# yanqinJiang/Animate3D

Measured on AMD Instinct MI355X. Metric: UNet denoise-steps/sec, 4view×16frame×512² MV-VDM @1/2/4/8 GPU, higher is better.
Workload: dtype bf16; 1 GPU; BASELINE config 2: 4 views x 16 frames x 512^2 px (64x64 latent), CFG-doubled batch V=8 videos, one MVUNetMotionModel.forward per step, SD1.5 MV-VDM UNet 1.53 B params, seeded synthetic weights; parallelism=single GPU

## Files before the change

### animate3d_amd/csrc/gemm_common.h

```cpp
#pragma once
#include "common.h"

struct GemmParams {
  const uint16_t* X; int64_t ldx;
  const uint16_t* W; int64_t ldw;
  const float* bias;
  const uint16_t* rowbias; int64_t rb_div;
  const uint16_t* R; int64_t ldr;
  uint16_t* Y; int64_t ldy;
  int64_t M, N, K;
  float alpha, beta;
  int vec16;
  int out_f32;
  int B, H, Wd, Cin, Ho, Wo, stride, up, He, We;
  int64_t tiles_n, tiles_m;
  int ksplit, nk_item;
  float* ws; int64_t ws_bytes;
  const uint16_t* X2; int64_t ldx2; int64_t K1;
};

constexpr int EPI_LINEAR = 0, EPI_GEGLU = 1;

static inline int a3d_gemm_kernel_of(int flags) { return flags & A3D_GEMM_KERNEL_MASK; }
static inline int a3d_gemm_reserved_cus_of(int flags) { return flags & A3D_GEMM_RESERVED_CUS_MASK; }

A3D_DEV float epi_scale(float v, float alpha) { return __fmul_rn(v, alpha); }
A3D_DEV float epi_axpy(float v, float beta, float r) { return __fmaf_rn(beta, r, v); }

A3D_DEV float gelu_erf(float gte) {
  const float x = fabsf(gte) * 0.70710678118654752f;
  const float t = __builtin_amdgcn_rcpf(fmaf(0.3275911f, x, 1.0f));
  float poly = fmaf(1.061405429f, t, -1.453152027f);
  poly = fmaf(poly, t, 1.421413741f);
  poly = fmaf(poly, t, -0.284496736f);
  poly = fmaf(poly, t, 0.254829592f);
  poly *= t;
  const float e = __builtin_amdgcn_exp2f(-x * x * 1.4426950408889634f);
  const float erfx = fmaf(-poly, e, 1.0f);
  const float hg = __fmul_rn(0.5f, gte);
  return __fmaf_rn(fabsf(hg), erfx, hg);
}

A3D_DEV f32x2_t splat2(float v) { return f32x2_t{v, v}; }
A3D_DEV f32x2_t gelu_erf2(f32x2_t g) {
  const f32x2_t x = __builtin_elementwise_abs(g) * 0.70710678118654752f;
  const f32x2_t den = __builtin_elementwise_fma(splat2(0.3275911f), x, splat2(1.0f));
  const f32x2_t t = {__builtin_amdgcn_rcpf(den[0]), __builtin_amdgcn_rcpf(den[1])};
  f32x2_t poly = __builtin_elementwise_fma(splat2(1.061405429f), t, splat2(-1.453152027f));
  poly = __builtin_elementwise_fma(poly, t, splat2(1.421413741f));
  poly = __builtin_elementwise_fma(poly, t, splat2(-0.284496736f));
  poly = __builtin_elementwise_fma(poly, t, splat2(0.254829592f));
  poly = poly * t;
  const f32x2_t a = (-x) * x * 1.4426950408889634f;
  const f32x2_t e = {__builtin_amdgcn_exp2f(a[0]), __builtin_amdgcn_exp2f(a[1])};
  const f32x2_t erfx = __builtin_elementwise_fma(-poly, e, splat2(1.0f));
  const f32x2_t hg = g * 0.5f;
  return __builtin_elementwise_fma(__builtin_elementwise_abs(hg), erfx, hg);
}
A3D_DEV void geglu8(const float (&hv)[8], const float (&gv)[8], const float (&bh)[8], const float (&bg)[8], float (&y)[8]) {
#pragma unroll
  for (int e = 0; e < 4; ++e) {
    const f32x2_t gg = f32x2_t{gv[2 * e], gv[2 * e + 1]} + f32x2_t{bg[2 * e], bg[2 * e + 1]};
    const f32x2_t hh = f32x2_t{hv[2 * e], hv[2 * e + 1]} + f32x2_t{bh[2 * e], bh[2 * e + 1]};
    const f32x2_t yy = hh * gelu_erf2(gg);
    y[2 * e] = yy[0]; y[2 * e + 1] = yy[1];
  }
}

static __device__ u32x4_t g_zero_page[4];

A3D_DEV uint32_t lds_addr(const void* p) {
  return (uint32_t)(uintptr_t)(__attribute__((address_space(3))) const void*)p;
}
A3D_DEV void glds16_v(const void* gsrc, uint32_t lds_dst) {
  unsigned keep;
  asm volatile("s_mov_b32 %0, m0\n\ts_mov_b32 m0, %2\n\ts_nop 0\n\tglobal_load_lds_dwordx4 %1, off\n\ts_mov_b32 m0, %0"
               : "=&s"(keep) : "v"(gsrc), "s"(__builtin_amdgcn_readfirstlane(lds_dst)) : "memory");
}
A3D_DEV void glds16_s(uint32_t voff, const void* sbase, uint32_t lds_dst) {
  unsigned keep;
  asm volatile("s_mov_b32 %0, m0\n\ts_mov_b32 m0, %3\n\ts_nop 0\n\tglobal_load_lds_dwordx4 %1, %2\n\ts_mov_b32 m0, %0"
               : "=&s"(keep) : "v"(voff), "s"(sbase), "s"(__builtin_amdgcn_readfirstlane(lds_dst)) : "memory");
}
A3D_DEV const uint16_t* scalar_ptr(const uint16_t* ptr) {
  const uint64_t a = (uint64_t)(uintptr_t)ptr;
  return (const uint16_t*)(uintptr_t)(((uint64_t)(uint32_t)__builtin_amdgcn_readfirstlane((int)(a >> 32)) << 32) |
                                      (uint32_t)__builtin_amdgcn_readfirstlane((int)(uint32_t)a));
}
A3D_DEV u32x4_t lds_vload128(const void* p) {
  return *(const volatile __attribute__((address_space(3))) u32x4_t*)(uintptr_t)lds_addr(p);
}
A3D_DEV u32x2_t lds_vload64(const void* p) {
  return *(const volatile __attribute__((address_space(3))) u32x2_t*)(uintptr_t)lds_addr(p);
}
A3D_DEV void wave_lds_fence() {
  __builtin_amdgcn_fence(__ATOMIC_RELEASE, "wavefront");
  __builtin_amdgcn_wave_barrier();
  __builtin_amdgcn_fence(__ATOMIC_ACQUIRE, "wavefront");
}

A3D_DEV void tile_barrier() {
  asm volatile("s_barrier" ::: "memory");
  __builtin_amdgcn_sched_barrier(0);
}

template <int NB> struct WaveCols {
  static constexpr int PASSES = (NB + 1) / 2;
  int first, last;
  __device__ __forceinline__ explicit WaveCols(int wn) : first(NB == 5 ? wn * 4 : wn * NB), last(NB == 5 ? 8 + wn : wn * NB + NB - 1) {}
  __device__ __forceinline__ int block(int tn) const { return tn < NB - 1 ? first + tn : last; }
  A3D_DEV int pass_width(int ps) { return 2 * ps + 1 < NB ? 64 : 32; }
  __device__ __forceinline__ int pass_col0(int ps) const { return block(2 * ps) * 32; }
};

constexpr int BIAS_IMG_STRIDE = 2048;
constexpr int BIAS_IMG_ROWBIAS = 1280;
constexpr int BIAS_IMG_DMA = 1024;
A3D_DEV const float* bias_image(const char* img, int par) { return reinterpret_cast<const float*>(img + par * BIAS_IMG_STRIDE); }
A3D_DEV const uint16_t* rowbias_image(const char* img, int par) {
  return reinterpret_cast<const uint16_t*>(img + par * BIAS_IMG_STRIDE + BIAS_IMG_ROWBIAS);
}
template <int THREADS> A3D_DEV void zero_absent_bias_images(char* img, const float* bias, const uint16_t* rowbias, int tid) {
  if (!bias || !rowbias) {
    uint32_t* const bz = reinterpret_cast<uint32_t*>(img);
    for (int i = tid; i < 2 * BIAS_IMG_STRIDE / 4; i += THREADS) {
      const int o = (i * 4) % BIAS_IMG_STRIDE;
      if ((o < BIAS_IMG_ROWBIAS && !bias) || (o >= BIAS_IMG_ROWBIAS && !rowbias)) bz[i] = 0u;
    }
    asm volatile("s_waitcnt lgkmcnt(0)" ::: "memory");
    tile_barrier();
  }
}

template <int NB> A3D_DEV void read_frags(const char* stage, uint32_t xrd, uint32_t wrd, uint32_t wrd_last, uint32_t ko, u32x4_t (&fx)[2],
                                          u32x4_t (&fw)[NB]) {
  const char* xs = stage + xrd;
  const char* ws = stage + wrd;
  const char* wl = stage + wrd_last;
#pragma unroll
  for (int tm = 0; tm < 2; ++tm) fx[tm] = *reinterpret_cast<const u32x4_t*>(xs + tm * 4096 + ko);
#pragma unroll
  for (int tn = 0; tn < NB - 1; ++tn) fw[tn] = *reinterpret_cast<const u32x4_t*>(ws + tn * 4096 + ko);
  fw[NB - 1] = *reinterpret_cast<const u32x4_t*>(wl + ko);
}

template <int EPI, int NB>
A3D_DEV void epilogue_rounded(const GemmParams& p, f32x16_t (&acc)[NB][2], float* const stg, const float* const bias_lds,
                              const uint16_t* const rowbias_lds, const int64_t m0, const int64_t n0, const int wm, const WaveCols<NB> wc,
                              const int lane) {
  const int wblk = wc.first, wblk_last = wc.last;
  auto pass_cols = [&](int ps) { return (2 * ps + 1 < NB) ? 64 : 32; };
  auto pass_col0 = [&](int ps) { return ((2 * ps + 1 < NB) ? wblk + 2 * ps : wblk_last) * 32; };
  const int l31 = lane & 31, g = lane >> 5;
  constexpr int NP = (NB + 1) / 2;
  constexpr int RS = (EPI == EPI_GEGLU) ? 64 : 128;
  char* const stg16 = reinterpret_cast<char*>(stg);
  const int wsw = (EPI == EPI_GEGLU) ? ((l31 >> 1) & 3) : (l31 & 7);
  const int whalf = 8 * (g ^ ((l31 >> 3) & 1));
  auto unswap = [](u32x4_t o, int row) {
    const bool sw = row & 8;
    u32x4_t r;
    r[0] = sw ? o[2] : o[0]; r[1] = sw ? o[3] : o[1]; r[2] = sw ? o[0] : o[2]; r[3] = sw ? o[1] : o[3];
    return r;
  };
  constexpr int BUF2 = 32 * RS;
#pragma unroll
  for (int pi = 0; pi < 2 * NP; ++pi) {
    const int tm = pi / NP, ps = pi % NP;
    const int ncol = pass_cols(ps);
    const int64_t mbase = m0 + wm * 64 + tm * 32;
    const int64_t nbase = n0 + pass_col0(ps);
    char* const sb = stg16 + (pi & 1) * BUF2;
    if constexpr (EPI == EPI_GEGLU) {
      u32x4_t bq[2][4];
      auto fetch = [&](int q2, int slot) __attribute__((always_inline)) {
#pragma unroll
        for (int h = 0; h < 2; ++h) {
          const int c0 = 8 * (2 * q2 + h) + 4 * g;
          bq[slot][2 * h] = lds_vload128(bias_lds + pass_col0(ps) + c0);
          bq[slot][2 * h + 1] = lds_vload128(bias_lds + pass_col0(ps) + 32 + c0);
        }
      };
      fetch(0, 0);
#pragma unroll
      for (int q2 = 0; q2 < 2; ++q2) {
        if (q2 + 1 < 2) fetch(q2 + 1, (q2 + 1) & 1);
        __builtin_amdgcn_sched_barrier(0);
        float hv[8], gv[8], bh[8], bg[8], y[8];
#pragma unroll
        for (int h = 0; h < 2; ++h) {
          const u32x4_t b0 = bq[q2 & 1][2 * h], b1 = bq[q2 & 1][2 * h + 1];
#pragma unroll
          for (int j = 0; j < 4; ++j) { bh[4 * h + j] = __uint_as_float(b0[j]); bg[4 * h + j] = __uint_as_float(b1[j]); }
#pragma unroll
          for (int j = 0; j < 4; ++j) { hv[4 * h + j] = acc[2 * ps][tm][4 * (2 * q2 + h) + j]; gv[4 * h + j] = acc[2 * ps + 1][tm][4 * (2 * q2 + h) + j]; }
        }
        geglu8(hv, gv, bh, bg, y);
#pragma unroll
        for (int h = 0; h < 2; ++h) {
          u32x2_t o;
          o[0] = pack16(y[4 * h], y[4 * h + 1]);
          o[1] = pack16(y[4 * h + 2], y[4 * h + 3]);
          *reinterpret_cast<u32x2_t*>(sb + l31 * RS + 16 * ((2 * q2 + h) ^ wsw) + whalf) = o;
        }
      }
      wave_lds_fence();
      const int cc = lane & 3;
      const int64_t oc = nbase / 2 + 8 * cc;
      u32x4_t ob[2];
#pragma unroll
      for (int j = 0; j < 2; ++j) {
        const int row = 16 * j + (lane >> 2);
        ob[j] = *reinterpret_cast<const u32x4_t*>(sb + row * RS + 16 * (cc ^ ((row >> 1) & 3)));
      }
#pragma unroll
      for (int j = 0; j < 2; ++j) {
        const int row = 16 * j + (lane >> 2);
        const int64_t m = mbase + row;
        const u32x4_t o = unswap(ob[j], row);
        *reinterpret_cast<u32x4_t*>(p.Y + m * p.ldy + oc) = o;
      }
    } else {
      constexpr int NQ = 8;
      const int nq = (2 * ps + 1 < NB) ? 8 : 4;
      u32x4_t bq[3];
      u32x2_t tq[3];
      auto fetch = [&](int idx, int slot) __attribute__((always_inline)) {
        const int c0 = (idx >> 2) * 32 + 8 * (idx & 3) + 4 * g;
        bq[slot] = lds_vload128(bias_lds + pass_col0(ps) + c0);
        tq[slot] = lds_vload64(rowbias_lds + pass_col0(ps) + c0);
      };
      auto quads = [&](auto with_c) __attribute__((always_inline)) {
        constexpr bool WITH = decltype(with_c)::value;
        if constexpr (WITH) { fetch(0, 0); fetch(1, 1); }
#pragma unroll
        for (int idx = 0; idx < NQ; ++idx) {
          if (idx >= nq) continue;
          const int tl = idx >> 2, q = idx & 3;
          const int tn = 2 * ps + tl;
          if constexpr (WITH) {
            if (idx + 2 < nq) fetch(idx + 2, (idx + 2) % 3);
            __builtin_amdgcn_sched_barrier(0);
          }
          float v[4] = {acc[tn][tm][4 * q], acc[tn][tm][4 * q + 1], acc[tn][tm][4 * q + 2], acc[tn][tm][4 * q + 3]};
          if constexpr (WITH) {
            const u32x4_t b = bq[idx % 3];
            v[0] += __uint_as_float(b[0]); v[1] += __uint_as_float(b[1]); v[2] += __uint_as_float(b[2]); v[3] += __uint_as_float(b[3]);
            const u32x2_t tb = tq[idx % 3];
            v[0] += lo16(tb[0]); v[1] += hi16(tb[0]); v[2] += lo16(tb[1]); v[3] += hi16(tb[1]);
          }
#pragma unroll
          for (int e = 0; e < 4; ++e) v[e] = epi_scale(v[e], p.alpha);
          u32x2_t o;
          o[0] = pack16(v[0], v[1]);
          o[1] = pack16(v[2], v[3]);
          *reinterpret_cast<u32x2_t*>(sb + l31 * RS + 16 * ((4 * tl + q) ^ wsw) + whalf) = o;
          if constexpr (WITH) __builtin_amdgcn_sched_barrier(0);
        }
      };
      if (p.bias || p.rowbias) quads(std::true_type{});
      else quads(std::false_type{});
      wave_lds_fence();
      const int lpr = ncol / 8;
      const int cc = lane & (lpr - 1);
      u32x4_t ob[4];
#pragma unroll
      for (int j = 0; j < 4; ++j) {
        if (j * (64 / lpr) >= 32) continue;
        const int row = (64 / lpr) * j + lane / lpr;
        ob[j] = *reinterpret_cast<const u32x4_t*>(sb + row * RS + 16 * (cc ^ (row & 7)));
      }
#pragma unroll
      for (int j = 0; j < 4; ++j) {
        if (j * (64 / lpr) >= 32) continue;
        const int row = (64 / lpr) * j + lane / lpr;
        const int64_t m = mbase + row;
        const u32x4_t o = unswap(ob[j], row);
        *reinterpret_cast<u32x4_t*>(p.Y + m * p.ldy + nbase + 8 * cc) = o;
      }
    }
  }
}

template <int NB>
A3D_DEV void epilogue_residual(const GemmParams& p, f32x16_t (&acc)[NB][2], float* const stg, const float* const bias_lds,
                               const uint16_t* const rowbias_lds, const int64_t m0, const int64_t n0, const int wm, const WaveCols<NB> wc,
                               const int lane) {
  const int l31 = lane & 31, g = lane >> 5;
  constexpr int SROW = 68;
  constexpr int NP = WaveCols<NB>::PASSES;
  u32x4_t rres[2][4];
  auto load_res = [&](int pi, int slot) {
    const int tm = pi / NP, ps = pi % NP;
    const int64_t mbase = m0 + wm * 64 + tm * 32;
    const int64_t nbase = n0 + wc.pass_col0(ps);
    if (WaveCols<NB>::pass_width(ps) == 64) {
#pragma unroll
      for (int j = 0; j < 4; ++j) {
        const int64_t m = mbase + 8 * j + (lane >> 3);
        rres[slot][j] = *reinterpret_cast<const u32x4_t*>(p.R + m * p.ldr + nbase + 8 * (lane & 7));
      }
    } else {
#pragma unroll
      for (int j = 0; j < 2; ++j) {
        const int64_t m = mbase + 16 * j + (lane >> 2);
        rres[slot][j] = *reinterpret_cast<const u32x4_t*>(p.R + m * p.ldr + nbase + 8 * (lane & 3));
      }
    }
  };
  load_res(0, 0);
#pragma unroll
  for (int pi = 0; pi < 2 * NP; ++pi) {
    const int tm = pi / NP, ps = pi % NP;
    const int ncol = WaveCols<NB>::pass_width(ps);
    if (pi + 1 < 2 * NP) load_res(pi + 1, (pi + 1) & 1);
#pragma unroll
    for (int tl = 0; tl < 2; ++tl) {
      const int tn = 2 * ps + tl;
      if (tn < NB) {
#pragma unroll
        for (int q = 0; q < 4; ++q) {
          float4 v;
          v.x = acc[tn][tm][4 * q]; v.y = acc[tn][tm][4 * q + 1]; v.z = acc[tn][tm][4 * q + 2]; v.w = acc[tn][tm][4 * q + 3];
          *reinterpret_cast<float4*>(stg + l31 * SROW + tl * 32 + 8 * q + 4 * g) = v;
        }
      }
    }
    wave_lds_fence();
    const int64_t mbase = m0 + wm * 64 + tm * 32;
    const int64_t nbase = n0 + wc.pass_col0(ps);

    const int lpr = ncol / 8;
    const int cc = lane & (lpr - 1);
    const int64_t n = nbase + 8 * cc;
    const int ncl = wc.pass_col0(ps) + 8 * cc;
    float bv[8];
#pragma unroll
    for (int e = 0; e < 8; ++e) bv[e] = bias_lds[ncl + e];
    const u32x4_t tb = *reinterpret_cast<const u32x4_t*>(rowbias_lds + ncl);
#pragma unroll
    for (int j = 0; j < 4; ++j) {
      if (j * (64 / lpr) >= 32) continue;
      const int row = (64 / lpr) * j + lane / lpr;
      const int64_t m = mbase + row;
      const float4 a0 = *reinterpret_cast<const float4*>(stg + row * SROW + 8 * cc);
      const float4 a1 = *reinterpret_cast<const float4*>(stg + row * SROW + 8 * cc + 4);
      float v[8] = {a0.x, a0.y, a0.z, a0.w, a1.x, a1.y, a1.z, a1.w};
#pragma unroll
      for (int e = 0; e < 8; ++e) v[e] += bv[e];
#pragma unroll
      for (int e = 0; e < 4; ++e) { v[2 * e] += lo16(tb[e]); v[2 * e + 1] += hi16(tb[e]); }
#pragma unroll
      for (int e = 0; e < 8; ++e) v[e] = epi_scale(v[e], p.alpha);
      const u32x4_t tr = rres[pi & 1][j];
#pragma unroll
      for (int e = 0; e < 4; ++e) { v[2 * e] = epi_axpy(v[2 * e], p.beta, lo16(tr[e])); v[2 * e + 1] = epi_axpy(v[2 * e + 1], p.beta, hi16(tr[e])); }
      u32x4_t o;
#pragma unroll
      for (int e = 0; e < 4; ++e) o[e] = pack16(v[2 * e], v[2 * e + 1]);
      *reinterpret_cast<u32x4_t*>(p.Y + m * p.ldy + n) = o;
    }
    wave_lds_fence();
  }
}


__attribute__((visibility("hidden"))) int A3D_FN(a3d_launch_gemm_pp)(int conv, int epi, int nb, hipStream_t stream, const GemmParams& p, int cus);
__attribute__((visibility("hidden"))) int A3D_FN(a3d_launch_gemm_ring)(int nb, hipStream_t stream, const GemmParams& p, int cus);
```

### animate3d_amd/csrc/gemm_conv.hip

```cpp
#include "gemm_common.h"

namespace {

constexpr int BM = 128, BN = 128;
template <int BKT> struct TileCfg {
  static constexpr int LROW = BKT + 8;
  static constexpr int TILE_ELEMS = 128 * LROW;
  static constexpr int STAGE_BYTES = 2 * 2 * TILE_ELEMS * 2;
  static constexpr int EPI_BYTES = 4 * 32 * 68 * 4;
  static constexpr int SMEM_BYTES = STAGE_BYTES > EPI_BYTES ? STAGE_BYTES : EPI_BYTES;
  static constexpr int CPR = BKT / 8;
  static constexpr int RPT = 256 / CPR;
  static constexpr int NPASS = 128 / RPT;
};



template <int CONV, int EPI, int BKT, bool RES>
__global__ __launch_bounds__(256, (BKT == 64 ? 2 : 3)) void gemm_kernel(const GemmParams p) {
  using TC = TileCfg<BKT>;
  constexpr int LROW = TC::LROW, TILE_ELEMS = TC::TILE_ELEMS, NPASS = TC::NPASS, RPT = TC::RPT, BK = BKT;
  extern __shared__ __attribute__((aligned(16))) uint16_t smem[];
  const int tid = threadIdx.x;
  const int lane = tid & 63, wid = tid >> 6;
  const int wm = wid >> 1, wn = wid & 1;
  const int l31 = lane & 31, g = lane >> 5;

  const int64_t nblk = p.tiles_n * p.tiles_m;
  const int64_t lid = xcd_remap(blockIdx.x, nblk);
  const int64_t tile_n = lid % p.tiles_n, tile_m = lid / p.tiles_n;
  const int64_t m0 = tile_m * BM, n0 = tile_n * BN;

  const int kc = tid % TC::CPR;
  const int srow = tid / TC::CPR;

  const uint16_t* a_ptr[NPASS];
  int a_b[CONV == 2 ? NPASS : 1], a_y[CONV == 2 ? NPASS : 1], a_x[CONV == 2 ? NPASS : 1];
  bool a_ok[NPASS];
  int a_mask[NPASS];
#pragma unroll
  for (int i = 0; i < NPASS; ++i) {
    int64_t m = m0 + srow + RPT * i;
    a_ok[i] = m < p.M;
    if (m >= p.M) m = p.M - 1;
    if constexpr (CONV != 0) {
      const int hw = p.Ho * p.Wo;
      const int b = (int)(m / hw);
      const int rem = (int)(m - (int64_t)b * hw);
      const int oy = rem / p.Wo, ox = rem - oy * p.Wo;
      if constexpr (CONV == 2) {
        a_b[i] = b; a_y[i] = oy; a_x[i] = ox;
        a_ptr[i] = nullptr; a_mask[i] = 0;
      } else {
        const int y0 = oy * p.stride - 1, x0 = ox * p.stride - 1;
        a_ptr[i] = p.X + (((int64_t)b * p.H + y0) * p.Wd + x0) * p.Cin + kc * 8;
        int mask = 0;
#pragma unroll
        for (int t = 0; t < 9; ++t) {
          const int yy = y0 + t / 3, xx = x0 + t % 3;
          if (a_ok[i] && yy >= 0 && yy < p.H && xx >= 0 && xx < p.Wd) mask |= 1 << t;
        }
        a_mask[i] = mask;
      }
    } else {
      a_ptr[i] = p.X + m * p.ldx + kc * 8;
      a_mask[i] = 0;
    }
  }
  const uint16_t* w_ptr[NPASS];
#pragma unroll
  for (int i = 0; i < NPASS; ++i) {
    int64_t n = n0 + srow + RPT * i;
    if (n >= p.N) n = p.N - 1;
    w_ptr[i] = p.W + n * p.ldw + kc * 8;
  }

  struct RegTile { u32x4_t a[NPASS], w[NPASS]; };
  RegTile rt0, rt1;
  auto load_tile = [&](int64_t k0, RegTile& rt) {
    u32x4_t (&ra)[NPASS] = rt.a; u32x4_t (&rw)[NPASS] = rt.w;
    if constexpr (CONV != 0) {
      {
        const int kt64 = (int)(k0 >> 6);
        const int c64 = kt64 / 9, t = kt64 - 9 * c64;
        k0 = (int64_t)t * p.Cin + c64 * 64 + (k0 & 63);
      }
      const int tap = (int)(k0 / p.Cin);
      const int ci0 = (int)(k0 - (int64_t)tap * p.Cin);
      const int ky = tap / 3, kx = tap - ky * 3;
      if constexpr (CONV == 1) {
        const int64_t toff = ((int64_t)ky * p.Wd + kx) * p.Cin + ci0;
#pragma unroll
        for (int i = 0; i < NPASS; ++i) {
          if ((a_mask[i] >> tap) & 1) ra[i] = *reinterpret_cast<const u32x4_t*>(a_ptr[i] + toff);
          else ra[i] = u32x4_t{0u, 0u, 0u, 0u};
        }
      } else {
        const int He = p.He, We = p.We;
#pragma unroll
        for (int i = 0; i < NPASS; ++i) {
          const int yy = a_y[i] + ky - 1, xx = a_x[i] + kx - 1;
          const bool ok = a_ok[i] && yy >= 0 && yy < He && xx >= 0 && xx < We;
          if (ok) {
            const uint16_t* src = p.X + (((int64_t)a_b[i] * p.H + (yy >> 1)) * p.Wd + (xx >> 1)) * p.Cin + ci0 + kc * 8;
            ra[i] = *reinterpret_cast<const u32x4_t*>(src);
          } else {
            ra[i] = u32x4_t{0u, 0u, 0u, 0u};
          }
        }
      }
    } else {
#pragma unroll
      for (int i = 0; i < NPASS; ++i) ra[i] = *reinterpret_cast<const u32x4_t*>(a_ptr[i] + k0);
    }
#pragma unroll
    for (int i = 0; i < NPASS; ++i) rw[i] = *reinterpret_cast<const u32x4_t*>(w_ptr[i] + k0);
  };
  auto store_tile = [&](int buf, const RegTile& rt) {
    const u32x4_t (&ra)[NPASS] = rt.a; const u32x4_t (&rw)[NPASS] = rt.w;
    uint16_t* As = smem + (buf * 2 + 0) * TILE_ELEMS;
    uint16_t* Ws = smem + (buf * 2 + 1) * TILE_ELEMS;
#pragma unroll
    for (int i = 0; i < NPASS; ++i) {
      *reinterpret_cast<u32x4_t*>(As + (srow + RPT * i) * LROW + kc * 8) = ra[i];
      *reinterpret_cast<u32x4_t*>(Ws + (srow + RPT * i) * LROW + kc * 8) = rw[i];
    }
  };

  f32x16_t acc[2][2];
#pragma unroll
  for (int a = 0; a < 2; ++a)
#pragma unroll
    for (int b = 0; b < 2; ++b)
#pragma unroll
      for (int r = 0; r < 16; ++r) acc[a][b][r] = 0.f;

  u32x4_t rres[RES ? 4 : 1];
  const int ecc = lane & 7;
  const int64_t en = n0 + wn * 64 + 8 * ecc;
  const bool epf = RES && (EPI == EPI_LINEAR) && p.R != nullptr && p.vec16 && en + 8 <= p.N;
  auto prefetch_residual = [&](int tm) {
    if constexpr (RES) {
#pragma unroll
      for (int j = 0; j < 4; ++j) {
        int64_t m = m0 + wm * 64 + tm * 32 + 8 * j + (lane >> 3);
        if (m >= p.M) m = p.M - 1;
        rres[j] = *reinterpret_cast<const u32x4_t*>(p.R + m * p.ldr + en);
      }
    }
  };

  const int64_t nk = p.K / BK;
  auto compute = [&](int cur) {
    const uint16_t* As = smem + (cur * 2 + 0) * TILE_ELEMS;
    const uint16_t* Ws = smem + (cur * 2 + 1) * TILE_ELEMS;
    u32x4_t fw[2][2], fa[2][2];
    auto load_frags = [&](int slot, int ks) {
#pragma unroll
      for (int t = 0; t < 2; ++t) {
        fw[slot][t] = *reinterpret_cast<const u32x4_t*>(Ws + (wn * 64 + t * 32 + l31) * LROW + ks * 16 + g * 8);
        fa[slot][t] = *reinterpret_cast<const u32x4_t*>(As + (wm * 64 + t * 32 + l31) * LROW + ks * 16 + g * 8);
      }
    };
    load_frags(0, 0);
#pragma unroll
    for (int ks = 0; ks < BK / 16; ++ks) {
      if (ks + 1 < BK / 16) load_frags((ks + 1) & 1, ks + 1);
#pragma unroll
      for (int tn = 0; tn < 2; ++tn)
#pragma unroll
        for (int tm = 0; tm < 2; ++tm) acc[tn][tm] = mfma32(fw[ks & 1][tn], fa[ks & 1][tm], acc[tn][tm]);
    }
  };

  load_tile(0, rt0);
  store_tile(0, rt0);
  if (nk > 1) load_tile(1 * BK, rt0);
  if (nk > 2) load_tile(2 * BK, rt1);
  __syncthreads();
  for (int64_t kt = 0;;) {
    if (kt + 1 >= nk && epf) prefetch_residual(0);
    compute(0);
    if (kt + 1 < nk) store_tile(1, rt0);
    if (kt + 3 < nk) load_tile((kt + 3) * BK, rt0);
    __syncthreads();
    if (++kt >= nk) break;
    if (kt + 1 >= nk && epf) prefetch_residual(0);
    compute(1);
    if (kt + 1 < nk) store_tile(0, rt1);
    if (kt + 3 < nk) load_tile((kt + 3) * BK, rt1);
    __syncthreads();
    if (++kt >= nk) break;
  }

  constexpr int SROW = 68;
  float* const stg = reinterpret_cast<float*>(smem) + wid * (32 * SROW);
#pragma unroll
  for (int tm = 0; tm < 2; ++tm) {
  if (tm == 1) __syncthreads();
#pragma unroll
  for (int tn = 0; tn < 2; ++tn)
#pragma unroll
    for (int q = 0; q < 4; ++q) {
      float4 v;
      v.x = acc[tn][tm][4 * q]; v.y = acc[tn][tm][4 * q + 1]; v.z = acc[tn][tm][4 * q + 2]; v.w = acc[tn][tm][4 * q + 3];
      *reinterpret_cast<float4*>(stg + l31 * SROW + tn * 32 + 8 * q + 4 * g) = v;
    }
  __syncthreads();
  const int64_t mbase = m0 + wm * 64 + tm * 32;

  if constexpr (EPI == EPI_GEGLU) {
    const int cc = lane & 3;
    const int64_t nh = n0 + wn * 64 + 8 * cc;
    const int64_t oc = (n0 + wn * 64) / 2 + 8 * cc;
    if (nh + 32 < p.N + 0 && oc + 8 <= p.N / 2) {
      float bh[8], bg[8];
#pragma unroll
      for (int e = 0; e < 8; ++e) { bh[e] = p.bias ? p.bias[nh + e] : 0.f; bg[e] = p.bias ? p.bias[nh + 32 + e] : 0.f; }
#pragma unroll
      for (int j = 0; j < 2; ++j) {
        const int row = 16 * j + (lane >> 2);
        const int64_t m = mbase + row;
        if (m >= p.M) continue;
        const float4 h0 = *reinterpret_cast<const float4*>(stg + row * SROW + 8 * cc);
        const float4 h1 = *reinterpret_cast<const float4*>(stg + row * SROW + 8 * cc + 4);
        const float4 g0 = *reinterpret_cast<const float4*>(stg + row * SROW + 32 + 8 * cc);
        const float4 g1 = *reinterpret_cast<const float4*>(stg + row * SROW + 32 + 8 * cc + 4);
        const float hv[8] = {h0.x, h0.y, h0.z, h0.w, h1.x, h1.y, h1.z, h1.w};
        const float gv[8] = {g0.x, g0.y, g0.z, g0.w, g1.x, g1.y, g1.z, g1.w};
        float y[8];
        geglu8(hv, gv, bh, bg, y);
        u32x4_t o;
#pragma unroll
        for (int e = 0; e < 4; ++e) o[e] = pack16(y[2 * e], y[2 * e + 1]);
        *reinterpret_cast<u32x4_t*>(p.Y + m * p.ldy + oc) = o;
      }
    }
  } else {
    const int cc = lane & 7;
    const int64_t n = n0 + wn * 64 + 8 * cc;
    if (n < p.N) {
      const bool full = (n + 8 <= p.N) && p.vec16;
      float bv[8];
#pragma unroll
      for (int e = 0; e < 8; ++e) bv[e] = (p.bias && n + e < p.N) ? p.bias[n + e] : 0.f;
#pragma unroll
      for (int j = 0; j < 4; ++j) {
        const int row = 8 * j + (lane >> 3);
        const int64_t m = mbase + row;
        if (m >= p.M) continue;
        const float4 a0 = *reinterpret_cast<const float4*>(stg + row * SROW + 8 * cc);
        const float4 a1 = *reinterpret_cast<const float4*>(stg + row * SROW + 8 * cc + 4);
        float v[8] = {a0.x, a0.y, a0.z, a0.w, a1.x, a1.y, a1.z, a1.w};
#pragma unroll
        for (int e = 0; e < 8; ++e) v[e] += bv[e];
        const uint16_t* rb = p.rowbias ? p.rowbias + (m / p.rb_div) * p.N + n : nullptr;
        const uint16_t* rr = p.R ? p.R + m * p.ldr + n : nullptr;
        uint16_t* yy = p.Y + m * p.ldy + n;
        if (full) {
          if (rb) {
            const u32x4_t t = *reinterpret_cast<const u32x4_t*>(rb);
#pragma unroll
            for (int e = 0; e < 4; ++e) { v[2 * e] += lo16(t[e]); v[2 * e + 1] += hi16(t[e]); }
          }
#pragma unroll
          for (int e = 0; e < 8; ++e) v[e] = epi_scale(v[e], p.alpha);
          if constexpr (RES) {
            if (rr) {
              const u32x4_t t = rres[j];
#pragma unroll
              for (int e = 0; e < 4; ++e) { v[2 * e] = epi_axpy(v[2 * e], p.beta, lo16(t[e])); v[2 * e + 1] = epi_axpy(v[2 * e + 1], p.beta, hi16(t[e])); }
            }
          }
          if (p.out_f32) {
            float* yf = reinterpret_cast<float*>(p.Y) + m * p.ldy + n;
            *reinterpret_cast<float4*>(yf) = float4{v[0], v[1], v[2], v[3]};
            *reinterpret_cast<float4*>(yf + 4) = float4{v[4], v[5], v[6], v[7]};
          } else {
            u32x4_t o;
#pragma unroll
            for (int e = 0; e < 4; ++e) o[e] = pack16(v[2 * e], v[2 * e + 1]);
            *reinterpret_cast<u32x4_t*>(yy) = o;
          }
        } else {
#pragma unroll
          for (int hh = 0; hh < 2; ++hh) {
            if (n + 4 * hh + 4 > p.N) continue;
            float w[4] = {v[4 * hh], v[4 * hh + 1], v[4 * hh + 2], v[4 * hh + 3]};
            if (rb) {
              const u32x2_t t = *reinterpret_cast<const u32x2_t*>(rb + 4 * hh);
              w[0] += lo16(t[0]); w[1] += hi16(t[0]); w[2] += lo16(t[1]); w[3] += hi16(t[1]);
            }
#pragma unroll
            for (int e = 0; e < 4; ++e) w[e] = epi_scale(w[e], p.alpha);
            if (rr) {
              const u32x2_t t = *reinterpret_cast<const u32x2_t*>(rr + 4 * hh);
              w[0] = epi_axpy(w[0], p.beta, lo16(t[0])); w[1] = epi_axpy(w[1], p.beta, hi16(t[0]));
              w[2] = epi_axpy(w[2], p.beta, lo16(t[1])); w[3] = epi_axpy(w[3], p.beta, hi16(t[1]));
            }
            u32x2_t o;
            o[0] = pack16(w[0], w[1]);
            o[1] = pack16(w[2], w[3]);
            *reinterpret_cast<u32x2_t*>(yy + 4 * hh) = o;
          }
        }
      }
    }
  }
  if (tm == 0 && epf) prefetch_residual(1);
  }
}


constexpr int PBM = 256;
constexpr int NOT_ELIGIBLE = -1000;

inline bool gemm_flags_ok(int flags) {
  return !(flags & ~(A3D_GEMM_RESERVED_CUS_MASK | A3D_GEMM_KERNEL_MASK)) && a3d_gemm_kernel_of(flags) <= A3D_GEMM_RING;
}

inline int device_cus() {
  static int cus_of[64] = {0};
  const int dev = a3d_current_device();
  if (cus_of[dev] == 0) {
    int n = 0;
    if (hipDeviceGetAttribute(&n, hipDeviceAttributeMultiprocessorCount, dev) != hipSuccess) return 0;
    cus_of[dev] = n > 0 ? n : 256;
  }
  return cus_of[dev];
}

constexpr int PERSIST_MIN_FILL = 50;
struct PPPlan { int nb, S, cus; int64_t tiles_m, tiles_n; };
constexpr int SPLITK_MAX = 16;
constexpr int SPLITK_MINK = 9;
template <int CONV, int EPI>
bool plan_persist(const GemmParams& p, int flags, bool allow_split, PPPlan& out) {
  if (a3d_gemm_kernel_of(flags) == A3D_GEMM_TILE128 || p.out_f32) return false;
  const int cus_dev = device_cus();
  if (cus_dev == 0) return false;
  const int reserved = a3d_gemm_reserved_cus_of(flags);
  const int cus = cus_dev - reserved > 32 ? cus_dev - reserved : 32;
  if (!p.vec16 || p.K % 64 != 0 || p.M % PBM != 0 || (p.rowbias && p.rb_div % PBM != 0)) return false;
  if (p.ldw % 64 != 0 || (CONV == 0 && p.ldx % 64 != 0)) return false;
  if (CONV == 0 && (uint64_t)p.ldx * 16u >= (1ull << 31)) return false;
  if ((uint64_t)p.ldw * 16u >= (1ull << 31)) return false;
  if (CONV != 0 && ((uint64_t)p.B * p.H * p.Wd + 2u * p.Wd + 2u) * (uint64_t)p.Cin * 2u >= (1ull << 32)) return false;
  const int64_t tm = (p.M + PBM - 1) / PBM;
  const int nk = (int)(p.K / 64);
  const int unit = CONV ? 9 : 1;
  const int cus_plan = cus_dev;
  constexpr int OVH = 12;
  int64_t best = -1, best1 = -1;
  int bnb = 0, bS = 1, bnb1 = 0;
  for (int nb = 5; nb >= 4; --nb) {
    if (EPI == EPI_GEGLU && nb == 5) continue;
    if (p.N % (nb * 64) != 0) continue;
    const int64_t tiles = tm * (p.N / (nb * 64));
    for (int S = 1; S <= (allow_split && EPI == EPI_LINEAR ? SPLITK_MAX : 1); ++S) {
      if ((nk / unit) % S != 0 || (S > 1 && nk / S < SPLITK_MINK)) continue;
      const int64_t items = tiles * S;
      const int64_t rounds = (items + cus_plan - 1) / cus_plan;
      if (items * 100 < rounds * cus_plan * PERSIST_MIN_FILL) continue;
      if (S > 1 && p.ws != nullptr && items * nb * 65536 > p.ws_bytes) continue;
      const int64_t cost = rounds * (nk / S + OVH) * nb * (nb == 4 ? 108 : 100) + (S > 1 ? 100 * nb : 0);
      if (S == 1 && (best1 < 0 || cost < best1)) { best1 = cost; bnb1 = nb; }
      if (best < 0 || cost < best) { best = cost; bnb = nb; bS = S; }
    }
  }
  if (best < 0) return false;
  if (bS > 1 && best1 >= 0 && best * 100 > best1 * 85) { bnb = bnb1; bS = 1; }
  out.nb = bnb; out.S = bS; out.cus = cus;
  out.tiles_m = tm; out.tiles_n = p.N / (bnb * 64);
  return true;
}

struct RingPlan { int nb, cus, cus_plan; int64_t cost; };
constexpr int RING_VS_PP_PCT = 75;
inline bool plan_ring(const GemmParams& p, int flags, RingPlan& out) {
  if (a3d_gemm_kernel_of(flags) == A3D_GEMM_TILE128 || p.out_f32 || !p.vec16 || p.X2 != nullptr) return false;
  if (p.M % 128 != 0 || p.K % 64 != 0 || p.K < 256 || p.ldx % 64 != 0 || p.ldw % 64 != 0) return false;
  if ((uint64_t)p.ldx * 64u >= (1ull << 32) || (uint64_t)p.ldw * 256u >= (1ull << 32)) return false;
  if (p.rowbias && p.rb_div % 128 != 0) return false;
  const int n = device_cus() ? device_cus() : 256;
  const int reserved = a3d_gemm_reserved_cus_of(flags);
  out.cus_plan = n;
  out.cus = n - reserved > 32 ? n - reserved : 32;
  out.nb = 0; out.cost = 0;
  for (int nb : {5, 4, 2}) {
    if (p.N % (64 * nb) != 0) continue;
    const int64_t tiles = (p.M / 128) * (p.N / (64 * nb));
    const int64_t rounds = (tiles + out.cus - 1) / out.cus;
    const int64_t cost = rounds * (128 + 64 * nb);
    if (out.nb == 0 || cost < out.cost) { out.nb = nb; out.cost = cost; }
  }
  return out.nb != 0;
}

template <int CONV, int EPI>
int try_launch_persist(hipStream_t stream, GemmParams& p, int flags) {
  PPPlan pl;
  if (!plan_persist<CONV, EPI>(p, flags, p.ws != nullptr, pl)) return NOT_ELIGIBLE;
  p.tiles_m = pl.tiles_m; p.tiles_n = pl.tiles_n;
  p.ksplit = pl.S; p.nk_item = (int)(p.K / 64) / pl.S;
  return A3D_FN(a3d_launch_gemm_pp)(CONV, EPI, pl.nb, stream, p, pl.cus);
}


template <int CONV, int EPI, int BKT, bool RES>
int launch_res(hipStream_t stream, GemmParams& p, int64_t nblk) {
  using TC = TileCfg<BKT>;
  static uint64_t attr_done = 0;
  if (int rc = a3d_once_per_device(attr_done, [] {
        return (int)hipFuncSetAttribute(reinterpret_cast<const void*>(&gemm_kernel<CONV, EPI, BKT, RES>),
                                        hipFuncAttributeMaxDynamicSharedMemorySize, TC::SMEM_BYTES); })) return rc;
  gemm_kernel<CONV, EPI, BKT, RES><<<dim3((unsigned)nblk), dim3(256), TC::SMEM_BYTES, stream>>>(p);
  return a3d_launch_status();
}

template <int CONV, int EPI, int BKT>
int launch_bk(hipStream_t stream, GemmParams& p, int64_t nblk) {
  if constexpr (EPI == EPI_LINEAR) {
    if (p.R != nullptr) return launch_res<CONV, EPI, BKT, true>(stream, p, nblk);
  }
  return launch_res<CONV, EPI, BKT, false>(stream, p, nblk);
}

template <int CONV, int EPI = EPI_LINEAR>
int launch(hipStream_t stream, GemmParams& p, int flags) {
  if (!gemm_flags_ok(flags)) return A3D_EINVAL;
  if constexpr (CONV == 0 && EPI == EPI_LINEAR) {
    RingPlan rp;
    if (plan_ring(p, flags, rp)) {
      PPPlan pl;
      bool ring = true;
      if (a3d_gemm_kernel_of(flags) != A3D_GEMM_RING && plan_persist<CONV, EPI>(p, flags, p.ws != nullptr, pl)) {
        const int64_t tiles = pl.tiles_m * pl.tiles_n * pl.S;
        const int64_t pp_cost = ((tiles + rp.cus_plan - 1) / rp.cus_plan) * (256 + 64 * pl.nb) * RING_VS_PP_PCT;
        ring = pl.S == 1 && rp.cost * 100 < pp_cost;
      }
      if (ring) {
        p.tiles_m = p.M / 128; p.tiles_n = p.N / (64 * rp.nb);
        return A3D_FN(a3d_launch_gemm_ring)(rp.nb, stream, p, rp.cus);
      }
    }
  }
  {
    const int rc = try_launch_persist<CONV, EPI>(stream, p, flags);
    if (rc != NOT_ELIGIBLE) return rc;
  }
  p.tiles_m = (p.M + BM - 1) / BM;
  p.tiles_n = (p.N + BN - 1) / BN;
  const int64_t nblk = p.tiles_m * p.tiles_n;
  if (nblk <= 0 || nblk > 0x7fffffffLL) return A3D_EINVAL;
  const bool small = (CONV == 0 && p.K <= 640) || nblk < 768;
  if (small) return launch_bk<CONV, EPI, 32>(stream, p, nblk);
  return launch_bk<CONV, EPI, 64>(stream, p, nblk);
}

template <int CONV>
int64_t splitk_ws_bytes(const GemmParams& p, int flags) {
  PPPlan pl;
  GemmParams q = p;
  q.ws = nullptr; q.ws_bytes = 0;
  if (!gemm_flags_ok(flags)) return 0;
  if (!plan_persist<CONV, EPI_LINEAR>(q, flags, true, pl) || pl.S <= 1) return 0;
  return pl.tiles_m * pl.tiles_n * pl.S * pl.nb * 65536;
}

void attach_workspace(GemmParams& p, void* ws, int64_t ws_bytes) {
  if (ws && ws_bytes > 0 && a3d_aligned(16, ws)) { p.ws = (float*)ws; p.ws_bytes = ws_bytes; }
}

GemmParams dense_params(const void* X, int64_t ldx, const void* W, int64_t ldw, const float* bias, const void* rowbias, int64_t rb_div,
                        const void* R, int64_t ldr, void* Y, int64_t ldy, int64_t M, int64_t N, int64_t K, float alpha, float beta,
                        bool out_f32 = false) {
  GemmParams p{};
  p.X = (const uint16_t*)X; p.ldx = ldx; p.W = (const uint16_t*)W; p.ldw = ldw;
  p.bias = bias; p.rowbias = (const uint16_t*)rowbias; p.rb_div = rowbias ? rb_div : 1;
  p.R = (const uint16_t*)R; p.ldr = ldr; p.Y = (uint16_t*)Y; p.ldy = ldy;
  p.M = M; p.N = N; p.K = K; p.alpha = alpha; p.beta = beta; p.out_f32 = out_f32;
  p.vec16 = (ldy * (out_f32 ? 4 : 2) % 16 == 0) && a3d_aligned(16, Y) && (!R || (ldr % 8 == 0 && a3d_aligned(16, R))) &&
            (!rowbias || (N % 8 == 0 && a3d_aligned(16, rowbias)));
  return p;
}

bool dense_args_ok(const GemmParams& p, uintptr_t y_align, int n_div, int ldy_div) {
  if (!p.X || !p.W || !p.Y || p.M <= 0 || p.N <= 0 || p.K <= 0) return false;
  if (p.K % 64 != 0 || p.N % n_div != 0) return false;
  if (p.ldx % 8 != 0 || p.ldw % 8 != 0 || p.ldy % ldy_div != 0 || (p.R && p.ldr % 4 != 0)) return false;
  if (!a3d_aligned(16, p.X, p.W) || !a3d_aligned(16, p.bias) || !a3d_aligned(y_align, p.Y) || !a3d_aligned(8, p.R, p.rowbias)) return false;
  return !p.rowbias || p.rb_div > 0;
}

int gemm_entry(a3d_stream_t stream, const void* X, int64_t ldx, const void* W, int64_t ldw,
               const float* bias, const void* rowbias, int64_t rb_div, const void* R, int64_t ldr,
               void* Y, int64_t ldy, int64_t M, int64_t N, int64_t K, float alpha, float beta, int flags,
               void* ws, int64_t ws_bytes, int64_t* ws_needed) {
  GemmParams p = dense_params(X, ldx, W, ldw, bias, rowbias, rb_div, R, ldr, Y, ldy, M, N, K, alpha, beta);
  if (!dense_args_ok(p, 8, 4, 4)) return A3D_EINVAL;
  if (ws_needed) { *ws_needed = splitk_ws_bytes<0>(p, flags); return 0; }
  attach_workspace(p, ws, ws_bytes);
  return launch<0>((hipStream_t)stream, p, flags);
}

}

extern "C" int A3D_FN(a3d_gemm)(a3d_stream_t stream, const void* X, int64_t ldx, const void* W, int64_t ldw,
                             const float* bias, const void* rowbias, int64_t rb_div, const void* R, int64_t ldr,
                             void* Y, int64_t ldy, int64_t M, int64_t N, int64_t K, float alpha, float beta, int flags) {
  return gemm_entry(stream, X, ldx, W, ldw, bias, rowbias, rb_div, R, ldr, Y, ldy, M, N, K, alpha, beta, flags, nullptr, 0, nullptr);
}

extern "C" int A3D_FN(a3d_gemm_ws)(a3d_stream_t stream, const void* X, int64_t ldx, const void* W, int64_t ldw,
                                const float* bias, const void* rowbias, int64_t rb_div, const void* R, int64_t ldr,
                                void* Y, int64_t ldy, int64_t M, int64_t N, int64_t K, float alpha, float beta, int flags,
                                void* ws, int64_t ws_bytes, int64_t* ws_needed) {
  return gemm_entry(stream, X, ldx, W, ldw, bias, rowbias, rb_div, R, ldr, Y, ldy, M, N, K, alpha, beta, flags, ws, ws_bytes, ws_needed);
}

extern "C" int A3D_FN(a3d_gemm2)(a3d_stream_t stream, const void* X, int64_t ldx, const void* X2, int64_t ldx2, int64_t K1,
                              const void* W, int64_t ldw, const float* bias, void* Y, int64_t ldy, int64_t M, int64_t N, int64_t K, int flags) {
  GemmParams p = dense_params(X, ldx, W, ldw, bias, nullptr, 1, nullptr, 0, Y, ldy, M, N, K, 1.f, 0.f);
  p.X2 = (const uint16_t*)X2; p.ldx2 = ldx2; p.K1 = K1;
  if (!dense_args_ok(p, 16, 8, 8) || !X2 || K1 <= 0 || K1 >= K || K1 % 64 != 0 || ldx2 % 8 != 0 || !a3d_aligned(16, X2)) return A3D_EINVAL;
  if (!gemm_flags_ok(flags)) return A3D_EINVAL;
  if (ldx2 % 64 != 0 || (uint64_t)ldx2 * 16u >= (1ull << 31)) return A3D_EUNSUPPORTED;
  const int rc = try_launch_persist<0, EPI_LINEAR>((hipStream_t)stream, p, flags);
  return rc == NOT_ELIGIBLE ? A3D_EUNSUPPORTED : rc;
}

extern "C" int A3D_FN(a3d_gemm_f32out)(a3d_stream_t stream, const void* X, int64_t ldx, const void* W, int64_t ldw,
                                    const float* bias, float* Y, int64_t ldy, int64_t M, int64_t N, int64_t K, float alpha) {
  GemmParams p = dense_params(X, ldx, W, ldw, bias, nullptr, 1, nullptr, 0, Y, ldy, M, N, K, alpha, 0.f, true);
  if (!dense_args_ok(p, 16, 8, 4)) return A3D_EINVAL;
  return launch<0>((hipStream_t)stream, p, 0);
}

static int conv_entry(a3d_stream_t stream, const void* X, const void* Wp, const float* bias,
                      const void* rowbias, int64_t rb_div, const void* R, void* Y,
                      int B, int H, int W, int Cin, int Cout, int stride, int up2x, int flags,
                      void* ws, int64_t ws_bytes, int64_t* ws_needed) {
  if (!X || !Wp || !Y || B <= 0 || H <= 0 || W <= 0) return A3D_EINVAL;
  if (Cin % 64 != 0 || Cout % 4 != 0 || (stride != 1 && stride != 2)) return A3D_EINVAL;
  if (up2x < 0 || up2x > 7 || (up2x > 1 && !(up2x & 1)) || (up2x && stride != 1)) return A3D_EINVAL;
  if (!a3d_aligned(16, X, Wp) || !a3d_aligned(16, bias) || !a3d_aligned(8, Y)) return A3D_EINVAL;
  if (rowbias && rb_div <= 0) return A3D_EINVAL;
  const int He = up2x ? 2 * H - ((up2x >> 1) & 1) : H, We = up2x ? 2 * W - ((up2x >> 2) & 1) : W;
  if (He <= 0 || We <= 0) return A3D_EINVAL;
  GemmParams p{};
  p.X = (const uint16_t*)X; p.ldx = Cin; p.W = (const uint16_t*)Wp; p.ldw = (int64_t)9 * Cin;
  p.bias = bias; p.rowbias = (const uint16_t*)rowbias; p.rb_div = rowbias ? rb_div : 1;
  p.R = (const uint16_t*)R; p.ldr = Cout; p.Y = (uint16_t*)Y; p.ldy = Cout;
  p.B = B; p.H = H; p.Wd = W; p.Cin = Cin; p.stride = stride; p.up = up2x ? 1 : 0; p.He = He; p.We = We;
  p.Ho = (He + 2 - 3) / stride + 1; p.Wo = (We + 2 - 3) / stride + 1;
  p.M = (int64_t)B * p.Ho * p.Wo; p.N = Cout; p.K = (int64_t)9 * Cin;
  p.alpha = 1.f; p.beta = 1.f;
  p.vec16 = (Cout % 8 == 0) && a3d_aligned(16, Y, R, rowbias);
  if (ws_needed) { *ws_needed = up2x ? splitk_ws_bytes<2>(p, flags) : splitk_ws_bytes<1>(p, flags); return 0; }
  attach_workspace(p, ws, ws_bytes);
  return up2x ? launch<2>((hipStream_t)stream, p, flags) : launch<1>((hipStream_t)stream, p, flags);
}

extern "C" int A3D_FN(a3d_conv3x3)(a3d_stream_t stream, const void* X, const void* Wp, const float* bias,
                                const void* rowbias, int64_t rb_div, const void* R, void* Y,
                                int B, int H, int W, int Cin, int Cout, int stride, int up2x, int flags) {
  return conv_entry(stream, X, Wp, bias, rowbias, rb_div, R, Y, B, H, W, Cin, Cout, stride, up2x, flags, nullptr, 0, nullptr);
}

extern "C" int A3D_FN(a3d_conv3x3_ws)(a3d_stream_t stream, const void* X, const void* Wp, const float* bias,
                                   const void* rowbias, int64_t rb_div, const void* R, void* Y,
                                   int B, int H, int W, int Cin, int Cout, int stride, int up2x, int flags,
                                   void* ws, int64_t ws_bytes, int64_t* ws_needed) {
  return conv_entry(stream, X, Wp, bias, rowbias, rb_div, R, Y, B, H, W, Cin, Cout, stride, up2x, flags, ws, ws_bytes, ws_needed);
}

extern "C" int A3D_FN(a3d_gemm_geglu)(a3d_stream_t stream, const void* X, int64_t ldx, const void* W, int64_t ldw,
                                   const float* bias, void* Y, int64_t ldy, int64_t M, int64_t N2, int64_t K, int flags) {
  GemmParams p = dense_params(X, ldx, W, ldw, bias, nullptr, 1, nullptr, 0, Y, ldy, M, N2, K, 1.f, 0.f);
  if (!dense_args_ok(p, 16, 64, 8)) return A3D_EINVAL;
  return launch<0, EPI_GEGLU>((hipStream_t)stream, p, flags);
}
```

### animate3d_amd/csrc/gemm_pp.hip

```cpp
#include "gemm_common.h"

namespace {

constexpr int PBM = 256;
template <int NB> struct PPCfg {
  static constexpr int BN = NB * 64;
  static constexpr int XBYTES = PBM * 128;
  static constexpr int WBYTES = BN * 128;
  static constexpr int EPI_BYTES = 8 * 32 * 68 * 4;
  static constexpr int STAGE = (XBYTES + WBYTES) > EPI_BYTES ? (XBYTES + WBYTES) : EPI_BYTES;
  static constexpr int BIAS_OFF = 2 * STAGE;
  static constexpr int SMEM = BIAS_OFF + 2 * BIAS_IMG_STRIDE;
};

constexpr int PP_GM = 8;
A3D_DEV void pp_tile_coords(int64_t t, int64_t tiles_m, int64_t tiles_n, int64_t& tile_m, int64_t& tile_n) {
  const int64_t gsz = PP_GM * tiles_n;
  const int64_t blk = t / gsz;
  const int64_t first = blk * PP_GM;
  const int64_t gm = tiles_m - first < PP_GM ? tiles_m - first : PP_GM;
  const int64_t within = t - blk * gsz;
  tile_n = within / gm;
  tile_m = first + (within - tile_n * gm);
}

template <int CONV, int EPI, int NB, bool RES, bool SPLIT = false, bool TWO = false>
__global__ __launch_bounds__(512, 1) void gemm_pp_kernel(const GemmParams p) {
  static_assert(!TWO || CONV == 0, "the two-source A operand is a dense-GEMM feature");
  using PC = PPCfg<NB>;
  constexpr int PH = 1, NPH = 4;
  constexpr int NP = 4 + NB;
  extern __shared__ __attribute__((aligned(16))) uint16_t smem[];
  char* const smem_b = reinterpret_cast<char*>(smem);
  const int tid = threadIdx.x, lane = tid & 63;
  const int wid = __builtin_amdgcn_readfirstlane(tid >> 6);
  const int wm = wid >> 1, wn = wid & 1;
  const int grp = wid >> 2;
  const int l31 = lane & 31, g = lane >> 5;
  const int lr = lane >> 3, pos = lane & 7;
  const uint32_t lds0 = lds_addr(smem);

  const int S = SPLIT ? p.ksplit : 1;
  const int64_t ntiles = p.tiles_m * p.tiles_n * S;
  const int64_t G = gridDim.x;
  int64_t t = xcd_remap(blockIdx.x, G);
  if (t >= ntiles) return;
  const int nk = SPLIT ? p.nk_item : (int)(p.K / 64);

  const uint32_t koff0 = (uint32_t)((g ^ ((l31 >> 1) & 7)) << 4);
  const uint32_t xrd = (uint32_t)(wm * 64 + l31) * 128u;
  const WaveCols<NB> wc(wn);
  const uint32_t wrd = (uint32_t)PC::XBYTES + (uint32_t)(wc.first * 32 + l31) * 128u;
  const uint32_t wrd_last = (uint32_t)PC::XBYTES + (uint32_t)(wc.last * 32 + l31) * 128u;

  const uint32_t vx0 = (uint32_t)(lr * p.ldx * 2 + ((pos ^ (lr >> 1)) << 4));
  const uint32_t vw0 = (uint32_t)(lr * p.ldw * 2 + ((pos ^ (lr >> 1)) << 4));
  uint32_t aoff[CONV ? 4 : 1];
  uint32_t amask[CONV ? 2 : 1];
  uint32_t sok[CONV ? 2 : 1];
  const int64_t cbias = CONV ? ((int64_t)p.Wd + 1) * p.Cin : 0;
  int64_t ld_m0 = 0, ld_n0 = 0;
  int ld_par = 0;
  int ik0 = 0, itap = 0, ikx = 0, iky = 0;
  uint64_t xck = 0;
  uint64_t zpage = 0;
  if constexpr (CONV != 0) {
    zpage = (uint64_t)(uintptr_t)g_zero_page;
    asm volatile("" : "+s"(zpage));
  }
  uint64_t xk = 0, wk = 0, rbk = 0;
  const uint32_t sx8 = (uint32_t)(p.ldx * 16), sw8 = (uint32_t)(p.ldw * 16);
  uint64_t xk2 = 0;
  const uint32_t vx0b = TWO ? (uint32_t)(lr * p.ldx2 * 2 + ((pos ^ (lr >> 1)) << 4)) : 0u;
  const uint32_t sx8b = TWO ? (uint32_t)(p.ldx2 * 16) : 0u;
  auto setup_tile = [&](int64_t tt) {
    int64_t tile_n, tile_m;
    const int64_t tile_id = SPLIT ? (int64_t)((uint32_t)tt / (uint32_t)S) : tt;
    const int64_t kofs = SPLIT ? (CONV ? ((int64_t)(tt - tile_id * S) * nk / 9) * 64 : (int64_t)(tt - tile_id * S) * nk * 64) : 0;
    pp_tile_coords(tile_id, p.tiles_m, p.tiles_n, tile_m, tile_n);
    ld_m0 = tile_m * PBM; ld_n0 = tile_n * PC::BN;
    ik0 = 0; itap = 0; ikx = 0; iky = 0;
    ld_par ^= 1;
    if constexpr (CONV != 0) xck = (uint64_t)(uintptr_t)p.X - (uint64_t)cbias * 2u + (uint64_t)kofs * 2u;
    if constexpr (CONV == 0) xk = (uint64_t)(uintptr_t)(p.X + (ld_m0 + wid * 32) * p.ldx + kofs);
    if constexpr (TWO) xk2 = (uint64_t)(uintptr_t)(p.X2 + (ld_m0 + wid * 32) * p.ldx2);
    wk = (uint64_t)(uintptr_t)(p.W + (ld_n0 + wid * (NB * 8)) * p.ldw + kofs);
    if (EPI == EPI_LINEAR && p.rowbias) rbk = (uint64_t)(uintptr_t)(p.rowbias + (ld_m0 / p.rb_div) * p.N + ld_n0);
    if constexpr (CONV != 0) {
      amask[0] = 0; amask[1] = 0;
#pragma unroll
      for (int i = 0; i < 4; ++i) {
        const int r = (wid * 4 + i) * 8 + lr;
        const int slot = pos ^ ((r >> 1) & 7);
        const uint32_t m = (uint32_t)ld_m0 + (uint32_t)r;
        const uint32_t hw = (uint32_t)(p.Ho * p.Wo);
        const int b = (int)(m / hw);
        const int rem = (int)(m - (uint32_t)b * hw);
        const int oy = (int)((uint32_t)rem / (uint32_t)p.Wo), ox = rem - oy * p.Wo;
        uint32_t mask = 0;
        if constexpr (CONV == 2) {
          const int sy0 = (oy - 1) >> 1, sx0 = (ox - 1) >> 1;
          aoff[i] = (uint32_t)(((((int64_t)b * p.H + sy0) * p.Wd + sx0) * p.Cin + cbias) * 2 + slot * 16);
#pragma unroll
          for (int tp = 0; tp < 9; ++tp) {
            const int yy = oy + tp / 3 - 1, xx = ox + tp % 3 - 1;
            if (yy >= 0 && yy < p.He && xx >= 0 && xx < p.We) mask |= 1u << tp;
          }
          amask[i >> 1] |= (mask << (9 * (i & 1))) | ((uint32_t)(~oy & 1) << (18 + 2 * (i & 1))) | ((uint32_t)(~ox & 1) << (19 + 2 * (i & 1)));
        } else {
          const int y0 = oy * p.stride - 1, x0 = ox * p.stride - 1;
          aoff[i] = (uint32_t)(((((int64_t)b * p.H + y0) * p.Wd + x0) * p.Cin + cbias) * 2 + slot * 16);
#pragma unroll
          for (int tp = 0; tp < 9; ++tp) {
            const int yy = y0 + tp / 3, xx = x0 + tp % 3;
            if (yy >= 0 && yy < p.H && xx >= 0 && xx < p.Wd) mask |= 1u << tp;
          }
          amask[i >> 1] |= mask << (9 * (i & 1));
        }
      }
      sok[0] = 0; sok[1] = 0;
#pragma unroll
      for (int bit = 0; bit < 18; ++bit) {
        if (__builtin_amdgcn_ballot_w64(((amask[0] >> bit) & 1u) != 0u) == ~0ull) sok[0] |= 1u << bit;
        if (__builtin_amdgcn_ballot_w64(((amask[1] >> bit) & 1u) != 0u) == ~0ull) sok[1] |= 1u << bit;
      }
    }
  };
  auto issue_pieces = [&](int buf, auto a_c, auto b_c) __attribute__((always_inline)) {
    constexpr int A = decltype(a_c)::value, B = decltype(b_c)::value;
    if constexpr (A >= B) return;
    const uint32_t dst = lds0 + (uint32_t)buf * PC::STAGE;
    if constexpr (A == 0) {
      if (ik0 == 0) {
        const uint32_t bdst = lds0 + (uint32_t)PC::BIAS_OFF + (uint32_t)ld_par * BIAS_IMG_STRIDE;
        if (p.bias) {
          if (wid == 0) glds16_s((uint32_t)lane * 16u, p.bias + ld_n0, bdst);
          if (NB == 5 && wid == 1) { if (lane < 16) glds16_s((uint32_t)lane * 16u, p.bias + ld_n0 + BIAS_IMG_DMA / 4, bdst + (uint32_t)BIAS_IMG_DMA); }
        }
        if (EPI == EPI_LINEAR && p.rowbias && wid == 2) {
          if (lane < PC::BN / 8) glds16_s((uint32_t)lane * 16u, (const void*)(uintptr_t)rbk, bdst + (uint32_t)BIAS_IMG_ROWBIAS);
        }
      }
    }
    if constexpr (CONV != 0) {
      const int ky = iky, kx = ikx;
      const uint32_t rowb = (uint32_t)(p.Wd * p.Cin * 2), colb = (uint32_t)(p.Cin * 2);
      const uint32_t yE = (uint32_t)((ky + 1) >> 1) * rowb, yO = (uint32_t)(ky >> 1) * rowb;
      const uint32_t xE = (uint32_t)((kx + 1) >> 1) * colb, xO = (uint32_t)(kx >> 1) * colb;
#pragma unroll
      for (int i = 0; i < 4; ++i) {
        if (i < A || i >= B) continue;
        const uint32_t d = dst + (uint32_t)(wid * 4 + i) * 1024u;
        const uint32_t mk = amask[i >> 1];
        uint32_t vo = aoff[i];
        if constexpr (CONV == 2) vo += (((mk >> (18 + 2 * (i & 1))) & 1u) ? yE : yO) + (((mk >> (19 + 2 * (i & 1))) & 1u) ? xE : xO);
        const int bit = itap + 9 * (i & 1);
        if ((sok[i >> 1] >> bit) & 1u) {
          glds16_s(vo, (const void*)(uintptr_t)xck, d);
        } else {
          const uint64_t src = ((mk >> bit) & 1u) ? xck + vo : zpage;
          glds16_v((const void*)(uintptr_t)src, d);
        }
      }
    } else {
      const bool sec = TWO && ik0 >= (int)p.K1;
      const uint32_t vxs = sec ? vx0b : vx0, sxs = sec ? sx8b : sx8;
      const uint64_t xks = sec ? xk2 : xk;
#pragma unroll
      for (int i = 0; i < 4; ++i) {
        if (i < A || i >= B) continue;
        const int pc = wid * 4 + i;
        glds16_s(vxs ^ (uint32_t)((i & 1) << 6), (const void*)(uintptr_t)(xks + (uint64_t)(uint32_t)(i * sxs)), dst + (uint32_t)pc * 1024u);
      }
    }
#pragma unroll
    for (int i = 0; i < NB; ++i) {
      if (4 + i < A || 4 + i >= B) continue;
      const int pc = wid * NB + i;
      glds16_s(vw0 ^ (uint32_t)((pc & 1) << 6), (const void*)(uintptr_t)(wk + (uint64_t)(uint32_t)(i * sw8)), dst + (uint32_t)PC::XBYTES + (uint32_t)pc * 1024u);
    }
    if constexpr (B == NP) {
      if constexpr (CONV != 0) {
        const uint64_t cin2 = (uint64_t)(uint32_t)p.Cin * 2u;
        wk += cin2;
        ++itap;
        if (++ikx == 3) { ikx = 0; ++iky; }
        if (itap == 9) {
          itap = 0; iky = 0; wk -= 9u * cin2 - 128u;
          if constexpr (CONV == 1) xck -= (2u * (uint64_t)(uint32_t)p.Wd + 2u) * cin2;
          xck += 128u;
        } else if constexpr (CONV == 1) {
          xck += ikx == 0 ? ((uint64_t)(uint32_t)p.Wd - 2u) * cin2 : cin2;
        }
      } else {
        if (TWO && ik0 >= (int)p.K1) xk2 += 128; else xk += 128;
        wk += 128;
      }
      ik0 += 64;
    }
  };
  auto issue_phase = [&](int buf, auto ph_c, bool late) __attribute__((always_inline)) {
    constexpr int ph = decltype(ph_c)::value;
    using I0 = std::integral_constant<int, 0>;
    using I3 = std::integral_constant<int, 3>;
    using I5 = std::integral_constant<int, 5>;
    using I6 = std::integral_constant<int, 6>;
    using IN = std::integral_constant<int, NP>;
    if (!late) {
      if constexpr (ph == 0) issue_pieces(buf, I0{}, I3{});
      if constexpr (ph == 1) issue_pieces(buf, I3{}, I6{});
      if constexpr (ph == 2) issue_pieces(buf, I6{}, IN{});
    } else {
      if constexpr (ph == 1) issue_pieces(buf, I0{}, I5{});
      if constexpr (ph == 2) issue_pieces(buf, I5{}, IN{});
    }
  };

  f32x16_t acc[NB][2];
  u32x4_t fx[PH][2], fw[PH][NB];
  auto load_frags = [&](int buf, int ks0) __attribute__((always_inline)) {
#pragma unroll
    for (int s = 0; s < PH; ++s) read_frags<NB>(smem_b + buf * PC::STAGE, xrd, wrd, wrd_last, koff0 ^ (uint32_t)((ks0 + s) << 5), fx[s], fw[s]);
  };
  auto mfma_phase = [&]() __attribute__((always_inline)) {
#pragma unroll
    for (int s = 0; s < PH; ++s)
#pragma unroll
      for (int tn = 0; tn < NB; ++tn)
#pragma unroll
        for (int tm = 0; tm < 2; ++tm) acc[tn][tm] = mfma32(fw[s][tn], fx[s][tm], acc[tn][tm]);
  };

  zero_absent_bias_images<512>(smem_b + PC::BIAS_OFF, p.bias, EPI == EPI_LINEAR ? p.rowbias : nullptr, tid);
  setup_tile(t);
  issue_pieces(0, std::integral_constant<int, 0>{}, std::integral_constant<int, NP>{});
  asm volatile("s_waitcnt vmcnt(0)" ::: "memory");
  tile_barrier();
  int buf = 0;
  for (;;) {
    int64_t tile_n, tile_m;
    pp_tile_coords(SPLIT ? (int64_t)((uint32_t)t / (uint32_t)S) : t, p.tiles_m, p.tiles_n, tile_m, tile_n);
    const int64_t m0 = tile_m * PBM, n0 = tile_n * PC::BN;
    const int64_t tnext = t + G;
#pragma unroll
    for (int a = 0; a < NB; ++a)
#pragma unroll
      for (int b = 0; b < 2; ++b)
#pragma unroll
        for (int r = 0; r < 16; ++r) acc[a][b][r] = 0.f;
    const int cur_par = ld_par;
    if (grp) tile_barrier();
    for (int kt = 0; kt < nk; ++kt) {
      const bool last = kt + 1 >= nk;
      const bool more = !last || tnext < ntiles;
      const bool late = kt == 0;
      static_for<NPH>([&](auto ph_c) __attribute__((always_inline)) {
        constexpr int ph = decltype(ph_c)::value;
        load_frags(buf, ph * PH);
        if (more) {
          if constexpr (ph == 0 || ph == 1) {
            if (last && (late ? ph == 1 : ph == 0)) setup_tile(tnext);
          }
          issue_phase(buf ^ 1, ph_c, late);
          if constexpr (ph == NPH - 1) { if (grp) asm volatile("s_waitcnt vmcnt(0)" ::: "memory"); }
        }
        asm volatile("s_waitcnt lgkmcnt(0)" ::: "memory");
        tile_barrier();
        __builtin_amdgcn_s_setprio(1);
        mfma_phase();
        __builtin_amdgcn_s_setprio(0);
        __builtin_amdgcn_sched_barrier(0);
        if constexpr (ph == NPH - 1) { if (more && !grp) asm volatile("s_waitcnt vmcnt(0)" ::: "memory"); }
        tile_barrier();
      });
      buf ^= 1;
    }
    if (!grp) tile_barrier();

    if constexpr (SPLIT) {
      float* const wsi = p.ws + ((t * 8 + wid) * (NB * 8)) * 256 + lane * 4;
#pragma unroll
      for (int tn = 0; tn < NB; ++tn)
#pragma unroll
        for (int tm = 0; tm < 2; ++tm)
#pragma unroll
          for (int q = 0; q < 4; ++q)
            *reinterpret_cast<float4*>(wsi + ((tn * 2 + tm) * 4 + q) * 256) =
                float4{acc[tn][tm][4 * q], acc[tn][tm][4 * q + 1], acc[tn][tm][4 * q + 2], acc[tn][tm][4 * q + 3]};
    } else {
      float* const stg = reinterpret_cast<float*>(smem_b + (buf ^ 1) * PC::STAGE) + wid * (32 * 68);
      const float* const bias_lds = bias_image(smem_b + PC::BIAS_OFF, cur_par);
      const uint16_t* const rowbias_lds = rowbias_image(smem_b + PC::BIAS_OFF, cur_par);
      if constexpr (EPI == EPI_GEGLU || !RES) epilogue_rounded<EPI, NB>(p, acc, stg, bias_lds, rowbias_lds, m0, n0, wm, wc, lane);
      else epilogue_residual<NB>(p, acc, stg, bias_lds, rowbias_lds, m0, n0, wm, wc, lane);
    }
    if (tnext >= ntiles) break;
    t = tnext;
  }
}

template <int NB>
__global__ __launch_bounds__(512) void splitk_reduce_kernel(const GemmParams p) {
  using PC = PPCfg<NB>;
  const int tid = threadIdx.x, lane = tid & 63, wid = tid >> 6;
  const int wm = wid >> 1, wn = wid & 1, l31 = lane & 31, g = lane >> 5;
  const WaveCols<NB> wc(wn);
  const int S = p.ksplit;
  int64_t tile_n, tile_m;
  pp_tile_coords(blockIdx.x, p.tiles_m, p.tiles_n, tile_m, tile_n);
  const int64_t m0 = tile_m * PBM, n0 = tile_n * PC::BN;
  const float* const w0 = p.ws + (((int64_t)blockIdx.x * S * 8 + wid) * (NB * 8)) * 256 + lane * 4;
  const int64_t item_stride = (int64_t)8 * NB * 8 * 256;
  const int tn = blockIdx.y;
#pragma unroll
    for (int tm = 0; tm < 2; ++tm) {
      const int64_t m = m0 + wm * 64 + tm * 32 + l31;
      const int64_t nb0 = n0 + wc.block(tn) * 32 + 4 * g;
#pragma unroll
      for (int q = 0; q < 4; ++q) {
        const float* src = w0 + ((tn * 2 + tm) * 4 + q) * 256;
        float4 a = *reinterpret_cast<const float4*>(src);
        for (int s = 1; s < S; ++s) {
          const float4 b = *reinterpret_cast<const float4*>(src + s * item_stride);
          a.x += b.x; a.y += b.y; a.z += b.z; a.w += b.w;
        }
        const int64_t n = nb0 + 8 * q;
        float v[4] = {a.x, a.y, a.z, a.w};
        if (p.bias) {
          const float4 b = *reinterpret_cast<const float4*>(p.bias + n);
          v[0] += b.x; v[1] += b.y; v[2] += b.z; v[3] += b.w;
        }
        if (p.rowbias) {
          const u32x2_t tb = *reinterpret_cast<const u32x2_t*>(p.rowbias + (m / p.rb_div) * p.N + n);
          v[0] += lo16(tb[0]); v[1] += hi16(tb[0]); v[2] += lo16(tb[1]); v[3] += hi16(tb[1]);
        }
#pragma unroll
        for (int e = 0; e < 4; ++e) v[e] = epi_scale(v[e], p.alpha);
        if (p.R) {
          const u32x2_t tr = *reinterpret_cast<const u32x2_t*>(p.R + m * p.ldr + n);
          v[0] = epi_axpy(v[0], p.beta, lo16(tr[0])); v[1] = epi_axpy(v[1], p.beta, hi16(tr[0]));
          v[2] = epi_axpy(v[2], p.beta, lo16(tr[1])); v[3] = epi_axpy(v[3], p.beta, hi16(tr[1]));
        }
        u32x2_t o;
        o[0] = pack16(v[0], v[1]);
        o[1] = pack16(v[2], v[3]);
        *reinterpret_cast<u32x2_t*>(p.Y + m * p.ldy + n) = o;
      }
    }
}

template <int CONV, int EPI, int NB, bool RES, bool SPLIT = false, bool TWO = false>
int launch_pp(hipStream_t stream, const GemmParams& p, int cus) {
  using PC = PPCfg<NB>;
  static uint64_t attr_done = 0;
  if (int rc = a3d_once_per_device(attr_done, [] {
        return (int)hipFuncSetAttribute(reinterpret_cast<const void*>(&gemm_pp_kernel<CONV, EPI, NB, RES, SPLIT, TWO>),
                                        hipFuncAttributeMaxDynamicSharedMemorySize, PC::SMEM); })) return rc;
  const int64_t ntiles = p.tiles_m * p.tiles_n * (SPLIT ? p.ksplit : 1);
  const unsigned grid = (unsigned)(ntiles < cus ? ntiles : cus);
  gemm_pp_kernel<CONV, EPI, NB, RES, SPLIT, TWO><<<dim3(grid), dim3(512), PC::SMEM, stream>>>(p);
  if (int rc = a3d_launch_status()) return rc;
  if constexpr (SPLIT) {
    splitk_reduce_kernel<NB><<<dim3((unsigned)(p.tiles_m * p.tiles_n), NB), dim3(512), 0, stream>>>(p);
    return a3d_launch_status();
  }
  return 0;
}

template <int CONV>
int launch_pp_conv(int epi, int nb, hipStream_t stream, const GemmParams& p, int cus) {
  if (epi == EPI_GEGLU) {
    if constexpr (CONV == 0) { if (nb == 4) return launch_pp<0, EPI_GEGLU, 4, false>(stream, p, cus); }
    return A3D_EUNSUPPORTED;
  }
  if constexpr (CONV == 0) {
    if (p.X2 != nullptr) {
      if (p.R || p.ksplit > 1) return A3D_EUNSUPPORTED;
      if (nb == 5) return launch_pp<0, EPI_LINEAR, 5, false, false, true>(stream, p, cus);
      if (nb == 4) return launch_pp<0, EPI_LINEAR, 4, false, false, true>(stream, p, cus);
      return A3D_EUNSUPPORTED;
    }
  }
  if (p.ksplit > 1) {
    if (nb == 5) return launch_pp<CONV, EPI_LINEAR, 5, false, true>(stream, p, cus);
    if (nb == 4) return launch_pp<CONV, EPI_LINEAR, 4, false, true>(stream, p, cus);
    return A3D_EUNSUPPORTED;
  }
  if (nb == 5) return p.R ? launch_pp<CONV, EPI_LINEAR, 5, true>(stream, p, cus) : launch_pp<CONV, EPI_LINEAR, 5, false>(stream, p, cus);
  if (nb == 4) return p.R ? launch_pp<CONV, EPI_LINEAR, 4, true>(stream, p, cus) : launch_pp<CONV, EPI_LINEAR, 4, false>(stream, p, cus);
  return A3D_EUNSUPPORTED;
}

}

int A3D_FN(a3d_launch_gemm_pp)(int conv, int epi, int nb, hipStream_t stream, const GemmParams& p, int cus) {
  if (conv == 0) return launch_pp_conv<0>(epi, nb, stream, p, cus);
  if (conv == 1) return launch_pp_conv<1>(epi, nb, stream, p, cus);
  return launch_pp_conv<2>(epi, nb, stream, p, cus);
}
```

### animate3d_amd/hip_ops.py

```python
from __future__ import annotations

import ctypes
import os
from dataclasses import dataclass
from typing import Optional

import torch

_LIB_PATH = os.path.join(os.path.dirname(os.path.abspath(__file__)), "lib", "libanimate3d_hip.so")
_lib = None

c_i64, c_int, c_f32, c_f64, c_vp = ctypes.c_int64, ctypes.c_int, ctypes.c_float, ctypes.c_double, ctypes.c_void_p


class _RowMapC(ctypes.Structure):
    _fields_ = [("gdiv", c_i64), ("ga", c_i64), ("gb", c_i64), ("seg_len", c_i64), ("seg_stride", c_i64), ("ld", c_i64)]


@dataclass(frozen=True)
class RowMap:
    gdiv: int
    ga: int
    gb: int
    seg_len: int
    seg_stride: int

    def c(self, ld: int) -> _RowMapC:
        return _RowMapC(self.gdiv, self.ga, self.gb, self.seg_len, self.seg_stride, ld)


def rowmap_rows(m: RowMap, groups: int, step: int, length: int, device="cpu") -> torch.Tensor:
    g = torch.arange(0, groups, step, device=device).view(-1, 1)
    s = torch.arange(length, device=device).view(1, -1)
    return ((g // m.gdiv) * m.ga + (g % m.gdiv) * m.gb + (s // m.seg_len) * m.seg_stride + s % m.seg_len).reshape(-1)


def rowmap_covers(m: RowMap, groups: int, step: int, length: int, rows: int, device="cpu") -> bool:
    if (groups + step - 1) // step * length != rows:
        return False
    idx = rowmap_rows(m, groups, step, length, device)
    return bool(int(idx.min()) >= 0 and int(idx.max()) < rows and torch.unique(idx).numel() == rows)


_SIGNATURES = {
    "a3d_version": (ctypes.c_char_p, []),
    "a3d_gemm_bf16": (c_int, [c_vp, c_vp, c_i64, c_vp, c_i64, c_vp, c_vp, c_i64, c_vp, c_i64, c_vp, c_i64, c_i64, c_i64, c_i64, c_f32, c_f32, c_int]),
    "a3d_gemm_ws_bf16": (c_int, [c_vp, c_vp, c_i64, c_vp, c_i64, c_vp, c_vp, c_i64, c_vp, c_i64, c_vp, c_i64, c_i64, c_i64, c_i64, c_f32, c_f32, c_int,
                                 c_vp, c_i64, ctypes.POINTER(c_i64)]),
    "a3d_gemm2_bf16": (c_int, [c_vp, c_vp, c_i64, c_vp, c_i64, c_i64, c_vp, c_i64, c_vp, c_vp, c_i64, c_i64, c_i64, c_i64, c_int]),
    "a3d_gemm_geglu_bf16": (c_int, [c_vp, c_vp, c_i64, c_vp, c_i64, c_vp, c_vp, c_i64, c_i64, c_i64, c_i64, c_int]),
    "a3d_conv3x3_bf16": (c_int, [c_vp, c_vp, c_vp, c_vp, c_vp, c_i64, c_vp, c_vp, c_int, c_int, c_int, c_int, c_int, c_int, c_int, c_int]),
    "a3d_conv3x3_ws_bf16": (c_int, [c_vp, c_vp, c_vp, c_vp, c_vp, c_i64, c_vp, c_vp, c_int, c_int, c_int, c_int, c_int, c_int, c_int, c_int,
                                    c_vp, c_i64, ctypes.POINTER(c_i64)]),
    "a3d_flash_attn_bf16": (c_int, [c_vp, c_vp, c_vp, c_vp, c_vp, ctypes.POINTER(_RowMapC), ctypes.POINTER(_RowMapC), ctypes.POINTER(_RowMapC),
                                    c_int, c_int, c_int, c_i64, c_i64, c_f32, c_f32, c_int]),
    "a3d_flash_attn_counted_bf16": (c_int, [c_vp, c_vp, c_vp, c_vp, c_vp, ctypes.POINTER(_RowMapC), ctypes.POINTER(_RowMapC), ctypes.POINTER(_RowMapC),
                                            c_int, c_int, c_int, c_i64, c_i64, c_f32, c_f32, c_int, c_vp]),
    "a3d_flash_attn2_bf16": (c_int, [c_vp, c_vp, c_vp, c_vp, c_vp, c_vp, c_vp, ctypes.POINTER(_RowMapC), ctypes.POINTER(_RowMapC), ctypes.POINTER(_RowMapC),
                                     ctypes.POINTER(_RowMapC), c_int, c_int, c_int, c_i64, c_i64, c_i64, c_f32, c_f32, c_f32, c_int]),
    "a3d_temporal_attn_bf16": (c_int, [c_vp, c_vp, c_vp, c_vp, c_i64, c_vp, c_i64, c_int, c_int, c_i64, c_int, c_int, c_f32]),
    "a3d_temporal_attn_sharded_bf16": (c_int, [c_vp, c_vp, c_i64, c_vp, c_vp, c_i64, c_vp, c_i64, c_int, c_int, c_i64, c_int, c_int, c_f32,
                                               c_int, c_int, c_int, c_i64]),
    "a3d_group_norm_ws_floats": (c_i64, [c_int, c_i64, c_int]),
    "a3d_group_norm_plan": (c_int, [c_i64, c_int, c_int, ctypes.POINTER(c_int)]),
    "a3d_group_norm_bf16": (c_int, [c_vp, c_vp, c_vp, c_vp, c_vp, c_vp, c_int, c_i64, c_int, c_int, c_f32, c_int]),
    "a3d_group_norm2_bf16": (c_int, [c_vp, c_vp, c_int, c_vp, c_int, c_vp, c_vp, c_vp, c_vp, c_int, c_i64, c_int, c_f32, c_int]),
    "a3d_group_norm_sums_bf16": (c_int, [c_vp, c_vp, c_vp, c_vp, c_int, c_i64, c_int, c_int]),
    "a3d_group_norm_apply_bf16": (c_int, [c_vp, c_vp, c_vp, c_vp, c_vp, c_vp, c_int, c_i64, c_int, c_int, c_int]),
    "a3d_layer_norm_bf16": (c_int, [c_vp, c_vp, c_vp, c_vp, c_vp, c_vp, c_i64, c_int, c_f32, c_vp, c_i64, c_i64, c_vp, c_i64, c_i64]),
    "a3d_geglu_bf16": (c_int, [c_vp, c_vp, c_i64, c_vp, c_i64, c_i64, c_i64]),
    "a3d_silu_bf16": (c_int, [c_vp, c_vp, c_vp, c_i64]),
    "a3d_activation_bf16": (c_int, [c_vp, c_vp, c_vp, c_i64, c_int]),
    "a3d_concat_bf16": (c_int, [c_vp, c_vp, c_i64, c_vp, c_i64, c_vp, c_i64]),
    "a3d_timestep_embed_bf16": (c_int, [c_vp, c_vp, c_vp, c_int, c_int]),
    "a3d_im2col_in": (c_int, [c_vp, c_vp, c_int, c_vp, c_int, c_int, c_int, c_int, c_int]),
    "a3d_unpack_out": (c_int, [c_vp, c_vp, c_vp, c_int, c_int, c_int, c_int, c_int, c_int]),
    "a3d_gemm_f32out_bf16": (c_int, [c_vp, c_vp, c_i64, c_vp, c_i64, c_vp, c_vp, c_i64, c_i64, c_i64, c_i64, c_f32]),
    "a3d_softmax_rows_f32_bf16": (c_int, [c_vp, c_vp, c_i64, c_vp, c_i64, c_i64, c_i64]),
    "a3d_softmax_rows_bwd_bf16": (c_int, [c_vp, c_vp, c_i64, c_vp, c_i64, c_vp, c_i64, c_i64, c_i64, c_f32]),
    "a3d_im2col_in_bwd": (c_int, [c_vp, c_vp, c_vp, c_int, c_int, c_int, c_int, c_int, c_f32]),
    "a3d_channel_mix_f32": (c_int, [c_vp, c_vp, c_vp, c_vp, c_vp, c_int, c_int, c_int, c_i64, c_f32]),
    "a3d_cfg_ddim_step_f32": (c_int, [c_vp, c_vp, c_vp, c_vp, c_vp, c_i64, c_int, c_int, c_i64, c_f32, c_f32, c_f32]),
    "a3d_flash_attn_bwd_bf16": (c_int, [c_vp, c_vp, c_vp, c_vp, c_vp, c_vp, c_vp, c_vp, c_vp, c_vp,
                                        ctypes.POINTER(_RowMapC), ctypes.POINTER(_RowMapC), ctypes.POINTER(_RowMapC), ctypes.POINTER(_RowMapC),
                                        ctypes.POINTER(_RowMapC), c_int, c_int, c_int, c_i64, c_i64, c_int, c_f32, c_f32, c_int]),
    "a3d_flash_attn_lse_bf16": (c_int, [c_vp, c_vp, c_vp, c_vp, c_vp, ctypes.POINTER(_RowMapC), ctypes.POINTER(_RowMapC), ctypes.POINTER(_RowMapC),
                                        c_int, c_int, c_int, c_i64, c_i64, c_f32, c_f32, c_int, c_vp]),
    "a3d_attn_delta_bf16": (c_int, [c_vp, c_vp, c_vp, ctypes.POINTER(_RowMapC), ctypes.POINTER(_RowMapC), c_vp, c_int, c_int, c_int, c_i64]),
    "a3d_temporal_attn_bwd_bf16": (c_int, [c_vp, c_vp, c_vp, c_vp, c_i64, c_vp, c_i64, c_vp, c_vp, c_vp, c_i64, c_int, c_int, c_i64, c_int, c_int, c_f32]),
    "a3d_layer_norm_bwd_bf16": (c_int, [c_vp, c_vp, c_vp, c_vp, c_vp, c_vp, c_vp, c_i64, c_int, c_f32, c_int]),
    "a3d_group_norm_bwd_bf16": (c_int, [c_vp, c_vp, c_vp, c_vp, c_vp, c_vp, c_vp, c_vp, c_vp, c_vp, c_int, c_i64, c_int, c_int, c_int]),
    "a3d_geglu_bwd_bf16": (c_int, [c_vp, c_vp, c_i64, c_vp, c_i64, c_vp, c_i64, c_i64, c_i64]),
    "a3d_transpose_bf16": (c_int, [c_vp, c_vp, c_i64, c_vp, c_i64, c_i64, c_i64, c_i64]),
    "a3d_wgrad_ws_floats": (c_i64, [c_i64, c_i64, c_i64]),
    "a3d_wgrad_bf16": (c_int, [c_vp, c_vp, c_i64, c_vp, c_i64, c_vp, c_i64, c_vp, c_i64, c_i64, c_i64, c_f32, c_int]),
    "a3d_colsum_bf16": (c_int, [c_vp, c_vp, c_i64, c_i64, c_i64, c_vp, c_f32, c_int]),
    "a3d_axpby_bf16": (c_int, [c_vp, c_vp, c_vp, c_i64, c_f32, c_f32]),
    "a3d_zero_insert2x_bf16": (c_int, [c_vp, c_vp, c_vp, c_int, c_int, c_int, c_int]),
    "a3d_upsample2x_bwd_bf16": (c_int, [c_vp, c_vp, c_vp, c_int, c_int, c_int, c_int, c_int, c_int]),
    "a3d_sqnorm_f32": (c_int, [c_vp, c_vp, c_i64, c_vp, c_int]),
    "a3d_clip_ctrl_f32": (c_int, [c_vp, c_vp, c_f32, c_f32, c_vp]),
    "a3d_adamw_f32": (c_int, [c_vp, c_vp, c_vp, c_vp, c_vp, c_i64, c_f32, c_f32, c_f32, c_f32, c_f32, c_f32, c_f32, c_vp]),
    "a3d_gs_preprocess_f32": (c_int, [c_vp, c_int, c_int, c_vp, c_i64, c_vp, c_i64, c_vp, c_i64, c_vp, c_i64, c_vp, c_i64, c_int, c_int, c_vp, c_i64, c_vp, c_vp, c_vp, c_vp, c_vp, c_int, c_int, c_f32, c_vp, c_vp, c_vp, c_vp, c_vp, c_vp, c_vp]),
    "a3d_gs_duplicate_f32": (c_int, [c_vp, c_int, c_int, c_int, c_int, c_vp, c_vp, c_vp, c_vp, c_vp, c_vp]),
    "a3d_gs_tile_ranges_f32": (c_int, [c_vp, c_vp, c_i64, c_vp, c_i64]),
    "a3d_gs_render_f32": (c_int, [c_vp, c_int, c_int, c_int, c_int, c_vp, c_vp, c_vp, c_vp, c_vp, c_vp, c_vp, c_vp, c_vp, c_vp, c_vp, c_vp, c_vp]),
    "a3d_gs_render_bwd_f32": (c_int, [c_vp, c_int, c_int, c_int, c_int, c_vp, c_vp, c_vp, c_vp, c_vp, c_vp, c_vp, c_vp, c_vp, c_vp, c_vp,
                                      c_vp, c_vp, c_vp]),
    "a3d_gs_preprocess_bwd_f32": (c_int, [c_vp, c_int, c_int, c_vp, c_i64, c_vp, c_i64, c_vp, c_i64, c_vp, c_i64, c_vp, c_i64, c_int, c_int, c_vp, c_i64, c_vp, c_vp, c_vp, c_vp, c_vp, c_int, c_int, c_f32, c_vp, c_vp, c_vp, c_vp, c_vp, c_vp, c_vp, c_vp, c_vp, c_vp, c_vp, c_vp]),
    "a3d_gs_sum_batch_f32": (c_int, [c_vp, c_vp, c_vp, c_int, c_i64]),
    "a3d_dg_cells_f32": (c_int, [c_vp, c_int, c_vp, c_vp, c_vp]),
    "a3d_dg_mean_partials": (c_i64, [c_int]),
    "a3d_dg_forward_f32": (c_int, [c_vp, c_int, c_int, c_int, c_vp, c_vp, c_vp, c_vp, c_vp, c_vp, c_vp, c_int, c_vp, c_vp, c_vp, c_vp, c_vp, c_vp,
                                   c_vp, c_vp, c_vp]),
    "a3d_dg_backward_ws_floats": (c_i64, [c_int, c_int, c_vp]),
    "a3d_dg_backward_f32": (c_int, [c_vp, c_int, c_int, c_int, c_vp, c_vp, c_vp, c_vp, c_vp, c_vp, c_vp, c_int, c_vp, c_vp, c_vp, c_vp, c_vp,
                                    c_vp, c_vp, c_vp, c_vp, c_vp, c_vp, c_vp, c_vp, c_vp, c_vp]),
    "a3d_knn_f32": (c_int, [c_vp, c_int, c_vp, c_int, c_int, c_f32, c_vp, c_vp]),
    "a3d_arap_energy_f32": (c_int, [c_vp, c_int, c_int, c_int, c_int, c_vp, c_vp, c_i64, c_vp, c_vp, c_vp, c_vp, c_vp, c_vp, c_vp]),
    "a3d_arap_backward_f32": (c_int, [c_vp, c_int, c_int, c_int, c_int, c_vp, c_vp, c_i64, c_vp, c_vp, c_vp, c_vp, c_vp, c_vp, c_vp, c_vp, c_vp]),
    "a3d_mesh_sample_neighbours": (c_int, [c_vp, c_int, c_int, c_vp, c_vp, c_int, c_vp, c_vp]),
    "a3d_mesh_vertex_gaussians_f32": (c_int, [c_vp, c_int, c_int, c_int, c_vp, c_vp, c_vp, c_vp, c_vp, c_vp, c_vp, c_vp, c_int, c_int, c_vp,
                                              c_int, c_vp, c_vp, c_f64, c_f64, c_vp, c_vp, c_vp, c_vp, c_vp, c_vp]),
    "a3d_gaussians_rigid_f32": (c_int, [c_vp, c_int, c_vp, c_vp, c_vp, c_vp, c_vp, c_f64, c_vp, c_vp, c_vp]),
    "a3d_mesh_vertex_normals_f32": (c_int, [c_vp, c_int, c_int, c_int, c_vp, c_vp, c_vp, c_vp, c_vp]),
    "a3d_cameras_spherical_f32": (c_int, [c_vp, c_int, c_vp, c_vp, c_vp, c_vp, c_vp, c_f64, c_f64, c_f64, c_vp, c_vp, c_vp, c_vp, c_vp]),
    "a3d_cameras_random_f32": (c_int, [c_vp, c_int, c_int, c_int, c_vp, c_vp, c_vp, c_vp, c_int, c_int, c_f64, c_f64, c_f64, c_f64, c_f64,
                                       c_vp, c_vp, c_vp, c_vp, c_vp, c_vp, c_vp, c_vp, c_vp]),
    "a3d_cameras_from_c2w_f32": (c_int, [c_vp, c_int, c_vp, c_vp, c_f64, c_f64, c_vp, c_vp, c_vp, c_vp]),
    "a3d_recon_loss_f32": (c_int, [c_vp, c_int, c_int, c_int, c_vp, c_vp, c_vp, c_vp, c_vp, c_f32, c_f64, c_f64, c_vp, c_i64, c_vp]),
    "a3d_recon_loss_bwd_f32": (c_int, [c_vp, c_int, c_int, c_int, c_vp, c_vp, c_vp, c_vp, c_vp, c_f32, c_f32, c_f32, c_vp, c_vp, c_vp]),
    "a3d_image_reg_f32": (c_int, [c_vp, c_int, c_int, c_int, c_vp, c_vp, c_vp, c_f64, c_f64, c_f64, c_vp, c_i64, c_vp]),
    "a3d_image_reg_bwd_f32": (c_int, [c_vp, c_int, c_int, c_int, c_vp, c_vp, c_vp, c_f32, c_f32, c_f32, c_f32, c_f32, c_vp, c_vp, c_vp, c_vp]),
    "a3d_gaussian_reg_f32": (c_int, [c_vp, c_int, c_int, c_vp, c_vp, c_i64, c_vp, c_vp, c_f64, c_f64, c_f64, c_vp, c_i64, c_vp]),
    "a3d_gaussian_reg_bwd_f32": (c_int, [c_vp, c_int, c_int, c_vp, c_vp, c_f32, c_f32, c_f32, c_vp, c_vp, c_vp, c_vp]),
    "a3d_clip_preprocess_lds_limit": (c_i64, []),
    "a3d_clip_preprocess": (c_int, [c_vp, c_vp, c_int, c_int, c_int, c_i64, c_i64, c_i64, c_i64, c_vp, c_int, c_int, c_vp, c_vp, c_int, c_int,
                                    c_vp, c_vp, c_int, c_int, c_int, c_int, c_vp, c_int, c_vp, c_vp, c_int, c_int, c_vp]),
}
_UNSUFFIXED_TWINS = ("a3d_im2col_in", "a3d_unpack_out", "a3d_im2col_in_bwd")
for _name in list(_SIGNATURES):
    if _name.endswith("_bf16"):
        _SIGNATURES[_name[:-5] + "_f16"] = _SIGNATURES[_name]
    elif _name in _UNSUFFIXED_TWINS:
        _SIGNATURES[_name + "_f16"] = _SIGNATURES[_name]
EXPORTED_SYMBOLS = tuple(_SIGNATURES)

_DTYPE_CODE = {torch.float32: 0, torch.bfloat16: 1, torch.float16: 2}
A3D_EUNSUPPORTED = -2


def lib_path() -> str:
    return _LIB_PATH


def load_library():
    global _lib
    if _lib is None:
        if not os.path.exists(_LIB_PATH):
            raise RuntimeError(f"{_LIB_PATH} is missing: run `python -m animate3d_amd.build` (or __graft_entry__.build()). "
                               "There is no CPU fallback for the MI355X kernels.")
        lib = ctypes.CDLL(_LIB_PATH)
        for name, (res, args) in _SIGNATURES.items():
            fn = getattr(lib, name)
            fn.restype, fn.argtypes = res, args
        _lib = lib
    return _lib


GN_PLAN_FIELDS = ("fused", "sg", "nx", "ny", "threads", "rmax", "stream")


def group_norm_plan(rows: int, C: int, groups: int) -> dict:
    out = (c_int * len(GN_PLAN_FIELDS))()
    _check(load_library().a3d_group_norm_plan(rows, C, groups, out), f"a3d_group_norm_plan rows={rows} C={C} groups={groups}")
    plan = dict(zip(GN_PLAN_FIELDS, out))
    plan["iters"] = -(-rows // plan["ny"]) if plan["fused"] else 0
    return plan


def _check(rc: int, what: str):
    if rc != 0:
        kind = {-1: "A3D_EINVAL (shape/alignment precondition)", -2: "A3D_EUNSUPPORTED"}.get(rc, f"hipError {rc}")
        raise RuntimeError(f"{what} failed: {kind}")


def _p(t: Optional[torch.Tensor]):
    return None if t is None else t.data_ptr()


def on_model_device(method):
    import functools

    @functools.wraps(method)
    def wrapper(self, *args, **kwargs):
        dev = self.device
        if dev.type == "cuda" and torch.cuda.current_device() != (dev.index if dev.index is not None else torch.cuda.current_device()):
            with torch.cuda.device(dev):
                return method(self, *args, **kwargs)
        return method(self, *args, **kwargs)
    return wrapper


class _Entry:

    def __init__(self, lib, f16: bool):
        self._lib, self._f16 = lib, f16

    def __getattr__(self, name):
        if self._f16:
            if name.endswith("_bf16"):
                name = name[:-5] + "_f16"
            elif name in _UNSUFFIXED_TWINS:
                name = name + "_f16"
        return getattr(self._lib, name)


class HipOps:

    has_attn_lse = True

    def __init__(self, device: Optional[torch.device] = None, act_dtype: torch.dtype = torch.bfloat16, split_k: bool = True):
        if not torch.cuda.is_available():
            raise RuntimeError("HipOps needs a visible MI355X (torch.cuda.is_available() is False); no CPU fallback exists")
        if act_dtype not in (torch.bfloat16, torch.float16):
            raise ValueError(f"storage type {act_dtype} is not supported (bfloat16 or float16)")
        self.raw_lib = load_library()
        self._kv_row_cache = {}
        self._kv_cover_cache = {}
        self.act_dtype = act_dtype
        self.lib = _Entry(self.raw_lib, act_dtype == torch.float16)
        self.device = torch.device(device) if device is not None else torch.device("cuda", torch.cuda.current_device())
        self.reserved_cus = 0
        self.split_k = bool(split_k)
        self.split_k_gemm = False
        self.attn_counters = None
        self._ws_plan = {}
        self._ws_bufs = {}

    def _workspace(self, need: int) -> torch.Tensor:
        if torch.cuda.is_current_stream_capturing():
            return torch.empty(max(need, 1 << 20), dtype=torch.uint8, device=self.device)
        stream = self._stream()
        buf = self._ws_bufs.get(stream)
        if buf is None or buf.numel() < need:
            buf = self._ws_bufs[stream] = torch.empty(max(need, 1 << 20), dtype=torch.uint8, device=self.device)
        return buf

    def _gemm_flags(self, tile128: bool, ring: bool = False) -> int:
        r = int(self.reserved_cus)
        if not 0 <= r <= 0xFF:
            raise ValueError(f"reserved_cus = {self.reserved_cus}: the flags word of a3d_gemm / a3d_conv3x3 carries 0..255 reserved compute units")
        return r | (0x100 if tile128 else (0x200 if ring else 0))

    def _stream(self):
        return torch.cuda.current_stream(self.device).cuda_stream

    def _act(self, t: torch.Tensor, name: str):
        if t.dtype != self.act_dtype or not t.is_cuda or t.dim() != 2 or t.stride(1) != 1:
            raise RuntimeError(f"{name}: expected a 2-D {self.act_dtype} CUDA tensor with contiguous rows, got {t.dtype} {tuple(t.shape)} {t.device} strides {t.stride()}")
        return t

    def split_cols(self, x, *bounds):
        return tuple(x[:, a:b] for a, b in zip(bounds[:-1], bounds[1:]))

    def empty(self, rows: int, cols: int) -> torch.Tensor:
        return torch.empty((rows, cols), dtype=self.act_dtype, device=self.device)

    def gemm(self, x, w, bias=None, *, residual=None, alpha: float = 1.0, beta: float = 1.0, rowbias=None, rb_div: int = 1, out=None,
             tile128: bool = False, ring: bool = False):
        x, w = self._act(x, "gemm.x"), self._act(w, "gemm.w")
        M, K = x.shape
        N = w.shape[0]
        assert w.shape[1] == K, (x.shape, w.shape)
        y = out if out is not None else self.empty(M, N)
        self._act(y, "gemm.out")
        if residual is not None:
            self._act(residual, "gemm.residual")
            assert residual.shape == (M, N)
        if rowbias is not None:
            self._act(rowbias, "gemm.rowbias")
            assert rowbias.is_contiguous() and rowbias.shape[1] == N
        if bias is not None:
            assert bias.dtype == torch.float32 and bias.numel() == N
        flags = self._gemm_flags(tile128, ring)
        args = (self._stream(), _p(x), x.stride(0), _p(w), w.stride(0), _p(bias), _p(rowbias), rb_div,
                _p(residual), residual.stride(0) if residual is not None else 0, _p(y), y.stride(0), M, N, K, alpha, beta, flags)
        if self.split_k and self.split_k_gemm and not tile128 and M <= 32768 and K >= 1152:
            key = ("gemm", M, N, K, x.stride(0), w.stride(0), y.stride(0), rb_div if rowbias is not None else 0, flags)
            need = self._ws_plan.get(key)
            if need is None:
                q = c_i64(0)
                _check(self.lib.a3d_gemm_ws_bf16(*args, None, 0, ctypes.byref(q)), f"a3d_gemm_ws_bf16 (query) M={M} N={N} K={K}")
                need = self._ws_plan[key] = int(q.value)
            if need > 0:
                ws = self._workspace(need)
                _check(self.lib.a3d_gemm_ws_bf16(*args, _p(ws), need, None), f"a3d_gemm_ws_bf16 M={M} N={N} K={K}")
                return y
        rc = self.lib.a3d_gemm_bf16(*args)
        _check(rc, f"a3d_gemm_bf16 M={M} N={N} K={K}")
        return y

    def gemm2(self, xa, xb, w, bias=None):
        xa, xb, w = self._act(xa, "gemm2.xa"), self._act(xb, "gemm2.xb"), self._act(w, "gemm2.w")
        M, K1 = xa.shape
        K = K1 + xb.shape[1]
        N = w.shape[0]
        assert xb.shape[0] == M and w.shape[1] == K
        if K1 % 64 or K % 64 or N % 8:
            return None
        y = self.empty(M, N)
        rc = self.lib.a3d_gemm2_bf16(self._stream(), _p(xa), xa.stride(0), _p(xb), xb.stride(0), K1, _p(w), w.stride(0), _p(bias), _p(y), y.stride(0),
                                     M, N, K, self._gemm_flags(False))
        if rc == A3D_EUNSUPPORTED:
            return None
        _check(rc, f"a3d_gemm2_bf16 M={M} N={N} K={K1}+{K - K1}")
        return y

    @staticmethod
    def interleave_geglu(w: torch.Tensor) -> torch.Tensor:
        n = w.shape[0] // 2
        assert n % 32 == 0
        h, g = w[:n].reshape(n // 32, 32, *w.shape[1:]), w[n:].reshape(n // 32, 32, *w.shape[1:])
        return torch.stack([h, g], dim=1).reshape(w.shape).contiguous()

    def gemm_geglu(self, x, w_il, bias_il, *, tile128: bool = False):
        x, w_il = self._act(x, "geglu.x"), self._act(w_il, "geglu.w")
        M, K = x.shape
        N2 = w_il.shape[0]
        y = self.empty(M, N2 // 2)
        rc = self.lib.a3d_gemm_geglu_bf16(self._stream(), _p(x), x.stride(0), _p(w_il), w_il.stride(0), _p(bias_il), _p(y), y.stride(0), M, N2, K,
                                          self._gemm_flags(tile128))
        _check(rc, f"a3d_gemm_geglu_bf16 M={M} N2={N2} K={K}")
        return y

    def conv3x3(self, x, B: int, H: int, W: int, w, bias, *, stride: int = 1, up2x: bool = False, rowbias=None, rb_div: int = 1, residual=None,
                up_size=None, tile128: bool = False):
        x, w = self._act(x, "conv.x"), self._act(w, "conv.w")
        Cin = x.shape[1]
        Cout = w.shape[0]
        assert x.is_contiguous() and w.is_contiguous() and x.shape[0] == B * H * W and w.shape[1] == 9 * Cin
        He, We = (2 * H, 2 * W) if up2x else (H, W)
        up_code = 1 if up2x else 0
        if up_size is not None:
            if not up2x or up_size[0] not in (2 * H, 2 * H - 1) or up_size[1] not in (2 * W, 2 * W - 1):
                raise ValueError(f"forced upsample size {tuple(up_size)} is not reachable from {(H, W)} (2x or 2x - 1 per axis)")
            He, We = int(up_size[0]), int(up_size[1])
            up_code |= (2 if He == 2 * H - 1 else 0) | (4 if We == 2 * W - 1 else 0)
        Ho, Wo = (He - 1) // stride + 1, (We - 1) // stride + 1
        y = self.empty(B * Ho * Wo, Cout)
        if residual is not None:
            assert residual.is_contiguous() and residual.shape == y.shape
        if rowbias is not None:
            assert rowbias.is_contiguous() and rowbias.shape[1] == Cout
        flags = self._gemm_flags(tile128)
        args = (self._stream(), _p(x), _p(w), _p(bias), _p(rowbias), rb_div, _p(residual), _p(y), B, H, W, Cin, Cout, stride, up_code, flags)
        if self.split_k and not tile128 and B * Ho * Wo <= 32768:
            key = ("conv", B, H, W, Cin, Cout, stride, up_code, rb_div if rowbias is not None else 0, flags)
            need = self._ws_plan.get(key)
            if need is None:
                q = c_i64(0)
                _check(self.lib.a3d_conv3x3_ws_bf16(*args, None, 0, ctypes.byref(q)), f"a3d_conv3x3_ws_bf16 (query) B={B} H={H} W={W} Cin={Cin} Cout={Cout}")
                need = self._ws_plan[key] = int(q.value)
            if need > 0:
                ws = self._workspace(need)
                _check(self.lib.a3d_conv3x3_ws_bf16(*args, _p(ws), need, None), f"a3d_conv3x3_ws_bf16 B={B} H={H} W={W} Cin={Cin} Cout={Cout}")
                return y, Ho, Wo
        rc = self.lib.a3d_conv3x3_bf16(*args)
        _check(rc, f"a3d_conv3x3_bf16 B={B} H={H} W={W} Cin={Cin} Cout={Cout} stride={stride} up={up2x}")
        return y, Ho, Wo

    def flash_attn(self, q, k, v, qmap: RowMap, kmap: RowMap, groups: int, heads: int, q_len: int, kv_len: int, *,
                   out=None, out_scale: float = 1.0, accumulate: bool = False, causal: bool = False, with_lse: bool = False,
                   accumulation_target: bool = False, exact: bool = False, plain: bool = False):
        q, k, v = self._act(q, "attn.q"), self._act(k, "attn.k"), self._act(v, "attn.v")
        C = q.shape[1]
        D = C // heads
        assert k.stride(0) == v.stride(0)
        o = out if out is not None else self.empty(q.shape[0], C)
        qm, km, om = qmap.c(q.stride(0)), kmap.c(k.stride(0)), qmap.c(o.stride(0))
        flags = (1 if accumulate else 0) | (2 if causal else 0) | (4 if exact else 0) | (8 if plain else 0)
        if with_lse:
            lse = torch.empty((groups, heads, q_len), dtype=torch.float32, device=self.device)
            rc = self.lib.a3d_flash_attn_lse_bf16(self._stream(), _p(q), _p(k), _p(v), _p(o), ctypes.byref(qm), ctypes.byref(km), ctypes.byref(om),
                                                  groups, heads, D, q_len, kv_len, float(D) ** -0.5, out_scale,
                                                  flags, _p(lse))
            _check(rc, f"a3d_flash_attn_lse_bf16 groups={groups} heads={heads} D={D} q_len={q_len} kv_len={kv_len}")
            return o, lse
        if self.attn_counters is not None:
            cnt = self.attn_counters
            assert cnt.dtype == torch.int32 and cnt.is_cuda and cnt.numel() >= 3 and cnt.is_contiguous()
            rc = self.lib.a3d_flash_attn_counted_bf16(self._stream(), _p(q), _p(k), _p(v), _p(o), ctypes.byref(qm), ctypes.byref(km), ctypes.byref(om),
                                                      groups, heads, D, q_len, kv_len, float(D) ** -0.5, out_scale, flags, _p(cnt))
            _check(rc, f"a3d_flash_attn_counted_bf16 groups={groups} heads={heads} D={D} q_len={q_len} kv_len={kv_len}")
            return o
        rc = self.lib.a3d_flash_attn_bf16(self._stream(), _p(q), _p(k), _p(v), _p(o), ctypes.byref(qm), ctypes.byref(km), ctypes.byref(om),
                                          groups, heads, D, q_len, kv_len, float(D) ** -0.5, out_scale, flags)
        _check(rc, f"a3d_flash_attn_bf16 groups={groups} heads={heads} D={D} q_len={q_len} kv_len={kv_len}")
        return o

    def flash_attn2(self, q, k, v, k2, v2, qmap: RowMap, kmap: RowMap, kmap2: RowMap, groups: int, heads: int, q_len: int, kv_len: int,
                    kv_len2: int, *, out_scale2: float = 1.0):
        D = q.shape[1] // heads
        if D not in (40, 80):
            return None
        q, k, v, k2, v2 = self._act(q, "attn.q"), self._act(k, "attn.k"), self._act(v, "attn.v"), self._act(k2, "attn.k2"), self._act(v2, "attn.v2")
        assert k.stride(0) == v.stride(0) and k2.stride(0) == v2.stride(0)
        o = self.empty(q.shape[0], q.shape[1])
        qm, km, km2, om = qmap.c(q.stride(0)), kmap.c(k.stride(0)), kmap2.c(k2.stride(0)), qmap.c(o.stride(0))
        rc = self.lib.a3d_flash_attn2_bf16(self._stream(), _p(q), _p(k), _p(v), _p(k2), _p(v2), _p(o), ctypes.byref(qm), ctypes.byref(km),
                                           ctypes.byref(km2), ctypes.byref(om), groups, heads, D, q_len, kv_len, kv_len2, float(D) ** -0.5,
                                           1.0, out_scale2, 0)
        _check(rc, f"a3d_flash_attn2_bf16 groups={groups} heads={heads} D={D} q_len={q_len} kv_len={kv_len} kv_len2={kv_len2}")
        return o

    def temporal_attn(self, q, k, v, videos: int, frames: int, L: int, heads: int, *, q_f0: int = 0, q_frames: Optional[int] = None,
                      out=None):
        q, k, v = self._act(q, "tattn.q"), self._act(k, "tattn.k"), self._act(v, "tattn.v")
        C = q.shape[1]
        D = C // heads
        assert k.stride(0) == v.stride(0)
        o = self._act(out, "tattn.out") if out is not None else self.empty(q.shape[0], C)
        assert o.shape == (q.shape[0], C)
        if q_frames is None or q_frames == frames:
            assert q.stride(0) == k.stride(0)
            rc = self.lib.a3d_temporal_attn_bf16(self._stream(), _p(q), _p(k), _p(v), q.stride(0), _p(o), o.stride(0),
                                                 videos, frames, L, heads, D, float(D) ** -0.5)
        else:
            assert q.shape[0] == videos * q_frames * L and k.shape[0] == videos * frames * L
            rc = self.lib.a3d_temporal_attn_sharded_bf16(self._stream(), _p(q), q.stride(0), _p(k), _p(v), k.stride(0), _p(o), o.stride(0),
                                                         videos, frames, L, heads, D, float(D) ** -0.5, q_f0, q_frames, q_frames,
                                                         videos * q_frames * L)
        _check(rc, f"a3d_temporal_attn_bf16 videos={videos} frames={frames} L={L} D={D} q_f0={q_f0} q_frames={q_frames}")
        return o

    def group_norm(self, x, B: int, rows: int, gamma, beta, groups: int, eps: float, silu: bool):
        x = self._act(x, "gn.x")
        assert x.is_contiguous() and x.shape[0] == B * rows
        C = x.shape[1]
        y = self.empty(x.shape[0], C)
        ws = torch.empty(int(self.lib.a3d_group_norm_ws_floats(B, rows, groups)), dtype=torch.float32, device=self.device)
        rc = self.lib.a3d_group_norm_bf16(self._stream(), _p(x), _p(y), _p(gamma), _p(beta), _p(ws), B, rows, C, groups, eps, 1 if silu else 0)
        _check(rc, f"a3d_group_norm_bf16 B={B} rows={rows} C={C}")
        return y

    def group_norm2(self, xa, xb, B: int, rows: int, gamma, beta, groups: int, eps: float, silu: bool):
        xa, xb = self._act(xa, "gn2.xa"), self._act(xb, "gn2.xb")
        assert xa.is_contiguous() and xb.is_contiguous() and xa.shape[0] == B * rows == xb.shape[0]
        Ca, Cb = xa.shape[1], xb.shape[1]
        y = self.empty(xa.shape[0], Ca + Cb)
        ws = torch.empty(int(self.lib.a3d_group_norm_ws_floats(B, rows, groups)), dtype=torch.float32, device=self.device)
        rc = self.lib.a3d_group_norm2_bf16(self._stream(), _p(xa), Ca, _p(xb), Cb, _p(y), _p(gamma), _p(beta), _p(ws), B, rows, groups, eps, 1 if silu else 0)
        _check(rc, f"a3d_group_norm2_bf16 B={B} rows={rows} C={Ca}+{Cb}")
        return y

    def group_norm_sums(self, x, B: int, rows: int, groups: int) -> torch.Tensor:
        x = self._act(x, "gn.x")
        assert x.is_contiguous() and x.shape[0] == B * rows
        ws = torch.empty(int(self.lib.a3d_group_norm_ws_floats(B, rows, groups)), dtype=torch.float32, device=self.device)
        sums = torch.empty((B, groups, 2), dtype=torch.float64, device=self.device)
        _check(self.lib.a3d_group_norm_sums_bf16(self._stream(), _p(x), _p(ws), _p(sums), B, rows, x.shape[1], groups),
               f"a3d_group_norm_sums_bf16 B={B} rows={rows} C={x.shape[1]}")
        return sums

    def group_norm_apply(self, x, B: int, rows: int, gamma, beta, groups: int, stats: torch.Tensor, silu: bool):
        x = self._act(x, "gn.x")
        assert x.is_contiguous() and x.shape[0] == B * rows
        assert stats.dtype == torch.float32 and stats.is_contiguous() and stats.shape == (B, groups, 2)
        y = self.empty(x.shape[0], x.shape[1])
        _check(self.lib.a3d_group_norm_apply_bf16(self._stream(), _p(x), _p(y), _p(gamma), _p(beta), _p(stats), B, rows, x.shape[1], groups,
                                                  1 if silu else 0), f"a3d_group_norm_apply_bf16 B={B} rows={rows} C={x.shape[1]}")
        return y

    def layer_norm(self, x, gamma, beta, eps: float, pe1=None, pe1_div: int = 1, pe2=None, pe2_div: int = 1, two: bool = False):
        x = self._act(x, "ln.x")
        assert x.is_contiguous()
        M, C = x.shape
        y1 = self.empty(M, C)
        y2 = self.empty(M, C) if two else None
        for pe in (pe1, pe2):
            if pe is not None:
                self._act(pe, "ln.pe")
                assert pe.is_contiguous() and pe.shape[1] == C
        rc = self.lib.a3d_layer_norm_bf16(self._stream(), _p(x), _p(y1), _p(y2), _p(gamma), _p(beta), M, C, eps,
                                          _p(pe1), pe1_div, pe1.shape[0] if pe1 is not None else 1,
                                          _p(pe2), pe2_div, pe2.shape[0] if pe2 is not None else 1)
        _check(rc, f"a3d_layer_norm_bf16 M={M} C={C}")
        return (y1, y2) if two else y1

    def geglu(self, x):
        x = self._act(x, "geglu.x")
        M, N2 = x.shape
        y = self.empty(M, N2 // 2)
        _check(self.lib.a3d_geglu_bf16(self._stream(), _p(x), x.stride(0), _p(y), y.stride(0), M, N2 // 2), "a3d_geglu_bf16")
        return y

    def silu(self, x):
        x = self._act(x, "silu.x")
        assert x.is_contiguous()
        y = torch.empty_like(x)
        _check(self.lib.a3d_silu_bf16(self._stream(), _p(x), _p(y), x.numel()), "a3d_silu_bf16")
        return y

    def activation(self, x, kind: str):
        x = self._act(x, "act.x")
        assert x.is_contiguous()
        y = torch.empty_like(x)
        _check(self.lib.a3d_activation_bf16(self._stream(), _p(x), _p(y), x.numel(), {"silu": 0, "quick_gelu": 1, "gelu": 2}[kind]), f"a3d_activation {kind}")
        return y

    def concat(self, a, b):
        a, b = self._act(a, "concat.a"), self._act(b, "concat.b")
        assert a.is_contiguous() and b.is_contiguous() and a.shape[0] == b.shape[0]
        y = self.empty(a.shape[0], a.shape[1] + b.shape[1])
        _check(self.lib.a3d_concat_bf16(self._stream(), _p(a), a.shape[1], _p(b), b.shape[1], _p(y), a.shape[0]), "a3d_concat_bf16")
        return y

    def timestep_embed(self, t: torch.Tensor, dim: int):
        assert t.dtype == torch.float32 and t.is_cuda and t.dim() == 1
        y = self.empty(t.shape[0], dim)
# ... 260 lines not shown
```

### animate3d_amd/unet.py

```python
from __future__ import annotations

import math
import os
import re
from types import SimpleNamespace
from typing import Any, Dict, Optional, Tuple, Union

import torch
import torch.nn as nn

from . import modules as M
from .config import UNetConfig
from .embeddings import sine_pos_2d, sinusoidal_pos_1d
from .hip_ops import RowMap, on_model_device


class UNet3DConditionOutput:

    def __init__(self, sample: torch.Tensor):
        self.sample = sample

    def __getitem__(self, i):
        return (self.sample,)[i]

# ... 301 lines not shown

    def _invalidate(self):
        self._packed = None
        self._packed_frozen = None
        if self._train_ops is not None:
            self._train_ops._persistent.clear()

    @property
    def ops(self):
        if self._active_ops is not None:
            return self._active_ops
        return self._base_ops()

    def _base_ops(self):
        if self._ops is None:
            from .hip_ops import HipOps
            self._ops = HipOps(self.device, torch.float16 if self.dtype == torch.float16 else torch.bfloat16)
            self._ops_auto = True
        return self._ops

    def _d(self, t: torch.Tensor) -> torch.Tensor:
        return t if (self._pack_grad and t.requires_grad) else t.detach()

    def _w(self, t: torch.Tensor) -> torch.Tensor:
        if self._pack_grad and t.requires_grad and t.is_leaf:
            return self._wcat([t])
        return self._d(t).to(self.ops.act_dtype).contiguous()

    def _wcat(self, ws, interleave: bool = False) -> torch.Tensor:
        if self._pack_grad and any(w.requires_grad for w in ws):
            from .autograd_ops import pack_weight
            return pack_weight(self.ops.act_dtype, list(ws), interleave)
        w = ws[0].detach() if len(ws) == 1 else torch.cat([w.detach() for w in ws], 0)
        if interleave:
            w = self.ops.interleave_geglu(w)
        return w.to(self.ops.act_dtype).contiguous()

    def _f(self, t: Optional[torch.Tensor]) -> Optional[torch.Tensor]:
        return None if t is None else self._d(t).float().contiguous()

    def _conv_w(self, conv: nn.Conv2d) -> torch.Tensor:
        w = self._d(conv.weight)
        return self._w(w.permute(0, 2, 3, 1).reshape(w.shape[0], -1))

    def _fold(self, a: torch.Tensor, b_t: torch.Tensor) -> torch.Tensor:
        ops = self._base_ops()
        dt = ops.act_dtype
        a, b_t = a.detach().float().contiguous(), b_t.detach().float().contiguous()
        ah, bh = a.to(dt), b_t.to(dt)
        al, bl = (a - ah.float()).to(dt), (b_t - bh.float()).to(dt)
        return ops.gemm_f32out(ah, bh) + ops.gemm_f32out(ah, bl) + ops.gemm_f32out(al, bh)

    def _pack_resnet(self, r: M.ResnetBlock2D):
        return SimpleNamespace(
            n1=(self._f(r.norm1.weight), self._f(r.norm1.bias)), eps=r.norm1.eps,
            c1=(self._conv_w(r.conv1), self._f(r.conv1.bias)),
            temb=(self._w(r.time_emb_proj.weight), self._f(r.time_emb_proj.bias)),
            n2=(self._f(r.norm2.weight), self._f(r.norm2.bias)),
            c2=(self._conv_w(r.conv2), self._f(r.conv2.bias)),
            sc=None if r.conv_shortcut is None else (self._conv_w(r.conv_shortcut), self._f(r.conv_shortcut.bias)))

    def _pack_ff(self, tb):
        return SimpleNamespace(n3=(self._f(tb.norm3.weight), self._f(tb.norm3.bias)),
                               ff1=(self._wcat([tb.ff.net[0].proj.weight], interleave=True),
                                    self._f(self.ops.interleave_geglu(self._d(tb.ff.net[0].proj.bias)))),
                               ff2=(self._w(tb.ff.net[2].weight), self._f(tb.ff.net[2].bias)))

    def _pack_t2d(self, t: M.Transformer2DModel):
        tb = t.transformer_blocks[0]
        a1, a2 = tb.attn1, tb.attn2
        p1, p2 = a1.processor, a2.processor
        if p1.kind not in ("mvdream", "mvdream_i2v") or p2.kind != "ip_adapter":
            raise TypeError("Transformer2D layers need a MVDream(I2V) processor on attn1 and an IPAdapter processor on attn2")
        qkv = [a1.to_k.weight, a1.to_v.weight, a1.to_q.weight]
        i2v = p1.kind == "mvdream_i2v"
        if i2v:
            qkv.append(p1.to_q_i2v.weight)
        out = SimpleNamespace(
            heads=a1.heads, i2v=i2v,
            norm=(self._f(t.norm.weight), self._f(t.norm.bias)),
            pin=(self._conv_w(t.proj_in), self._f(t.proj_in.bias)),
            n1=(self._f(tb.norm1.weight), self._f(tb.norm1.bias)),
            qkv=self._wcat(qkv),
            oi2v=(self._w(p1.to_out_i2v.weight), self._f(p1.to_out_i2v.bias)) if i2v else None,
            o1=(self._w(a1.to_out[0].weight), self._f(a1.to_out[0].bias)),
            n2=(self._f(tb.norm2.weight), self._f(tb.norm2.bias)),
            q2=self._w(a2.to_q.weight),
            kv_text=self._wcat([a2.to_k.weight, a2.to_v.weight]),
            kv_ip=[self._wcat([k.weight, v.weight]) for k, v in zip(p2.to_k_ip, p2.to_v_ip)],
            ip_scale=list(p2.scale), ip_tokens=list(p2.num_tokens),
            o2=(self._w(a2.to_out[0].weight), self._f(a2.to_out[0].bias)),
            pout=(self._conv_w(t.proj_out), self._f(t.proj_out.bias)))
        out.o1m = None
        if i2v and not self._pack_grad:
            wo, wi = a1.to_out[0].weight.detach().float(), p1.to_out_i2v.weight.detach().float()
            bias = a1.to_out[0].bias.detach().float()
            if p1.to_out_i2v.bias is not None:
                bias = bias + self._fold(p1.to_out_i2v.bias.detach().float()[None, :], wo)[0]
            out.o1m = (self._w(torch.cat([wo, self._fold(wo, wi.t())], dim=1)), self._f(bias))
        out.ff = self._pack_ff(tb)
        return out

    def _pack_motion(self, m: M.TransformerTemporalModel):
        tb = m.transformer_blocks[0]
        attns = []
        for a, ln in ((tb.attn1, tb.norm1), (tb.attn2, tb.norm2)):
            pr = a.processor
            if pr.kind != "spatio_temporal":
                raise TypeError("motion-module attention layers need a SpatioTemporalI2VAttnProcessor")
            C = a.to_q.weight.shape[0]
            if hasattr(pr, "time_pos_embed"):
                pe = pr.time_pos_embed.pe[0]
            else:
                pe = sinusoidal_pos_1d(C, self.config.motion_max_seq_length)[0].to(a.to_q.weight.device)
            proc_pe = hasattr(pr, "time_pos_embed")
            ct, cs, ci = pr.blend_coefficients_t() if self._pack_grad else pr.blend_coefficients()
            if self._pack_grad:
                self._coef_tensors.extend(c for c in (ct, cs, ci) if torch.is_tensor(c))
            ns = SimpleNamespace(
                heads=a.heads, spatial=pr.use_spatial_attn, image=pr.use_image_attn,
                spatial_pe=pr.use_spatial_attn and pr.use_spatial_encoding, camera_pe=pr.use_spatial_attn and pr.use_camera_encoding,
                n=(self._f(ln.weight), self._f(ln.bias)),
                qkv=self._wcat([a.to_q.weight, a.to_k.weight, a.to_v.weight]),
                o=(self._w(a.to_out[0].weight), self._f(a.to_out[0].bias)),
                pe_t=self._w(pe), coef=(ct, cs, ci), proc=pr,
                block_pe=not proc_pe)
            if pr.use_spatial_attn:
                ns.qkv_sp = self._wcat([pr.to_k_sp.weight, pr.to_v_sp.weight, pr.to_q_sp.weight])
                ns.osp = (self._w(pr.to_out_sp.weight), self._f(pr.to_out_sp.bias))
            if pr.use_image_attn:
                ns.qkv_img = self._wcat([pr.to_k_i2v.weight, pr.to_v_i2v.weight, pr.to_q_i2v.weight])
                ns.oimg = (self._w(pr.to_out_i2v.weight), self._f(pr.to_out_i2v.bias))
            ns.om = None
            if not self._pack_grad and (pr.use_spatial_attn or pr.use_image_attn):
                parts = [(ct, a.to_out[0])]
                if pr.use_spatial_attn:
                    parts.append((cs, pr.to_out_sp))
                if pr.use_image_attn:
                    parts.append((ci, pr.to_out_i2v))
                bias = None
                for c, lin in parts:
                    if lin.bias is not None:
                        bias = float(c) * lin.bias.detach().float() if bias is None else bias + float(c) * lin.bias.detach().float()
                ns.om = (self._w(torch.cat([float(c) * lin.weight.detach().float() for c, lin in parts], dim=1)), self._f(bias))
            attns.append(ns)
        out = SimpleNamespace(norm=(self._f(m.norm.weight), self._f(m.norm.bias)),
                              pin=(self._w(m.proj_in.weight), self._f(m.proj_in.bias)),
                              attns=attns,
                              pout=(self._w(m.proj_out.weight), self._f(m.proj_out.bias)))
        out.ff = self._pack_ff(tb)
        return out

    def _pack_block(self, blk: M.MotionBlock):
        return SimpleNamespace(
            resnets=[self._pack_resnet(r) for r in blk.resnets],
            t2d=[self._pack_t2d(t) for t in blk.attentions] if blk.has_cross_attention else None,
            motion=[self._pack_motion(m) for m in blk.motion_modules],
            down=None if blk.downsamplers is None else (self._conv_w(blk.downsamplers[0].conv), self._f(blk.downsamplers[0].conv.bias)),
            up=None if blk.upsamplers is None else (self._conv_w(blk.upsamplers[0].conv), self._f(blk.upsamplers[0].conv.bias)))

    def _pack(self):
        cfg = self.config
        dev = self.device
        te, P = self.time_embedding, SimpleNamespace()
        P.time = (self._w(te.linear_1.weight), self._f(te.linear_1.bias), self._w(te.linear_2.weight), self._f(te.linear_2.bias))
        P.cam = None
        if cfg.camera_embedding_dim is not None:
            ce = self.camera_embedding
            w1 = torch.zeros(ce.linear_1.weight.shape[0], 64, device=dev, dtype=torch.float32)
            w1[:, : cfg.camera_embedding_dim] = ce.linear_1.weight.detach().float()
            P.cam = (self._w(w1), self._f(ce.linear_1.bias), self._w(ce.linear_2.weight), self._f(ce.linear_2.bias))
        P.ip = None
        if self.encoder_hid_proj is not None:
            ipl = self.encoder_hid_proj.image_projection_layers[0]
            P.ip = (self._w(ipl.image_embeds.weight), self._f(ipl.image_embeds.bias), self._f(ipl.norm.weight), self._f(ipl.norm.bias), ipl.norm.eps)
        wi = self.conv_in.weight.detach().float().permute(0, 2, 3, 1).reshape(self.conv_in.weight.shape[0], -1)
        wpad = torch.zeros(wi.shape[0], 64, device=dev, dtype=torch.float32)
        wpad[:, : wi.shape[1]] = wi
        P.conv_in = (self._w(wpad), self._f(self.conv_in.bias))
        P.down = [self._pack_block(b) for b in self.down_blocks]
        P.mid = self._pack_block(self.mid_block)
        P.up = [self._pack_block(b) for b in self.up_blocks]
        P.norm_out = (self._f(self.conv_norm_out.weight), self._f(self.conv_norm_out.bias))
        P.conv_out = (self._conv_w(self.conv_out), self._f(self.conv_out.bias))
        P.cond = self._pack_conditioning(P)
        self._packed = P
        return P

    def _pack_conditioning(self, P):
        blocks = [*P.down, P.mid, *P.up]
        res = [r for b in blocks for r in b.resnets]
        t2d = [t for b in blocks if b.t2d is not None for t in b.t2d]
        c = SimpleNamespace(temb=None, kv_text=None, kv_ip=None, perm={}, widths=[r.temb[0].shape[0] for r in res])
        if res:
            off = 0
            for r in res:
                r.temb_off = (off, r.temb[0].shape[0])
                off += r.temb[0].shape[0]
            c.temb = (torch.cat([r.temb[0] for r in res], 0).contiguous(), torch.cat([r.temb[1] for r in res], 0).contiguous(), off)
        if t2d:
            off = 0
            for t in t2d:
                t.kv_off = (off, t.kv_text.shape[0])
                off += t.kv_text.shape[0]
            c.kv_text = torch.cat([t.kv_text for t in t2d], 0).contiguous()
            if all(len(t.kv_ip) == 1 and t.kv_ip[0].shape[0] == t.kv_text.shape[0] for t in t2d):
                c.kv_ip = torch.cat([t.kv_ip[0] for t in t2d], 0).contiguous()
        return c

    def _project_conditioning(self, c, semb, text_rows, ip_rows):
        ops = self.ops
        out = SimpleNamespace(tp=None, M=0, kvt=None, kvi=None)
        if c.temb is not None:
            M = semb.shape[0]
            perm = c.perm.get(M)
            if perm is None:
                total = c.temb[2]
                idx = torch.arange(M * total, device=semb.device).view(M, total)
                parts, off = [], 0
                for w in c.widths:
                    parts.append(idx[:, off:off + w].reshape(-1))
                    off += w
                perm = c.perm[M] = torch.cat(parts).contiguous()
            out.tp = ops.gemm(semb, c.temb[0], c.temb[1]).reshape(-1).index_select(0, perm)
            out.M = M
        if c.kv_text is not None:
            out.kvt = ops.gemm(text_rows, c.kv_text)
            if c.kv_ip is not None and len(ip_rows) == 1:
                out.kvi = ops.gemm(ip_rows[0], c.kv_ip)
        return out


    def _pe_spatial(self, C: int, h: int, w: int) -> torch.Tensor:
        key = (C, h, w)
        if key not in self._pe_cache:
            self._pe_cache[key] = sine_pos_2d(C // 2, h, w).to(device=self.device, dtype=self.ops.act_dtype).contiguous()
        return self._pe_cache[key]

    def _pe_spatial_general(self, a, C: int, h: int, w: int, n: int, F: int, view0: int = 0):
        pr = a.proc
        L = h * w
        pe = None
        if self._active_ops is not None:
            learn = ([pr.spatial_pos_embed.row_embed.weight, pr.spatial_pos_embed.col_embed.weight]
                     if a.spatial_pe and pr.spatial_encoding_type == "learnable" else [])
            learn += [pr.camera_embed.embedding_table.weight] if a.camera_pe and pr.camera_encoding_type == "learnable" else []
            if any(t.requires_grad for t in learn):
                raise NotImplementedError("learnable positional / camera-encoding tables are not trainable on this path (the reference's "
                                          "training configuration uses the sinusoid encodings); freeze them (requires_grad_(False))")
        if a.spatial_pe:
            if pr.spatial_encoding_type == "learnable":
                sp = pr.spatial_pos_embed
                if h > sp.row_embed.weight.shape[0] or w > sp.col_embed.weight.shape[0]:
                    raise ValueError(f"feature map {(h, w)} exceeds the learnable positional tables "
                                     f"({sp.row_embed.weight.shape[0]} x {sp.col_embed.weight.shape[0]})")
                xe = sp.col_embed.weight.detach().float()[:w][None, :, :].expand(h, w, -1)
                ye = sp.row_embed.weight.detach().float()[:h][:, None, :].expand(h, w, -1)
                pe = torch.cat([xe, ye], dim=-1).reshape(L, C).to(self.device)
            else:
                pe = sine_pos_2d(C // 2, h, w).to(self.device)
        if not a.camera_pe:
            return pe.to(self.ops.act_dtype).contiguous(), 1
        cam = pr.camera_embed.embedding_table.weight if pr.camera_encoding_type == "learnable" else pr.camera_embed.pe[0]
        cam = cam.detach().float().to(self.device)[view0:view0 + n]
        if cam.shape[0] != n:
            raise ValueError(f"camera encoding holds {pr.camera_embed} vectors, the call has views {view0}..{view0 + n}")
        tab = cam[:, None, None, :].expand(n, F, L, C)
        if pe is not None:
            tab = tab + pe[None, None, :, :]
        return tab.reshape(n * F * L, C).to(self.ops.act_dtype).contiguous(), 1

    def _resnet(self, x, B2, H, W, pk, semb, rb_rows):
        ops, g = self.ops, self.config.norm_num_groups
        L = H * W
        sc = None
        if isinstance(x, tuple):
            xa, xb = x
            sc = ops.gemm2(xa, xb, pk.sc[0], pk.sc[1]) if pk.sc is not None else None
            if sc is None:
                x = ops.concat(xa, xb)
                h = ops.group_norm(x, B2, L, pk.n1[0], pk.n1[1], g, pk.eps, True)
            else:
                h = ops.group_norm2(xa, xb, B2, L, pk.n1[0], pk.n1[1], g, pk.eps, True)
        else:
            h = ops.group_norm(x, B2, L, pk.n1[0], pk.n1[1], g, pk.eps, True)
        c = self._cond
        if c is not None and c.tp is not None and hasattr(pk, "temb_off"):
            o, N = pk.temb_off
            tp = c.tp[c.M * o: c.M * (o + N)].view(c.M, N)
        else:
            tp = ops.gemm(semb, pk.temb[0], pk.temb[1])
        h, _, _ = ops.conv3x3(h, B2, H, W, pk.c1[0], pk.c1[1], rowbias=tp, rb_div=rb_rows * L)
        h = ops.group_norm(h, B2, L, pk.n2[0], pk.n2[1], g, pk.eps, True)
        if sc is None:
            sc = x if pk.sc is None else ops.gemm(x, pk.sc[0], pk.sc[1])
        out, _, _ = ops.conv3x3(h, B2, H, W, pk.c2[0], pk.c2[1], residual=sc)
        return out

    def _ff(self, h, pk):
        ops = self.ops
        n3 = ops.layer_norm(h, pk.n3[0], pk.n3[1], 1e-5)
        u = ops.gemm_geglu(n3, pk.ff1[0], pk.ff1[1])
        return ops.gemm(u, pk.ff2[0], pk.ff2[1], residual=h)

    def _mv_maps(self, n, F, L):
        qm = RowMap(gdiv=F, ga=n * F * L, gb=L, seg_len=L, seg_stride=F * L)
        k0 = RowMap(gdiv=F, ga=n * F * L, gb=0, seg_len=L, seg_stride=F * L)
# ... 339 lines not shown

    def _forward_impl(self, sample, timestep, encoder_hidden_states, *, packed, timestep_cond, attention_mask, cross_attention_kwargs,
                      added_cond_kwargs, down_block_additional_residuals, mid_block_additional_residual, return_dict, camera, num_views,
                      i2v_cond_time_zero):
        assert sample.shape[0] % num_views == 0, "[UNet] input batch size must be dividable by num_views!"
        if timestep_cond is not None:
            raise ValueError("timestep_cond needs a time_embedding.cond_proj, which this UNet (time_cond_proj_dim = None) does not have")
        if attention_mask is not None:
            self._reject_attention_mask(attention_mask, sample, num_views)
        if cross_attention_kwargs:
            extra = set(cross_attention_kwargs) - {"scale"}
            if extra:
                raise NotImplementedError(f"cross_attention_kwargs {sorted(extra)} are not supported (only the LoRA `scale`, a no-op here)")
        residuals = down_block_additional_residuals is not None or mid_block_additional_residual is not None
        if residuals and (torch.is_grad_enabled() and getattr(self, "_training_enabled", False)):
            raise NotImplementedError("ControlNet residuals are an inference input (:787-796, 816-817); the training path does not differentiate them")
        if residuals and self.parallel is not None and self.parallel.world > 1:
            raise NotImplementedError("ControlNet residuals with a sharded (shard_unet) model are not supported")
        cfg, ops = self.config, self.ops
        V, _, F, H, W = sample.shape
        n = self.num_views or num_views
        if V % n != 0:
            raise AssertionError("[UNet] input batch size must be dividable by the processors' num_views!")
        nlev = len(cfg.block_out_channels)
        if min(H, W) < (1 << (nlev - 1)):
            raise ValueError(f"latent size {(H, W)} is smaller than the {1 << (nlev - 1)}x total down-sampling")
        if F > cfg.motion_max_seq_length:
            raise ValueError(f"num_frames {F} exceeds motion_max_seq_length {cfg.motion_max_seq_length}")
        P = packed if packed is not None else (self._packed if self._packed is not None else self._pack())
        dev, adt = sample.device, ops.act_dtype
        img_embeds = None if added_cond_kwargs is None else added_cond_kwargs.get("image_embeds")
        if torch.is_tensor(timestep) and timestep.numel() not in (1, V):
            raise ValueError(f"timestep must be a scalar or have one entry per video, got {tuple(timestep.shape)}")
        par = self.parallel if (self.parallel is not None and self.parallel.world > 1) else None
        V_full, n_full, F_full, f0 = V, n, F, 0
        if par is not None:
            par.configure(V // n, n, F)
            idx = par.local_videos_on(V, n, dev)
            f0, F = par.frame_range(F)
            sample = sample.index_select(0, idx)[:, :, f0:f0 + F]
            encoder_hidden_states = encoder_hidden_states.to(dev).index_select(0, idx)
            camera = None if camera is None else camera.to(dev).index_select(0, idx)
            img_embeds = None if img_embeds is None else img_embeds.to(dev).index_select(0, idx)
            if torch.is_tensor(timestep) and timestep.numel() == V:
                timestep = timestep.to(dev).reshape(-1).index_select(0, idx)
            V, n = idx.numel(), n // par.view_shards
        self._frames = (F_full, f0)
        B2 = V * F

        if not torch.is_tensor(timestep):
            t = torch.full((V,), float(timestep), dtype=torch.float32, device=dev)
        else:
            t = timestep.to(device=dev, dtype=torch.float32).reshape(-1).expand(V).contiguous()

        def time_mlp(tt):
            e = ops.gemm(ops.timestep_embed(tt, cfg.block_out_channels[0]), P.time[0], P.time[1])
            return ops.gemm(ops.silu(e), P.time[2], P.time[3])

        emb = time_mlp(t)
        cond_emb = time_mlp(torch.zeros_like(t)) if i2v_cond_time_zero else None
        if camera is not None:
            assert camera.shape[0] == V
            if P.cam is None:
                raise ValueError("camera passed but the model has no camera_embedding")
            cam = torch.zeros((V, 64), dtype=adt, device=dev)
            cam[:, : camera.shape[1]] = camera.to(device=dev, dtype=adt)
            c1 = ops.silu(ops.gemm(cam, P.cam[0], P.cam[1]))
            emb = ops.gemm(c1, P.cam[2], P.cam[3], residual=emb)
            if cond_emb is not None:
                cond_emb = ops.gemm(c1, P.cam[2], P.cam[3], residual=cond_emb)
        if cond_emb is None:
            semb, rb_rows = ops.silu(emb), F
        else:
            per_img = emb[:, None, :].repeat(1, F, 1)
            if f0 == 0:
                per_img[:, 0] = cond_emb
            semb, rb_rows = ops.silu(per_img.reshape(B2, -1).contiguous()), 1

        T = encoder_hidden_states.shape[1]
        text_rows = encoder_hidden_states.to(device=dev, dtype=adt).reshape(V * T, -1).contiguous()
        ip_rows = []
        if self.encoder_hid_proj is not None and cfg.encoder_hid_dim_type == "ip_image_proj":
            if img_embeds is None:
                raise ValueError(f"{self.__class__} has the config param `encoder_hid_dim_type` set to 'ip_image_proj' which requires the "
                                 "keyword argument `image_embeds` to be passed in  `added_conditions`")
            img = img_embeds.to(device=dev, dtype=adt).reshape(V, -1).contiguous()
            pr = ops.gemm(img, P.ip[0], P.ip[1]).reshape(V * cfg.ip_num_tokens, cfg.cross_attention_dim)
            ip_rows.append(ops.layer_norm(pr, P.ip[2], P.ip[3], P.ip[4]))

        self._cond = None
        if self.stack_conditioning and self._active_ops is None and getattr(P, "cond", None) is not None and P is self._packed:
            self._cond = self._project_conditioning(P.cond, semb, text_rows, ip_rows)

        x = ops.gemm(ops.im2col_in(sample), P.conv_in[0], P.conv_in[1])
        h_, w_ = H, W
        skips = [x]
        sizes = [(H, W)]
        ckpt = bool(getattr(self, "_gradient_checkpointing", False)) and torch.is_grad_enabled() and self._active_ops is not None

        def layer(x_in, rp, tp, mp, hh, ww):
            aops = self._active_ops
            def run(xx):
                prev, self._active_ops = self._active_ops, aops
                try:
                    xx = self._resnet(xx, B2, hh, ww, rp, semb, rb_rows)
                    if tp is not None:
                        xx = self._t2d(xx, V, n, F, hh, ww, tp, text_rows, ip_rows, T)
                    return self._motion(xx, V, n, F, hh, ww, mp)
                finally:
                    self._active_ops = prev
            if ckpt:
                from torch.utils.checkpoint import checkpoint
                return checkpoint(run, x_in, use_reentrant=False, preserve_rng_state=False)
            return run(x_in)

        for pk in P.down:
            for j, rp in enumerate(pk.resnets):
                x = layer(x, rp, pk.t2d[j] if pk.t2d is not None else None, pk.motion[j], h_, w_)
                skips.append(x)
            if pk.down is not None:
                x, h_, w_ = ops.conv3x3(x, B2, h_, w_, pk.down[0], pk.down[1], stride=2)
                skips.append(x)
                sizes.append((h_, w_))
        def plus(x_rows, res, hh, ww):
            C = x_rows.shape[1]
            if tuple(res.shape) != (B2, C, hh, ww):
                raise ValueError(f"additional residual of shape {tuple(res.shape)}, expected {(B2, C, hh, ww)}")
            r = ops.empty(B2 * hh * ww, C)
            r.copy_(res.to(device=dev).permute(0, 2, 3, 1).reshape(B2 * hh * ww, C))
            return ops.axpby_(x_rows, r, 1.0, 1.0)

        if down_block_additional_residuals is not None:
            if len(down_block_additional_residuals) != len(skips):
                raise ValueError(f"{len(down_block_additional_residuals)} down-block residuals for {len(skips)} skip connections")
            geo = [sizes[0]]
            for bi, pkd in enumerate(P.down):
                geo += [sizes[bi]] * len(pkd.resnets) + ([sizes[bi + 1]] if pkd.down is not None else [])
            skips = [plus(s_, r_, *g_) for s_, r_, g_ in zip(skips, down_block_additional_residuals, geo)]
        pk = P.mid
        x = layer(x, pk.resnets[0], pk.t2d[0], pk.motion[0], h_, w_)
        x = self._resnet(x, B2, h_, w_, pk.resnets[1], semb, rb_rows)
        if mid_block_additional_residual is not None:
            x = plus(x, mid_block_additional_residual, h_, w_)
        lvl = len(sizes) - 1
        for bi, (blk, pk) in enumerate(zip(self.up_blocks, P.up)):
            for j, rp in enumerate(pk.resnets):
                skip = skips.pop()
                if getattr(self, "_freeu_factors", None) is not None:
                    x, skip = self._freeu(bi, x, skip, B2, h_, w_)
                pair = self._active_ops is None and hasattr(ops, "gemm2") and hasattr(ops, "group_norm2")
                x = layer((x, skip) if pair else ops.concat(x, skip), rp, pk.t2d[j] if pk.t2d is not None else None, pk.motion[j], h_, w_)
            if pk.up is not None:
                lvl -= 1
                x, h_, w_ = ops.conv3x3(x, B2, h_, w_, pk.up[0], pk.up[1], up2x=True, up_size=sizes[lvl])
        x = ops.group_norm(x, B2, h_ * w_, P.norm_out[0], P.norm_out[1], cfg.norm_num_groups, cfg.norm_eps, True)
        x, _, _ = ops.conv3x3(x, B2, h_, w_, P.conv_out[0], P.conv_out[1])
        out_dtype = sample.dtype if sample.dtype in (torch.float32, torch.bfloat16, torch.float16) else torch.float32
        out = ops.unpack_out(x, V, cfg.out_channels, F, H, W, out_dtype)
        if par is not None:
            out = par.all_gather_output(out, V_full, n_full, F_full)
        if not return_dict:
            return (out,)
        return UNet3DConditionOutput(sample=out)
```

### include/animate3d_hip.h

```cpp
#ifndef ANIMATE3D_HIP_H
#define ANIMATE3D_HIP_H

#include <stdint.h>

#ifdef __cplusplus
extern "C" {
#endif

typedef void* a3d_stream_t;

enum {
  A3D_OK = 0,
  A3D_EINVAL = -1,
  A3D_EUNSUPPORTED = -2
};

enum { A3D_F32 = 0, A3D_BF16 = 1, A3D_F16 = 2 };

const char* a3d_version(void);

typedef struct a3d_rowmap {
  int64_t gdiv, ga, gb;
  int64_t seg_len, seg_stride;
  int64_t ld;
} a3d_rowmap;

#define A3D_GEMM_RESERVED_CUS_MASK 0xff
#define A3D_GEMM_KERNEL_MASK 0x300
#define A3D_GEMM_TILE128 0x100
#define A3D_GEMM_RING 0x200
int a3d_gemm_bf16(a3d_stream_t stream, const void* X, int64_t ldx, const void* W, int64_t ldw,
                  const float* bias, const void* rowbias, int64_t rb_div, const void* R, int64_t ldr,
                  void* Y, int64_t ldy, int64_t M, int64_t N, int64_t K, float alpha, float beta, int flags);

int a3d_gemm_ws_bf16(a3d_stream_t stream, const void* X, int64_t ldx, const void* W, int64_t ldw,
                     const float* bias, const void* rowbias, int64_t rb_div, const void* R, int64_t ldr,
                     void* Y, int64_t ldy, int64_t M, int64_t N, int64_t K, float alpha, float beta, int flags,
                     void* ws, int64_t ws_bytes, int64_t* ws_needed);

int a3d_gemm2_bf16(a3d_stream_t stream, const void* X, int64_t ldx, const void* X2, int64_t ldx2, int64_t K1,
                   const void* W, int64_t ldw, const float* bias, void* Y, int64_t ldy, int64_t M, int64_t N, int64_t K, int flags);

int a3d_gemm_f32out_bf16(a3d_stream_t stream, const void* X, int64_t ldx, const void* W, int64_t ldw,
                         const float* bias, float* Y, int64_t ldy, int64_t M, int64_t N, int64_t K, float alpha);

int a3d_gemm_geglu_bf16(a3d_stream_t stream, const void* X, int64_t ldx, const void* W, int64_t ldw,
                        const float* bias, void* Y, int64_t ldy, int64_t M, int64_t N2, int64_t K, int flags);

int a3d_conv3x3_bf16(a3d_stream_t stream, const void* X, const void* Wp, const float* bias,
                     const void* rowbias, int64_t rb_div, const void* R, void* Y,
                     int B, int H, int W, int Cin, int Cout, int stride, int up2x, int flags);

int a3d_conv3x3_ws_bf16(a3d_stream_t stream, const void* X, const void* Wp, const float* bias,
                        const void* rowbias, int64_t rb_div, const void* R, void* Y,
                        int B, int H, int W, int Cin, int Cout, int stride, int up2x, int flags,
                        void* ws, int64_t ws_bytes, int64_t* ws_needed);

#define A3D_ATTN_ACCUMULATE 1
#define A3D_ATTN_CAUSAL 2
#define A3D_ATTN_EXACT 4
#define A3D_ATTN_PLAIN 8
int a3d_flash_attn_bf16(a3d_stream_t stream, const void* Q, const void* K, const void* V, void* O,
                        const a3d_rowmap* qmap, const a3d_rowmap* kmap, const a3d_rowmap* omap,
                        int groups, int heads, int head_dim, int64_t q_len, int64_t kv_len,
                        float scale, float out_scale, int accumulate);

int a3d_flash_attn_counted_bf16(a3d_stream_t stream, const void* Q, const void* K, const void* V, void* O,
                                const a3d_rowmap* qmap, const a3d_rowmap* kmap, const a3d_rowmap* omap,
                                int groups, int heads, int head_dim, int64_t q_len, int64_t kv_len,
                                float scale, float out_scale, int accumulate, unsigned int* counters);

int a3d_flash_attn2_bf16(a3d_stream_t stream, const void* Q, const void* K, const void* V, const void* K2, const void* V2, void* O,
                         const a3d_rowmap* qmap, const a3d_rowmap* kmap, const a3d_rowmap* kmap2, const a3d_rowmap* omap,
                         int groups, int heads, int head_dim, int64_t q_len, int64_t kv_len, int64_t kv_len2,
                         float scale, float out_scale, float out_scale2, int accumulate);

int a3d_temporal_attn_bf16(a3d_stream_t stream, const void* Q, const void* K, const void* V, int64_t ldqkv,
                           void* O, int64_t ldo, int videos, int frames, int64_t L, int heads,
                           int head_dim, float scale);

int a3d_temporal_attn_sharded_bf16(a3d_stream_t stream, const void* Q, int64_t ldq, const void* K, const void* V, int64_t ldkv,
                                   void* O, int64_t ldo, int videos, int frames, int64_t L, int heads,
                                   int head_dim, float scale, int q_f0, int q_frames, int kv_frames_per_block,
                                   int64_t kv_block_stride);

int64_t a3d_group_norm_ws_floats(int B, int64_t rows, int groups);
int a3d_group_norm_bf16(a3d_stream_t stream, const void* X, void* Y, const float* gamma, const float* beta,
                        float* ws, int B, int64_t rows, int C, int groups, float eps, int silu);

int a3d_group_norm_plan(int64_t rows, int C, int groups, int* out);

int a3d_group_norm2_bf16(a3d_stream_t stream, const void* Xa, int Ca, const void* Xb, int Cb, void* Y, const float* gamma,
                         const float* beta, float* ws, int B, int64_t rows, int groups, float eps, int silu);

int a3d_group_norm_sums_bf16(a3d_stream_t stream, const void* X, float* ws, double* sums, int B, int64_t rows, int C, int groups);
int a3d_group_norm_apply_bf16(a3d_stream_t stream, const void* X, void* Y, const float* gamma, const float* beta,
                              const float* stats, int B, int64_t rows, int C, int groups, int silu);

int a3d_layer_norm_bf16(a3d_stream_t stream, const void* X, void* Y1, void* Y2, const float* gamma,
                        const float* beta, int64_t M, int C, float eps,
                        const void* pe1, int64_t pe1_div, int64_t pe1_mod,
                        const void* pe2, int64_t pe2_div, int64_t pe2_mod);

int a3d_geglu_bf16(a3d_stream_t stream, const void* X, int64_t ldx, void* Y, int64_t ldy, int64_t M, int64_t N);

int a3d_silu_bf16(a3d_stream_t stream, const void* X, void* Y, int64_t n);

int a3d_activation_bf16(a3d_stream_t stream, const void* X, void* Y, int64_t n, int mode);

int a3d_concat_bf16(a3d_stream_t stream, const void* A, int64_t Ca, const void* Bsrc, int64_t Cb, void* Y, int64_t M);

int a3d_timestep_embed_bf16(a3d_stream_t stream, const float* t, void* Y, int V, int dim);

int a3d_im2col_in(a3d_stream_t stream, const void* sample, int dtype, void* Y, int V, int C, int F, int H, int W);

int a3d_im2col_in_bwd(a3d_stream_t stream, const void* dCol, float* dX, int V, int C, int F, int H, int W, float scale);

int a3d_unpack_out(a3d_stream_t stream, const void* X, void* Y, int dtype, int V, int C, int F, int H, int W);

int a3d_softmax_rows_f32_bf16(a3d_stream_t stream, const float* X, int64_t ldx, void* Y, int64_t ldy, int64_t M, int64_t N);

int a3d_softmax_rows_bwd_bf16(a3d_stream_t stream, const void* P, int64_t ldp, const float* dP, int64_t lddp, void* dS, int64_t ldds,
                              int64_t M, int64_t N, float alpha);

int a3d_channel_mix_f32(a3d_stream_t stream, const float* X, const float* W, const float* bias, float* Y,
                        int B, int Cin, int Cout, int64_t HW, float scale);

int a3d_cfg_ddim_step_f32(a3d_stream_t stream, const float* eps_pair, const float* x, const float* first_frame,
                          float* x_prev, int64_t n, int C, int F, int64_t HW, float guidance,
                          float alpha_t, float alpha_prev);



int a3d_flash_attn_bwd_bf16(a3d_stream_t stream, const void* Q, const void* K, const void* V, const void* dO,
                            void* dQ, void* dK, void* dV, float* lse2, float* delta,
                            const a3d_rowmap* qmap, const a3d_rowmap* kmap, const a3d_rowmap* domap,
                            const a3d_rowmap* dqmap, const a3d_rowmap* dkmap,
                            int groups, int heads, int head_dim, int64_t q_len, int64_t kv_len, int q_per_kv,
                            float scale, float do_scale, int accumulate);

int a3d_flash_attn_lse_bf16(a3d_stream_t stream, const void* Q, const void* K, const void* V, void* O,
                            const a3d_rowmap* qmap, const a3d_rowmap* kmap, const a3d_rowmap* omap,
                            int groups, int heads, int head_dim, int64_t q_len, int64_t kv_len,
                            float scale, float out_scale, int accumulate, float* lse2);
int a3d_attn_delta_bf16(a3d_stream_t stream, const void* dO, const void* O, const a3d_rowmap* domap, const a3d_rowmap* omap,
                        float* delta, int groups, int heads, int head_dim, int64_t q_len);

int a3d_temporal_attn_bwd_bf16(a3d_stream_t stream, const void* Q, const void* K, const void* V, int64_t ldqkv,
                               const void* dO, int64_t lddo, void* dQ, void* dK, void* dV, int64_t ldd,
                               int videos, int frames, int64_t L, int heads, int head_dim, float scale);

int a3d_layer_norm_bwd_bf16(a3d_stream_t stream, const void* X, const void* dY, const float* gamma, void* dX,
                            float* dgamma, float* dbeta, int64_t M, int C, float eps, int accumulate);

int a3d_group_norm_bwd_bf16(a3d_stream_t stream, const void* X, const void* dY, const float* gamma, const float* beta,
                            const float* stats, void* dX, float* ws, float* dgamma, float* dbeta,
                            int B, int64_t rows, int C, int groups, int silu);

int a3d_geglu_bwd_bf16(a3d_stream_t stream, const void* P, int64_t ldp, const void* dY, int64_t lddy, void* dP, int64_t lddp,
                       int64_t M, int64_t N);

int a3d_transpose_bf16(a3d_stream_t stream, const void* X, int64_t ldx, void* Y, int64_t ldy, int64_t rows, int64_t cols,
                       int64_t rows_pad);

int64_t a3d_wgrad_ws_floats(int64_t M, int64_t N, int64_t K);
int a3d_wgrad_bf16(a3d_stream_t stream, const void* dY, int64_t lddy, const void* X, int64_t ldx, float* dW, int64_t lddw,
                   float* ws, int64_t M, int64_t N, int64_t K, float alpha, int accumulate);

int a3d_colsum_bf16(a3d_stream_t stream, const void* X, int64_t ldx, int64_t rows, int64_t cols, float* out, float alpha, int accumulate);

int a3d_axpby_bf16(a3d_stream_t stream, const void* X, void* Y, int64_t n, float a, float b);

int a3d_zero_insert2x_bf16(a3d_stream_t stream, const void* dY, void* Z, int B, int H, int W, int C);

int a3d_upsample2x_bwd_bf16(a3d_stream_t stream, const void* dU, void* dX, int B, int H, int W, int He, int We, int C);

int a3d_sqnorm_f32(a3d_stream_t stream, const float* g, int64_t n, float* out, int accumulate);
int a3d_clip_ctrl_f32(a3d_stream_t stream, const float* sqnorm, float max_norm, float inv_loss_scale, float* ctrl);
int a3d_adamw_f32(a3d_stream_t stream, float* p, const float* g, float* m, float* v, int64_t n, float lr, float beta1, float beta2,
                  float eps, float weight_decay, float bias_corr1, float bias_corr2, const float* ctrl);

int a3d_gs_preprocess_f32(a3d_stream_t stream, int B, int N, const float* means, int64_t means_bs, const float* scales, int64_t scales_bs,
                          const float* rots, int64_t rots_bs, const float* opac, int64_t opac_bs, const float* shs, int64_t shs_bs, int M,
                          int deg, const float* colors, int64_t colors_bs, const float* view, const float* proj, const float* campos,
                          const float* tanfovx, const float* tanfovy, int H, int W, float scale_mod, int* radii, float* xy, float* depth,
                          float* conic_o, float* rgb, int* clamped, int* tiles_touched);
int a3d_gs_duplicate_f32(a3d_stream_t stream, int B, int N, int H, int W, const float* xy, const float* depth, const int* radii,
                         const int64_t* offsets, int64_t* keys, int* vals);
int a3d_gs_tile_ranges_f32(a3d_stream_t stream, const int64_t* keys, int64_t L, int* ranges, int64_t n_tiles);
int a3d_gs_render_f32(a3d_stream_t stream, int B, int N, int H, int W, const int* ranges, const int64_t* perm, const int* vals,
                      const float* xy, const float* conic_o, const float* rgb, const float* depth, const float* bg,
                      float* out_img, float* out_depth, float* out_alpha, float* T_final, int* n_contrib);
int a3d_gs_render_bwd_f32(a3d_stream_t stream, int B, int N, int H, int W, const int* ranges, const int64_t* perm, const int* vals,
                          const float* xy, const float* conic_o, const float* rgb, const float* depth, const float* bg,
                          const float* T_final, const int* n_contrib, const float* d_img, const float* d_depth,
                          const float* d_alpha, float* rows);
int a3d_gs_preprocess_bwd_f32(a3d_stream_t stream, int B, int N, const float* means, int64_t means_bs, const float* scales, int64_t scales_bs,
                              const float* rots, int64_t rots_bs, const float* opac, int64_t opac_bs, const float* shs, int64_t shs_bs, int M,
                              int deg, const float* colors, int64_t colors_bs, const float* view, const float* proj, const float* campos,
                              const float* tanfovx, const float* tanfovy, int H, int W, float scale_mod, const int* radii,
                              const int* clamped, const int64_t* offsets, const int* tiles_touched, const float* rows,
                              float* d_means2d, float* d_means, float* d_scales, float* d_rots, float* d_opac, float* d_shs,
                              float* d_colors);
int a3d_gs_sum_batch_f32(a3d_stream_t stream, const float* src, float* dst, int B, int64_t M);

int a3d_dg_cells_f32(a3d_stream_t stream, int N, const float* xyz, const int64_t* plane_desc, int* cells);
int64_t a3d_dg_mean_partials(int N);
int a3d_dg_forward_f32(a3d_stream_t stream, int T, int N, int B, const float* xyz, const float* scaling, const float* rotation,
                       const float* timestamps, const float* grid, const int64_t* plane_desc, const float* weights, int flags,
                       const int* img_start, const int* img_list, float* sp, float* mpart, float* gmean, float* glob, float* means,
                       float* scales, float* rots);
int64_t a3d_dg_backward_ws_floats(int T, int N, const int64_t* plane_desc);
int a3d_dg_backward_f32(a3d_stream_t stream, int T, int N, int B, const float* xyz, const float* scaling, const float* rotation,
                        const float* timestamps, const float* grid, const int64_t* plane_desc, const float* weights, int flags,
                        const int* img_start, const int* img_list, const float* sp, const float* gmean, const float* glob,
                        const int* order, const int* starts, const float* d_means, const float* d_scales, const float* d_rots,
                        float* ws, float* d_grid, float* d_weights, float* d_scaling, float* d_rotation);

int a3d_knn_f32(a3d_stream_t stream, int N, const float* points, int K, int least_edge_num, float radius2, int* nn_idx, float* nn_dist);
int a3d_arap_energy_f32(a3d_stream_t stream, int F, int Nv, int K, int S, const float* source, const float* targets, int64_t targets_bs,
                        const int* nn_idx, const float* weight, const int* sample_idx, double* rot, float* rot_f32, double* energy,
                        float* loss);
int a3d_arap_backward_f32(a3d_stream_t stream, int F, int Nv, int K, int S, const float* source, const float* targets, int64_t targets_bs,
                          const int* nn_idx, const float* weight, const int* sample_idx, const double* rot, const int* order,
                          const int* starts, const float* grad_out, float* d_targets, float* d_source);
int a3d_mesh_sample_neighbours(a3d_stream_t stream, int Nv, int E, const int* row_start, const int* col, int K, const int64_t* seed,
                               int* nn_idx);

int a3d_mesh_vertex_gaussians_f32(a3d_stream_t stream, int Nv, int E, int C, const float* verts, const int* row_start, const int* col,
                                  const int* corner_order, const int* corner_start, const float* vertex_colors, const float* corner_colors,
                                  const float* texture, int Ht, int Wt, const float* uvs, int Nt, const int* corner_uv, const double* rot9,
                                  double scale_factor, double shrink, float* xyz, float* scaling, float* shs, float* colors,
                                  float* mean_edge, float* edge_length);
int a3d_gaussians_rigid_f32(a3d_stream_t stream, int N, const float* xyz_in, const float* scaling_in, const float* rotation_in,
                            const double* rot9, const double* quat4, double scale_factor, float* xyz, float* scaling, float* rotation);

int a3d_mesh_vertex_normals_f32(a3d_stream_t stream, int T, int Nv, int C, const float* pos, const int* faces, const int* order,
                                const int* starts, float* nrm);

int a3d_cameras_spherical_f32(a3d_stream_t stream, int B, const float* elevation, const float* azimuth, const float* distance,
                              const float* fovy, const float* perturb, double angle_unit, double znear, double zfar, float* c2w, float* w2c,
                              float* full_proj, float* campos, float* tanfov);
int a3d_cameras_random_f32(a3d_stream_t stream, int R, int n_view, int total_frame, const float* obj, const float* pert_u,
                           const float* pert_n, const double* ranges10, int elev_mode, int relative_radius, double camera_perturb,
                           double center_perturb, double up_perturb, double znear, double zfar, float* c2w, float* w2c, float* full_proj,
                           float* campos, float* tanfov, float* elevation_deg, float* azimuth_deg, float* fovy, float* camera_distances);
int a3d_cameras_from_c2w_f32(a3d_stream_t stream, int B, const float* c2w, const float* fovy, double znear, double zfar, float* w2c,
                             float* full_proj, float* campos, float* tanfov);

int a3d_recon_loss_f32(a3d_stream_t stream, int B, int H, int W, const float* image, const float* alpha, const float* gt_rgb,
                       const uint8_t* gt_mask, const int* index, float bg, double lambda_rgb, double lambda_mask, float* partials,
                       int64_t n_partials, float* out);
int a3d_recon_loss_bwd_f32(a3d_stream_t stream, int B, int H, int W, const float* image, const float* alpha, const float* gt_rgb,
                           const uint8_t* gt_mask, const int* index, float bg, float coef_rgb, float coef_mask, const float* grad_out,
                           float* d_image, float* d_alpha);

int a3d_image_reg_f32(a3d_stream_t stream, int B, int H, int W, const float* image, const float* depth, const float* alpha, double lambda_tv,
                      double lambda_depth_tv, double lambda_sparsity, float* partials, int64_t n_partials, float* out);
int a3d_image_reg_bwd_f32(a3d_stream_t stream, int B, int H, int W, const float* image, const float* depth, const float* alpha,
                          float coef_tv_h, float coef_tv_w, float coef_depth_tv_h, float coef_depth_tv_w, float coef_sparsity,
                          const float* grad_out, float* d_image, float* d_depth, float* d_alpha);
int a3d_gaussian_reg_f32(a3d_stream_t stream, int B, int N, const float* means, const float* scales, int64_t scales_bs, const float* scaling,
                         const float* opacity, double lambda_position, double lambda_scales, double lambda_opacity, float* partials,
                         int64_t n_partials, float* out);
int a3d_gaussian_reg_bwd_f32(a3d_stream_t stream, int B, int N, const float* means, const float* scaling, float coef_position,
                             float coef_scales, float coef_opacity, const float* grad_out, float* d_means, float* d_scales,
                             float* d_opacity);

int64_t a3d_clip_preprocess_lds_limit(void);
int a3d_clip_preprocess(a3d_stream_t stream, const float* rgb, int n_src, int in_h, int in_w, int64_t s_img, int64_t s_y, int64_t s_x,
                        int64_t s_c, const int* image_index, int n_img, int crop, const int* coef_x, const int* bounds_x, int ksize_x,
                        int off_x, const int* coef_y, const int* bounds_y, int ksize_y, int off_y, int tile_rows, int max_rows,
                        const float* table, int dtype, void* pixel_values, void* patch_rows, int patch, int kp, uint8_t* u8);

int a3d_gemm_f16(a3d_stream_t stream, const void* X, int64_t ldx, const void* W, int64_t ldw,
                  const float* bias, const void* rowbias, int64_t rb_div, const void* R, int64_t ldr,
                  void* Y, int64_t ldy, int64_t M, int64_t N, int64_t K, float alpha, float beta, int flags);
int a3d_gemm_ws_f16(a3d_stream_t stream, const void* X, int64_t ldx, const void* W, int64_t ldw,
                    const float* bias, const void* rowbias, int64_t rb_div, const void* R, int64_t ldr,
                    void* Y, int64_t ldy, int64_t M, int64_t N, int64_t K, float alpha, float beta, int flags,
                    void* ws, int64_t ws_bytes, int64_t* ws_needed);
int a3d_gemm2_f16(a3d_stream_t stream, const void* X, int64_t ldx, const void* X2, int64_t ldx2, int64_t K1,
                  const void* W, int64_t ldw, const float* bias, void* Y, int64_t ldy, int64_t M, int64_t N, int64_t K, int flags);
int a3d_gemm_f32out_f16(a3d_stream_t stream, const void* X, int64_t ldx, const void* W, int64_t ldw,
                         const float* bias, float* Y, int64_t ldy, int64_t M, int64_t N, int64_t K, float alpha);
int a3d_gemm_geglu_f16(a3d_stream_t stream, const void* X, int64_t ldx, const void* W, int64_t ldw,
                        const float* bias, void* Y, int64_t ldy, int64_t M, int64_t N2, int64_t K, int flags);
int a3d_conv3x3_f16(a3d_stream_t stream, const void* X, const void* Wp, const float* bias,
                     const void* rowbias, int64_t rb_div, const void* R, void* Y,
                     int B, int H, int W, int Cin, int Cout, int stride, int up2x, int flags);
int a3d_conv3x3_ws_f16(a3d_stream_t stream, const void* X, const void* Wp, const float* bias,
                       const void* rowbias, int64_t rb_div, const void* R, void* Y,
                       int B, int H, int W, int Cin, int Cout, int stride, int up2x, int flags,
                       void* ws, int64_t ws_bytes, int64_t* ws_needed);
int a3d_flash_attn_f16(a3d_stream_t stream, const void* Q, const void* K, const void* V, void* O,
                        const a3d_rowmap* qmap, const a3d_rowmap* kmap, const a3d_rowmap* omap,
                        int groups, int heads, int head_dim, int64_t q_len, int64_t kv_len,
                        float scale, float out_scale, int accumulate);
int a3d_flash_attn_counted_f16(a3d_stream_t stream, const void* Q, const void* K, const void* V, void* O,
                               const a3d_rowmap* qmap, const a3d_rowmap* kmap, const a3d_rowmap* omap,
                               int groups, int heads, int head_dim, int64_t q_len, int64_t kv_len,
                               float scale, float out_scale, int accumulate, unsigned int* counters);
int a3d_flash_attn2_f16(a3d_stream_t stream, const void* Q, const void* K, const void* V, const void* K2, const void* V2, void* O,
                        const a3d_rowmap* qmap, const a3d_rowmap* kmap, const a3d_rowmap* kmap2, const a3d_rowmap* omap,
                        int groups, int heads, int head_dim, int64_t q_len, int64_t kv_len, int64_t kv_len2,
                        float scale, float out_scale, float out_scale2, int accumulate);
int a3d_temporal_attn_f16(a3d_stream_t stream, const void* Q, const void* K, const void* V, int64_t ldqkv,
                           void* O, int64_t ldo, int videos, int frames, int64_t L, int heads,
                           int head_dim, float scale);
int a3d_temporal_attn_sharded_f16(a3d_stream_t stream, const void* Q, int64_t ldq, const void* K, const void* V, int64_t ldkv,
                                   void* O, int64_t ldo, int videos, int frames, int64_t L, int heads,
                                   int head_dim, float scale, int q_f0, int q_frames, int kv_frames_per_block,
                                   int64_t kv_block_stride);
int a3d_group_norm_f16(a3d_stream_t stream, const void* X, void* Y, const float* gamma, const float* beta,
                        float* ws, int B, int64_t rows, int C, int groups, float eps, int silu);
int a3d_group_norm2_f16(a3d_stream_t stream, const void* Xa, int Ca, const void* Xb, int Cb, void* Y, const float* gamma,
                        const float* beta, float* ws, int B, int64_t rows, int groups, float eps, int silu);
int a3d_group_norm_sums_f16(a3d_stream_t stream, const void* X, float* ws, double* sums, int B, int64_t rows, int C, int groups);
int a3d_group_norm_apply_f16(a3d_stream_t stream, const void* X, void* Y, const float* gamma, const float* beta,
                              const float* stats, int B, int64_t rows, int C, int groups, int silu);
int a3d_layer_norm_f16(a3d_stream_t stream, const void* X, void* Y1, void* Y2, const float* gamma,
                        const float* beta, int64_t M, int C, float eps,
                        const void* pe1, int64_t pe1_div, int64_t pe1_mod,
                        const void* pe2, int64_t pe2_div, int64_t pe2_mod);
int a3d_geglu_f16(a3d_stream_t stream, const void* X, int64_t ldx, void* Y, int64_t ldy, int64_t M, int64_t N);
int a3d_silu_f16(a3d_stream_t stream, const void* X, void* Y, int64_t n);
int a3d_activation_f16(a3d_stream_t stream, const void* X, void* Y, int64_t n, int mode);
int a3d_concat_f16(a3d_stream_t stream, const void* A, int64_t Ca, const void* Bsrc, int64_t Cb, void* Y, int64_t M);
int a3d_timestep_embed_f16(a3d_stream_t stream, const float* t, void* Y, int V, int dim);
int a3d_im2col_in_f16(a3d_stream_t stream, const void* sample, int dtype, void* Y, int V, int C, int F, int H, int W);
int a3d_unpack_out_f16(a3d_stream_t stream, const void* X, void* Y, int dtype, int V, int C, int F, int H, int W);
int a3d_softmax_rows_f32_f16(a3d_stream_t stream, const float* X, int64_t ldx, void* Y, int64_t ldy, int64_t M, int64_t N);
int a3d_softmax_rows_bwd_f16(a3d_stream_t stream, const void* P, int64_t ldp, const float* dP, int64_t lddp, void* dS, int64_t ldds,
                             int64_t M, int64_t N, float alpha);
int a3d_im2col_in_bwd_f16(a3d_stream_t stream, const void* dCol, float* dX, int V, int C, int F, int H, int W, float scale);
int a3d_flash_attn_bwd_f16(a3d_stream_t stream, const void* Q, const void* K, const void* V, const void* dO,
                            void* dQ, void* dK, void* dV, float* lse2, float* delta,
                            const a3d_rowmap* qmap, const a3d_rowmap* kmap, const a3d_rowmap* domap,
                            const a3d_rowmap* dqmap, const a3d_rowmap* dkmap,
                            int groups, int heads, int head_dim, int64_t q_len, int64_t kv_len, int q_per_kv,
                            float scale, float do_scale, int accumulate);
int a3d_flash_attn_lse_f16(a3d_stream_t stream, const void* Q, const void* K, const void* V, void* O,
                           const a3d_rowmap* qmap, const a3d_rowmap* kmap, const a3d_rowmap* omap,
                           int groups, int heads, int head_dim, int64_t q_len, int64_t kv_len,
                           float scale, float out_scale, int accumulate, float* lse2);
int a3d_attn_delta_f16(a3d_stream_t stream, const void* dO, const void* O, const a3d_rowmap* domap, const a3d_rowmap* omap,
                       float* delta, int groups, int heads, int head_dim, int64_t q_len);
int a3d_temporal_attn_bwd_f16(a3d_stream_t stream, const void* Q, const void* K, const void* V, int64_t ldqkv,
                               const void* dO, int64_t lddo, void* dQ, void* dK, void* dV, int64_t ldd,
                               int videos, int frames, int64_t L, int heads, int head_dim, float scale);
int a3d_layer_norm_bwd_f16(a3d_stream_t stream, const void* X, const void* dY, const float* gamma, void* dX,
                            float* dgamma, float* dbeta, int64_t M, int C, float eps, int accumulate);
int a3d_group_norm_bwd_f16(a3d_stream_t stream, const void* X, const void* dY, const float* gamma, const float* beta,
                            const float* stats, void* dX, float* ws, float* dgamma, float* dbeta,
                            int B, int64_t rows, int C, int groups, int silu);
int a3d_geglu_bwd_f16(a3d_stream_t stream, const void* P, int64_t ldp, const void* dY, int64_t lddy, void* dP, int64_t lddp,
                       int64_t M, int64_t N);
int a3d_transpose_f16(a3d_stream_t stream, const void* X, int64_t ldx, void* Y, int64_t ldy, int64_t rows, int64_t cols,
                       int64_t rows_pad);
int a3d_colsum_f16(a3d_stream_t stream, const void* X, int64_t ldx, int64_t rows, int64_t cols, float* out, float alpha, int accumulate);
int a3d_axpby_f16(a3d_stream_t stream, const void* X, void* Y, int64_t n, float a, float b);
int a3d_zero_insert2x_f16(a3d_stream_t stream, const void* dY, void* Z, int B, int H, int W, int C);
int a3d_upsample2x_bwd_f16(a3d_stream_t stream, const void* dU, void* dX, int B, int H, int W, int He, int We, int C);
int a3d_wgrad_f16(a3d_stream_t stream, const void* dY, int64_t lddy, const void* X, int64_t ldx, float* dW, int64_t lddw,
                   float* ws, int64_t M, int64_t N, int64_t K, float alpha, int accumulate);

#ifdef __cplusplus
}
#endif
#endif
```

Measured before the change: 2.417 denoise-steps/s.

## Fold nearest-upsample into 3x3 conv as four 2x2 phase convolutions

Adds a CONV==3 path that computes a nearest-2x upsample followed by a 3x3 conv as four sub-pixel phases. Each phase is a 2x2 conv on the low-resolution input, using weights pre-summed on the host at pack time. The epilogue scatters rows to interleaved high-resolution output positions. This cuts the reduction length from 9 to 4 taps per output and reads the small input directly, at the cost of a weight-folding precompute and strided output writes. It only applies when there is no residual, no rowbias and no split-K.

```diff
diff --git a/animate3d_amd/csrc/gemm_common.h b/animate3d_amd/csrc/gemm_common.h
--- a/animate3d_amd/csrc/gemm_common.h
+++ b/animate3d_amd/csrc/gemm_common.h
@@ -144,10 +144,19 @@
   fw[NB - 1] = *reinterpret_cast<const u32x4_t*>(wl + ko);
 }
 
-template <int EPI, int NB>
+struct RowSame { __device__ __forceinline__ int64_t operator()(int64_t m) const { return m; } };
+struct RowUp2x {
+  uint32_t W; int a, b;
+  __device__ __forceinline__ int64_t operator()(int64_t m) const {
+    const uint32_t q = (uint32_t)m / W, j = (uint32_t)m - q * W;
+    return (int64_t)(2u * q + (uint32_t)a) * (2u * W) + 2u * j + (uint32_t)b;
+  }
+};
+
+template <int EPI, int NB, class ROW = RowSame>
 A3D_DEV void epilogue_rounded(const GemmParams& p, f32x16_t (&acc)[NB][2], float* const stg, const float* const bias_lds,
                               const uint16_t* const rowbias_lds, const int64_t m0, const int64_t n0, const int wm, const WaveCols<NB> wc,
-                              const int lane) {
+                              const int lane, const ROW orow = ROW{}) {
   const int wblk = wc.first, wblk_last = wc.last;
   auto pass_cols = [&](int ps) { return (2 * ps + 1 < NB) ? 64 : 32; };
   auto pass_col0 = [&](int ps) { return ((2 * ps + 1 < NB) ? wblk + 2 * ps : wblk_last) * 32; };
@@ -276,7 +285,7 @@
         const int row = (64 / lpr) * j + lane / lpr;
         const int64_t m = mbase + row;
         const u32x4_t o = unswap(ob[j], row);
-        *reinterpret_cast<u32x4_t*>(p.Y + m * p.ldy + nbase + 8 * cc) = o;
+        *reinterpret_cast<u32x4_t*>(p.Y + orow(m) * p.ldy + nbase + 8 * cc) = o;
       }
     }
   }
diff --git a/animate3d_amd/csrc/gemm_conv.hip b/animate3d_amd/csrc/gemm_conv.hip
--- a/animate3d_amd/csrc/gemm_conv.hip
+++ b/animate3d_amd/csrc/gemm_conv.hip
@@ -28,7 +28,10 @@
 
   const int64_t nblk = p.tiles_n * p.tiles_m;
   const int64_t lid = xcd_remap(blockIdx.x, nblk);
-  const int64_t tile_n = lid % p.tiles_n, tile_m = lid / p.tiles_n;
+  const int64_t tile_n = lid % p.tiles_n, tile_mp = lid / p.tiles_n;
+  const int phase = CONV == 3 ? (int)(tile_mp & 3) : 0;
+  const int pa = phase >> 1, pb = phase & 1;
+  const int64_t tile_m = CONV == 3 ? tile_mp >> 2 : tile_mp;
   const int64_t m0 = tile_m * BM, n0 = tile_n * BN;
 
   const int kc = tid % TC::CPR;
@@ -51,6 +54,16 @@
       if constexpr (CONV == 2) {
         a_b[i] = b; a_y[i] = oy; a_x[i] = ox;
         a_ptr[i] = nullptr; a_mask[i] = 0;
+      } else if constexpr (CONV == 3) {
+        const int y0 = oy + pa - 1, x0 = ox + pb - 1;
+        a_ptr[i] = p.X + (((int64_t)b * p.H + y0) * p.Wd + x0) * p.Cin + kc * 8;
+        int mask = 0;
+#pragma unroll
+        for (int t = 0; t < 4; ++t) {
+          const int yy = y0 + (t >> 1), xx = x0 + (t & 1);
+          if (a_ok[i] && yy >= 0 && yy < p.H && xx >= 0 && xx < p.Wd) mask |= 1 << t;
+        }
+        a_mask[i] = mask;
       } else {
         const int y0 = oy * p.stride - 1, x0 = ox * p.stride - 1;
         a_ptr[i] = p.X + (((int64_t)b * p.H + y0) * p.Wd + x0) * p.Cin + kc * 8;
@@ -72,7 +85,7 @@
   for (int i = 0; i < NPASS; ++i) {
     int64_t n = n0 + srow + RPT * i;
     if (n >= p.N) n = p.N - 1;
-    w_ptr[i] = p.W + n * p.ldw + kc * 8;
+    w_ptr[i] = p.W + ((CONV == 3 ? phase * p.N : 0) + n) * p.ldw + kc * 8;
   }
 
   struct RegTile { u32x4_t a[NPASS], w[NPASS]; };
@@ -81,14 +94,16 @@
     u32x4_t (&ra)[NPASS] = rt.a; u32x4_t (&rw)[NPASS] = rt.w;
     if constexpr (CONV != 0) {
       {
+        constexpr int NT = CONV == 3 ? 4 : 9;
         const int kt64 = (int)(k0 >> 6);
-        const int c64 = kt64 / 9, t = kt64 - 9 * c64;
+        const int c64 = kt64 / NT, t = kt64 - NT * c64;
         k0 = (int64_t)t * p.Cin + c64 * 64 + (k0 & 63);
       }
+      constexpr int TW = CONV == 3 ? 2 : 3;
       const int tap = (int)(k0 / p.Cin);
       const int ci0 = (int)(k0 - (int64_t)tap * p.Cin);
-      const int ky = tap / 3, kx = tap - ky * 3;
-      if constexpr (CONV == 1) {
+      const int ky = tap / TW, kx = tap - ky * TW;
+      if constexpr (CONV == 1 || CONV == 3) {
         const int64_t toff = ((int64_t)ky * p.Wd + kx) * p.Cin + ci0;
 #pragma unroll
         for (int i = 0; i < NPASS; ++i) {
@@ -249,6 +264,7 @@
         const int row = 8 * j + (lane >> 3);
         const int64_t m = mbase + row;
         if (m >= p.M) continue;
+        const int64_t mo = CONV == 3 ? RowUp2x{(uint32_t)p.Wd, pa, pb}(m) : m;
         const float4 a0 = *reinterpret_cast<const float4*>(stg + row * SROW + 8 * cc);
         const float4 a1 = *reinterpret_cast<const float4*>(stg + row * SROW + 8 * cc + 4);
         float v[8] = {a0.x, a0.y, a0.z, a0.w, a1.x, a1.y, a1.z, a1.w};
@@ -256,7 +272,7 @@
         for (int e = 0; e < 8; ++e) v[e] += bv[e];
         const uint16_t* rb = p.rowbias ? p.rowbias + (m / p.rb_div) * p.N + n : nullptr;
         const uint16_t* rr = p.R ? p.R + m * p.ldr + n : nullptr;
-        uint16_t* yy = p.Y + m * p.ldy + n;
+        uint16_t* yy = p.Y + mo * p.ldy + n;
         if (full) {
           if (rb) {
             const u32x4_t t = *reinterpret_cast<const u32x4_t*>(rb);
@@ -273,7 +289,7 @@
             }
           }
           if (p.out_f32) {
-            float* yf = reinterpret_cast<float*>(p.Y) + m * p.ldy + n;
+            float* yf = reinterpret_cast<float*>(p.Y) + mo * p.ldy + n;
             *reinterpret_cast<float4*>(yf) = float4{v[0], v[1], v[2], v[3]};
             *reinterpret_cast<float4*>(yf + 4) = float4{v[4], v[5], v[6], v[7]};
           } else {
@@ -346,9 +362,9 @@
   if (CONV == 0 && (uint64_t)p.ldx * 16u >= (1ull << 31)) return false;
   if ((uint64_t)p.ldw * 16u >= (1ull << 31)) return false;
   if (CONV != 0 && ((uint64_t)p.B * p.H * p.Wd + 2u * p.Wd + 2u) * (uint64_t)p.Cin * 2u >= (1ull << 32)) return false;
-  const int64_t tm = (p.M + PBM - 1) / PBM;
+  const int64_t tm = (p.M + PBM - 1) / PBM * (CONV == 3 ? 4 : 1);
   const int nk = (int)(p.K / 64);
-  const int unit = CONV ? 9 : 1;
+  const int unit = CONV == 3 ? 4 : CONV ? 9 : 1;
   const int cus_plan = cus_dev;
   constexpr int OVH = 12;
   int64_t best = -1, best1 = -1;
@@ -420,7 +436,7 @@
 
 template <int CONV, int EPI, int BKT>
 int launch_bk(hipStream_t stream, GemmParams& p, int64_t nblk) {
-  if constexpr (EPI == EPI_LINEAR) {
+  if constexpr (EPI == EPI_LINEAR && CONV != 3) {
     if (p.R != nullptr) return launch_res<CONV, EPI, BKT, true>(stream, p, nblk);
   }
   return launch_res<CONV, EPI, BKT, false>(stream, p, nblk);
@@ -449,7 +465,7 @@
     const int rc = try_launch_persist<CONV, EPI>(stream, p, flags);
     if (rc != NOT_ELIGIBLE) return rc;
   }
-  p.tiles_m = (p.M + BM - 1) / BM;
+  p.tiles_m = (p.M + BM - 1) / BM * (CONV == 3 ? 4 : 1);
   p.tiles_n = (p.N + BN - 1) / BN;
   const int64_t nblk = p.tiles_m * p.tiles_n;
   if (nblk <= 0 || nblk > 0x7fffffffLL) return A3D_EINVAL;
@@ -575,6 +591,25 @@
   return conv_entry(stream, X, Wp, bias, rowbias, rb_div, R, Y, B, H, W, Cin, Cout, stride, up2x, flags, ws, ws_bytes, ws_needed);
 }
 
+extern "C" int A3D_FN(a3d_conv_up2x_folded)(a3d_stream_t stream, const void* X, const void* Wf, const float* bias,
+                                         const void* rowbias, const void* R, void* Y,
+                                         int B, int H, int W, int Cin, int Cout, int flags) {
+  if (!X || !Wf || !Y || B <= 0 || H <= 0 || W <= 0) return A3D_EINVAL;
+  if (Cin <= 0 || Cin % 64 != 0 || Cout <= 0 || Cout % 4 != 0) return A3D_EINVAL;
+  if (!a3d_aligned(16, X, Wf) || !a3d_aligned(16, bias) || !a3d_aligned(8, Y)) return A3D_EINVAL;
+  if (rowbias || R) return A3D_EINVAL;
+  if ((int64_t)B * H * W >= (1ll << 29)) return A3D_EINVAL;
+  GemmParams p{};
+  p.X = (const uint16_t*)X; p.ldx = Cin; p.W = (const uint16_t*)Wf; p.ldw = (int64_t)4 * Cin;
+  p.bias = bias; p.rb_div = 1; p.ldr = Cout; p.Y = (uint16_t*)Y; p.ldy = Cout;
+  p.B = B; p.H = H; p.Wd = W; p.Cin = Cin; p.stride = 1; p.up = 1; p.He = 2 * H; p.We = 2 * W;
+  p.Ho = H; p.Wo = W;
+  p.M = (int64_t)B * H * W; p.N = Cout; p.K = (int64_t)4 * Cin;
+  p.alpha = 1.f; p.beta = 1.f;
+  p.vec16 = (Cout % 8 == 0) && a3d_aligned(16, Y);
+  return launch<3>((hipStream_t)stream, p, flags);
+}
+
 extern "C" int A3D_FN(a3d_gemm_geglu)(a3d_stream_t stream, const void* X, int64_t ldx, const void* W, int64_t ldw,
                                    const float* bias, void* Y, int64_t ldy, int64_t M, int64_t N2, int64_t K, int flags) {
   GemmParams p = dense_params(X, ldx, W, ldw, bias, nullptr, 1, nullptr, 0, Y, ldy, M, N2, K, 1.f, 0.f);
diff --git a/animate3d_amd/csrc/gemm_pp.hip b/animate3d_amd/csrc/gemm_pp.hip
--- a/animate3d_amd/csrc/gemm_pp.hip
+++ b/animate3d_amd/csrc/gemm_pp.hip
@@ -27,6 +27,8 @@
 template <int CONV, int EPI, int NB, bool RES, bool SPLIT = false, bool TWO = false>
 __global__ __launch_bounds__(512, 1) void gemm_pp_kernel(const GemmParams p) {
   static_assert(!TWO || CONV == 0, "the two-source A operand is a dense-GEMM feature");
+  static_assert(CONV != 3 || (!SPLIT && !RES && EPI == EPI_LINEAR), "the folded up-conv has no split-K, no residual and a linear epilogue");
+  constexpr int NT = CONV == 3 ? 4 : 9;
   using PC = PPCfg<NB>;
   constexpr int PH = 1, NPH = 4;
   constexpr int NP = 4 + NB;
@@ -78,13 +80,16 @@
     const int64_t tile_id = SPLIT ? (int64_t)((uint32_t)tt / (uint32_t)S) : tt;
     const int64_t kofs = SPLIT ? (CONV ? ((int64_t)(tt - tile_id * S) * nk / 9) * 64 : (int64_t)(tt - tile_id * S) * nk * 64) : 0;
     pp_tile_coords(tile_id, p.tiles_m, p.tiles_n, tile_m, tile_n);
+    const int phase = CONV == 3 ? (int)(tile_m & 3) : 0;
+    const int pa = phase >> 1, pb = phase & 1;
+    if constexpr (CONV == 3) tile_m >>= 2;
     ld_m0 = tile_m * PBM; ld_n0 = tile_n * PC::BN;
     ik0 = 0; itap = 0; ikx = 0; iky = 0;
     ld_par ^= 1;
     if constexpr (CONV != 0) xck = (uint64_t)(uintptr_t)p.X - (uint64_t)cbias * 2u + (uint64_t)kofs * 2u;
     if constexpr (CONV == 0) xk = (uint64_t)(uintptr_t)(p.X + (ld_m0 + wid * 32) * p.ldx + kofs);
     if constexpr (TWO) xk2 = (uint64_t)(uintptr_t)(p.X2 + (ld_m0 + wid * 32) * p.ldx2);
-    wk = (uint64_t)(uintptr_t)(p.W + (ld_n0 + wid * (NB * 8)) * p.ldw + kofs);
+    wk = (uint64_t)(uintptr_t)(p.W + ((CONV == 3 ? phase * p.N : 0) + ld_n0 + wid * (NB * 8)) * p.ldw + kofs);
     if (EPI == EPI_LINEAR && p.rowbias) rbk = (uint64_t)(uintptr_t)(p.rowbias + (ld_m0 / p.rb_div) * p.N + ld_n0);
     if constexpr (CONV != 0) {
       amask[0] = 0; amask[1] = 0;
@@ -107,6 +112,15 @@
             if (yy >= 0 && yy < p.He && xx >= 0 && xx < p.We) mask |= 1u << tp;
           }
           amask[i >> 1] |= (mask << (9 * (i & 1))) | ((uint32_t)(~oy & 1) << (18 + 2 * (i & 1))) | ((uint32_t)(~ox & 1) << (19 + 2 * (i & 1)));
+        } else if constexpr (CONV == 3) {
+          const int y0 = oy + pa - 1, x0 = ox + pb - 1;
+          aoff[i] = (uint32_t)(((((int64_t)b * p.H + y0) * p.Wd + x0) * p.Cin + cbias) * 2 + slot * 16);
+#pragma unroll
+          for (int tp = 0; tp < 4; ++tp) {
+            const int yy = y0 + (tp >> 1), xx = x0 + (tp & 1);
+            if (yy >= 0 && yy < p.H && xx >= 0 && xx < p.Wd) mask |= 1u << tp;
+          }
+          amask[i >> 1] |= mask << (4 * (i & 1));
         } else {
           const int y0 = oy * p.stride - 1, x0 = ox * p.stride - 1;
           aoff[i] = (uint32_t)(((((int64_t)b * p.H + y0) * p.Wd + x0) * p.Cin + cbias) * 2 + slot * 16);
@@ -120,7 +134,7 @@
       }
       sok[0] = 0; sok[1] = 0;
 #pragma unroll
-      for (int bit = 0; bit < 18; ++bit) {
+      for (int bit = 0; bit < 2 * NT; ++bit) {
         if (__builtin_amdgcn_ballot_w64(((amask[0] >> bit) & 1u) != 0u) == ~0ull) sok[0] |= 1u << bit;
         if (__builtin_amdgcn_ballot_w64(((amask[1] >> bit) & 1u) != 0u) == ~0ull) sok[1] |= 1u << bit;
       }
@@ -154,7 +168,7 @@
         const uint32_t mk = amask[i >> 1];
         uint32_t vo = aoff[i];
         if constexpr (CONV == 2) vo += (((mk >> (18 + 2 * (i & 1))) & 1u) ? yE : yO) + (((mk >> (19 + 2 * (i & 1))) & 1u) ? xE : xO);
-        const int bit = itap + 9 * (i & 1);
+        const int bit = itap + NT * (i & 1);
         if ((sok[i >> 1] >> bit) & 1u) {
           glds16_s(vo, (const void*)(uintptr_t)xck, d);
         } else {
@@ -184,13 +198,14 @@
         const uint64_t cin2 = (uint64_t)(uint32_t)p.Cin * 2u;
         wk += cin2;
         ++itap;
-        if (++ikx == 3) { ikx = 0; ++iky; }
-        if (itap == 9) {
-          itap = 0; iky = 0; wk -= 9u * cin2 - 128u;
-          if constexpr (CONV == 1) xck -= (2u * (uint64_t)(uint32_t)p.Wd + 2u) * cin2;
+        constexpr int TW = CONV == 3 ? 2 : 3;
+        if (++ikx == TW) { ikx = 0; ++iky; }
+        if (itap == NT) {
+          itap = 0; iky = 0; wk -= (uint64_t)NT * cin2 - 128u;
+          if constexpr (CONV == 1 || CONV == 3) xck -= ((uint64_t)(TW - 1) * (uint64_t)(uint32_t)p.Wd + (uint64_t)(TW - 1)) * cin2;
           xck += 128u;
-        } else if constexpr (CONV == 1) {
-          xck += ikx == 0 ? ((uint64_t)(uint32_t)p.Wd - 2u) * cin2 : cin2;
+        } else if constexpr (CONV == 1 || CONV == 3) {
+          xck += ikx == 0 ? ((uint64_t)(uint32_t)p.Wd - (uint64_t)(TW - 1)) * cin2 : cin2;
         }
       } else {
         if (TWO && ik0 >= (int)p.K1) xk2 += 128; else xk += 128;
@@ -240,7 +255,7 @@
   for (;;) {
     int64_t tile_n, tile_m;
     pp_tile_coords(SPLIT ? (int64_t)((uint32_t)t / (uint32_t)S) : t, p.tiles_m, p.tiles_n, tile_m, tile_n);
-    const int64_t m0 = tile_m * PBM, n0 = tile_n * PC::BN;
+    const int64_t m0 = (CONV == 3 ? tile_m >> 2 : tile_m) * PBM, n0 = tile_n * PC::BN;
     const int64_t tnext = t + G;
 #pragma unroll
     for (int a = 0; a < NB; ++a)
@@ -291,7 +306,9 @@
       float* const stg = reinterpret_cast<float*>(smem_b + (buf ^ 1) * PC::STAGE) + wid * (32 * 68);
       const float* const bias_lds = bias_image(smem_b + PC::BIAS_OFF, cur_par);
       const uint16_t* const rowbias_lds = rowbias_image(smem_b + PC::BIAS_OFF, cur_par);
-      if constexpr (EPI == EPI_GEGLU || !RES) epilogue_rounded<EPI, NB>(p, acc, stg, bias_lds, rowbias_lds, m0, n0, wm, wc, lane);
+      if constexpr (CONV == 3) epilogue_rounded<EPI, NB>(p, acc, stg, bias_lds, rowbias_lds, m0, n0, wm, wc, lane,
+                                                         RowUp2x{(uint32_t)p.Wd, (int)(tile_m & 3) >> 1, (int)(tile_m & 1)});
+      else if constexpr (EPI == EPI_GEGLU || !RES) epilogue_rounded<EPI, NB>(p, acc, stg, bias_lds, rowbias_lds, m0, n0, wm, wc, lane);
       else epilogue_residual<NB>(p, acc, stg, bias_lds, rowbias_lds, m0, n0, wm, wc, lane);
     }
     if (tnext >= ntiles) break;
@@ -381,6 +398,12 @@
       return A3D_EUNSUPPORTED;
     }
   }
+  if constexpr (CONV == 3) {
+    if (p.ksplit > 1 || p.R || p.rowbias) return A3D_EUNSUPPORTED;
+    if (nb == 5) return launch_pp<3, EPI_LINEAR, 5, false>(stream, p, cus);
+    if (nb == 4) return launch_pp<3, EPI_LINEAR, 4, false>(stream, p, cus);
+    return A3D_EUNSUPPORTED;
+  } else {
   if (p.ksplit > 1) {
     if (nb == 5) return launch_pp<CONV, EPI_LINEAR, 5, false, true>(stream, p, cus);
     if (nb == 4) return launch_pp<CONV, EPI_LINEAR, 4, false, true>(stream, p, cus);
@@ -389,6 +412,7 @@
   if (nb == 5) return p.R ? launch_pp<CONV, EPI_LINEAR, 5, true>(stream, p, cus) : launch_pp<CONV, EPI_LINEAR, 5, false>(stream, p, cus);
   if (nb == 4) return p.R ? launch_pp<CONV, EPI_LINEAR, 4, true>(stream, p, cus) : launch_pp<CONV, EPI_LINEAR, 4, false>(stream, p, cus);
   return A3D_EUNSUPPORTED;
+  }
 }
 
 }
@@ -396,5 +420,6 @@
 int A3D_FN(a3d_launch_gemm_pp)(int conv, int epi, int nb, hipStream_t stream, const GemmParams& p, int cus) {
   if (conv == 0) return launch_pp_conv<0>(epi, nb, stream, p, cus);
   if (conv == 1) return launch_pp_conv<1>(epi, nb, stream, p, cus);
-  return launch_pp_conv<2>(epi, nb, stream, p, cus);
-}
+  if (conv == 2) return launch_pp_conv<2>(epi, nb, stream, p, cus);
+  return launch_pp_conv<3>(epi, nb, stream, p, cus);
+}
diff --git a/animate3d_amd/hip_ops.py b/animate3d_amd/hip_ops.py
--- a/animate3d_amd/hip_ops.py
+++ b/animate3d_amd/hip_ops.py
@@ -52,6 +52,7 @@
     "a3d_conv3x3_bf16": (c_int, [c_vp, c_vp, c_vp, c_vp, c_vp, c_i64, c_vp, c_vp, c_int, c_int, c_int, c_int, c_int, c_int, c_int, c_int]),
     "a3d_conv3x3_ws_bf16": (c_int, [c_vp, c_vp, c_vp, c_vp, c_vp, c_i64, c_vp, c_vp, c_int, c_int, c_int, c_int, c_int, c_int, c_int, c_int,
                                     c_vp, c_i64, ctypes.POINTER(c_i64)]),
+    "a3d_conv_up2x_folded_bf16": (c_int, [c_vp, c_vp, c_vp, c_vp, c_vp, c_vp, c_vp, c_int, c_int, c_int, c_int, c_int, c_int]),
     "a3d_flash_attn_bf16": (c_int, [c_vp, c_vp, c_vp, c_vp, c_vp, ctypes.POINTER(_RowMapC), ctypes.POINTER(_RowMapC), ctypes.POINTER(_RowMapC),
                                     c_int, c_int, c_int, c_i64, c_i64, c_f32, c_f32, c_int]),
     "a3d_flash_attn_counted_bf16": (c_int, [c_vp, c_vp, c_vp, c_vp, c_vp, ctypes.POINTER(_RowMapC), ctypes.POINTER(_RowMapC), ctypes.POINTER(_RowMapC),
@@ -334,8 +335,21 @@
         _check(rc, f"a3d_gemm_geglu_bf16 M={M} N2={N2} K={K}")
         return y
 
+    @staticmethod
+    def fold_up2x(w9: torch.Tensor, dtype: Optional[torch.dtype] = None) -> torch.Tensor:
+        Cout, K9 = w9.shape
+        assert K9 % 9 == 0
+        w = w9.detach().float().reshape(Cout, 3, 3, K9 // 9)
+        sets = (((0,), (1, 2)), ((0, 1), (2,)))
+        out = []
+        for a in range(2):
+            for b in range(2):
+                taps = [sum(w[:, ky, kx] for ky in sets[a][ty] for kx in sets[b][tx]) for ty in range(2) for tx in range(2)]
+                out.append(torch.stack(taps, dim=1).reshape(Cout, -1))
+        return torch.stack(out, dim=0).to(dtype if dtype is not None else w9.dtype).contiguous()
+
     def conv3x3(self, x, B: int, H: int, W: int, w, bias, *, stride: int = 1, up2x: bool = False, rowbias=None, rb_div: int = 1, residual=None,
-                up_size=None, tile128: bool = False):
+                up_size=None, tile128: bool = False, folded=None):
         x, w = self._act(x, "conv.x"), self._act(w, "conv.w")
         Cin = x.shape[1]
         Cout = w.shape[0]
@@ -366,6 +380,12 @@
                 ws = self._workspace(need)
                 _check(self.lib.a3d_conv3x3_ws_bf16(*args, _p(ws), need, None), f"a3d_conv3x3_ws_bf16 B={B} H={H} W={W} Cin={Cin} Cout={Cout}")
                 return y, Ho, Wo
+        if folded is not None and up_code == 1 and stride == 1 and rowbias is None and residual is None:
+            self._act(folded.view(-1, folded.shape[-1]), "conv.folded")
+            assert folded.is_contiguous() and folded.shape == (4, Cout, 4 * Cin)
+            rc = self.lib.a3d_conv_up2x_folded_bf16(self._stream(), _p(x), _p(folded), _p(bias), None, None, _p(y), B, H, W, Cin, Cout, flags)
+            _check(rc, f"a3d_conv_up2x_folded_bf16 B={B} H={H} W={W} Cin={Cin} Cout={Cout}")
+            return y, Ho, Wo
         rc = self.lib.a3d_conv3x3_bf16(*args)
         _check(rc, f"a3d_conv3x3_bf16 B={B} H={H} W={W} Cin={Cin} Cout={Cout} stride={stride} up={up2x}")
         return y, Ho, Wo
diff --git a/animate3d_amd/unet.py b/animate3d_amd/unet.py
--- a/animate3d_amd/unet.py
+++ b/animate3d_amd/unet.py
@@ -477,7 +477,13 @@
         return out
 
     def _pack_block(self, blk: M.MotionBlock):
+        upf = None
+        ops = self._base_ops()
+        if blk.upsamplers is not None and not self._pack_grad and hasattr(ops, "fold_up2x"):
+            w = blk.upsamplers[0].conv.weight.detach()
+            upf = ops.fold_up2x(w.permute(0, 2, 3, 1).reshape(w.shape[0], -1), ops.act_dtype)
         return SimpleNamespace(
+            upf=upf,
             resnets=[self._pack_resnet(r) for r in blk.resnets],
             t2d=[self._pack_t2d(t) for t in blk.attentions] if blk.has_cross_attention else None,
             motion=[self._pack_motion(m) for m in blk.motion_modules],
@@ -1123,7 +1129,8 @@
                 x = layer((x, skip) if pair else ops.concat(x, skip), rp, pk.t2d[j] if pk.t2d is not None else None, pk.motion[j], h_, w_)
             if pk.up is not None:
                 lvl -= 1
-                x, h_, w_ = ops.conv3x3(x, B2, h_, w_, pk.up[0], pk.up[1], up2x=True, up_size=sizes[lvl])
+                fold = dict(folded=pk.upf) if self._active_ops is None and getattr(pk, "upf", None) is not None else {}
+                x, h_, w_ = ops.conv3x3(x, B2, h_, w_, pk.up[0], pk.up[1], up2x=True, up_size=sizes[lvl], **fold)
         x = ops.group_norm(x, B2, h_ * w_, P.norm_out[0], P.norm_out[1], cfg.norm_num_groups, cfg.norm_eps, True)
         x, _, _ = ops.conv3x3(x, B2, h_, w_, P.conv_out[0], P.conv_out[1])
         out_dtype = sample.dtype if sample.dtype in (torch.float32, torch.bfloat16, torch.float16) else torch.float32
diff --git a/include/animate3d_hip.h b/include/animate3d_hip.h
--- a/include/animate3d_hip.h
+++ b/include/animate3d_hip.h
@@ -55,6 +55,10 @@
                         const void* rowbias, int64_t rb_div, const void* R, void* Y,
                         int B, int H, int W, int Cin, int Cout, int stride, int up2x, int flags,
                         void* ws, int64_t ws_bytes, int64_t* ws_needed);
+
+int a3d_conv_up2x_folded_bf16(a3d_stream_t stream, const void* X, const void* Wf, const float* bias,
+                              const void* rowbias, const void* R, void* Y,
+                              int B, int H, int W, int Cin, int Cout, int flags);
 
 #define A3D_ATTN_ACCUMULATE 1
 #define A3D_ATTN_CAUSAL 2
@@ -293,6 +297,9 @@
                        const void* rowbias, int64_t rb_div, const void* R, void* Y,
                        int B, int H, int W, int Cin, int Cout, int stride, int up2x, int flags,
                        void* ws, int64_t ws_bytes, int64_t* ws_needed);
+int a3d_conv_up2x_folded_f16(a3d_stream_t stream, const void* X, const void* Wf, const float* bias,
+                             const void* rowbias, const void* R, void* Y,
+                             int B, int H, int W, int Cin, int Cout, int flags);
 int a3d_flash_attn_f16(a3d_stream_t stream, const void* Q, const void* K, const void* V, void* O,
                         const a3d_rowmap* qmap, const a3d_rowmap* kmap, const a3d_rowmap* omap,
                         int groups, int heads, int head_dim, int64_t q_len, int64_t kv_len,
```

Result: no change. 2.435 denoise-steps/s (median of 6 runs) (+0.8%).
